# abajcsy/legged_games_gym

Hardware: AMD Instinct MI355X
Metric: env-steps/sec (whole node), ANYmal-C flat 4096 envs/GPU (higher is better)
Workload: dtype f32; 1 GPU; anymal_c_flat, 4096 envs/GPU, plane, actuator-net torques, self-collision ON (asset.self_collisions = 0), random-init policy [48, 128, 64, 32, 12] rollout (act = mu + sigma*eps), fixed command (0.5,0,0), obs noise + friction/mass randomisation + pushes on; envs_per_gpu=4096, decimation=4, parallelism=env-sharded x1, state_finite=True, policy=MFMA actor inside k_step (v_mfma_f32_16x16x4_f32, 4 waves)

## Files before the change

### legged_games_gym_amd/csrc/lg_kernels.hip

```cpp
#include <hip/hip_runtime.h>
#include <math.h>
#include <stdio.h>
#include <string.h>
#include <new>

#define LG_POLICY_BLOCKS_ONLY
#include "lg_host.h"

using namespace lg;

#define LG_BLOCK 64
#define LG_JS 40
#define LG_PASSES 2
#define LG_STEP_WAVES 4

struct AnymalTraits {
    static constexpr int K = 4, L = 3, NREP = 4, NPT = 5;
    static constexpr int pt_joint(int i) { return i < 2 ? 1 : 2; }
    static constexpr int pt_rep(int i) { return i < 2 ? 1 : (i < 4 ? 2 : 3); }
    static constexpr int FOOT_REP = 3;
    static constexpr int NCAP = 3, NGRP = 2;
    static constexpr int cap_p0(int c) { return 2 * c; }
    static constexpr int cap_p1(int c) { return c < 2 ? 2 * c + 1 : 4; }
    static constexpr int cap_grp(int c) { return c == 0 ? 0 : 1; }
    static constexpr int grp_c0(int g) { return g == 0 ? 0 : 2; }
    static constexpr int grp_c1(int g) { return g == 0 ? 1 : 4; }
    static constexpr int grp_cap_lo(int g) { return g == 0 ? 0 : 1; }
    static constexpr int grp_cap_hi(int g) { return g == 0 ? 1 : 3; }
};
struct CassieTraits {
    static constexpr int K = 2, L = 6, NREP = 6, NPT = 2;
    static constexpr int pt_joint(int) { return 5; }
    static constexpr int pt_rep(int) { return 5; }
    static constexpr int FOOT_REP = 5;
    static constexpr int NCAP = 1, NGRP = 1;
    static constexpr int cap_p0(int) { return 0; }
    static constexpr int cap_p1(int) { return 1; }
    static constexpr int cap_grp(int) { return 0; }
    static constexpr int grp_c0(int) { return 0; }
    static constexpr int grp_c1(int) { return 1; }
    static constexpr int grp_cap_lo(int) { return 0; }
    static constexpr int grp_cap_hi(int) { return 1; }
};
template <class T> struct Tab { static constexpr int GRP = T::L * LG_JS + 4 * T::NPT;
                          static constexpr int BPT = GRP + T::NGRP + 1;
                          static constexpr int STRIDE = BPT + 4; };
enum { J_POS = 0, J_ROT = 3, J_AXIS = 12, J_MASS = 15, J_COM = 16, J_INERTIA = 19, J_LO = 25, J_HI = 26, J_VLIM = 27,
       J_ARM = 28, J_DAMP = 29, J_KP = 30, J_KD = 31, J_Q0 = 32, J_TLIM = 33, J_SLO = 34, J_SHI = 35, J_DVL = 36,
       J_SUBM = 37  };

struct BaseTab { float mass, com[3], inertia[6]; float pts[LG_MAX_BASE_POINTS][4]; int32_t num_pts; float mass_robot; };

struct RollArgs {
    int      steps;
    float   *obs;
    const float *obs0;
    float   *actions, *mean;
    float   *rew;
    uint8_t *done, *time_outs;
    float   *extras;
    int      sub;
    int     *cursor;
};

struct PostHead {
    int32_t  resample_interval, heading_command, push_interval, max_episode_length;
    float    max_push_vel; uint32_t termination_mask, penalised_mask, _pad0;
    int64_t *episode_length_buf; float *commands, *contact_forces; uint32_t _pad[2];
};
struct PostRew {
    float    dt_policy, soft_dof_vel_limit, soft_torque_limit, max_contact_force, base_height_target, tracking_sigma;
    int32_t  only_positive_rewards; uint32_t slot_mask ; int32_t num_height_points, terrain_curriculum;
    float   *last_actions, *feet_air_time; uint8_t *last_contacts;
    float    reward_scale[LG_NUM_REWARD_TERMS];
    float   *env_origins; uint32_t _pad[2];
};
struct PostObs {
    float    obs_scale_lin_vel, obs_scale_ang_vel, obs_scale_dof_pos, obs_scale_dof_vel;
    float    noise_lin_vel, noise_ang_vel, noise_gravity, noise_dof_pos, noise_dof_vel, clip_observations;
    int32_t  add_noise, num_obs, num_envs; uint32_t _pad;
    float   *roll_obs;
};
struct PostStore {
    float   *dof_state, *actions, *torques, *last_actions, *last_dof_vel, *feet_air_time; uint8_t *last_contacts; float *root_states;
};
struct PostStoreEnv {
    float   *last_root_vel, *commands, *base_lin_vel, *base_ang_vel, *projected_gravity, *rew_buf; uint8_t *reset_buf, *time_out_buf;
    int64_t *episode_length_buf; float *roll_rew; uint8_t *roll_done, *roll_time_outs;
};
struct PostArgs { PostHead head; PostRew rew; PostObs obs; PostStore store; PostStoreEnv store_env; };
static_assert(sizeof(PostHead) == 64 && sizeof(PostRew) == 160 && sizeof(PostObs) == 64 && sizeof(PostStore) == 64 && sizeof(PostStoreEnv) == 96, "blocks of whole 8-dword groups, no padding");
static_assert(LG_NUM_REWARD_TERMS <= 32, "PostRew::slot_mask");

struct KArgs {
    lg_params  P;
    lg_buffers B;
    BaseTab    base;
    const float *limb_table;
    const float *hpts;
    const float *weights;
    const float *actions_in;
    const int32_t *env_ids;
    int32_t    count;
    uint32_t   penalised_mask, termination_mask;
    unsigned int *done_counter;
    float *accum_alt;
    int   flush_parts;
    int   defer;
    int64_t    step;
    PolicyArgs pol;
    unsigned long long *prof;
    unsigned int *status;
    int   spin_limit;
    int   debug_skip;
    RollArgs roll;
    PostArgs post;
};

template <bool ROLL> LG_DEV const KArgs &step_args(const KArgs &A) {
    if constexpr (ROLL) {
        typedef __attribute__((address_space(4))) const KArgs *KernArgs;
        KernArgs p = (KernArgs)__builtin_amdgcn_kernarg_segment_ptr();
        asm volatile("" : "+s"(p));
        return *(const KArgs *)p;
    } else return A;
}

typedef uint32_t lg_u32x16 __attribute__((ext_vector_type(16)));
typedef uint32_t lg_u32x8 __attribute__((ext_vector_type(8)));
template <class S> struct KargFetch {
    static_assert(sizeof(S) % 32 == 0 && sizeof(S) <= 192, "blocks are fetched 16 and 8 dwords at a time");
    static constexpr int N16 = sizeof(S) / 64, N8 = sizeof(S) % 64 / 32;
    lg_u32x16 a[N16 ? N16 : 1];
    lg_u32x8  b;
};
template <class S> LG_DEV KargFetch<S> karg_request(const S &src) {
    typedef lg_u32x16 __attribute__((aligned(4))) w16;
    typedef lg_u32x8 __attribute__((aligned(4))) w8;
    typedef __attribute__((address_space(4))) const char *kptr;
    const kptr p = (kptr)reinterpret_cast<const char *>(&src);
    KargFetch<S> f;
#pragma unroll
    for (int i = 0; i < KargFetch<S>::N16; i++) f.a[i] = *(__attribute__((address_space(4))) const w16 *)(p + 64 * i);
    if constexpr (KargFetch<S>::N8 != 0) f.b = *(__attribute__((address_space(4))) const w8 *)(p + 64 * KargFetch<S>::N16);
    return f;
}
template <class S> LG_DEV S karg_take(KargFetch<S> &f) {
    S out;
#pragma unroll
    for (int i = 0; i < KargFetch<S>::N16; i++) { asm volatile("" : "+s"(f.a[i])); __builtin_memcpy(reinterpret_cast<char *>(&out) + 64 * i, &f.a[i], 64); }
    if constexpr (KargFetch<S>::N8 != 0) { asm volatile("" : "+s"(f.b)); __builtin_memcpy(reinterpret_cast<char *>(&out) + 64 * KargFetch<S>::N16, &f.b, 32); }
    return out;
}

LG_DEV const double *cmd_x_range(const KArgs &A) { return A.P.cmd_curriculum ? A.B.cmd_range : nullptr; }
LG_DEV void cmd_x_range_f32(const KArgs &A, float *out) {
    const double *xr = cmd_x_range(A);
    out[0] = xr ? (float)xr[0] : A.P.cmd_lin_vel_x[0];
    out[1] = xr ? (float)xr[1] : A.P.cmd_lin_vel_x[1];
}
LG_DEV bool curriculum_tick_step(const KArgs &A, int64_t step) {
    return A.P.cmd_curriculum && A.step < 0 && A.P.max_episode_length > 0 && step % A.P.max_episode_length == 0;
}

LG_DEV void lg_report(unsigned int *status, unsigned int bit) {
    if (status) __hip_atomic_fetch_or(status, bit, __ATOMIC_RELAXED, __HIP_MEMORY_SCOPE_SYSTEM);
}

#define LG_NPROF 20
#define LG_NPROF_BLOCKS 1024
#define LG_NPROF_ROLL 33
#define LG_NPROF_TOTAL (LG_NPROF + LG_NPROF_BLOCKS * 40 + LG_NPROF_ROLL * LG_NPROF_BLOCKS)
#ifdef LG_PROFILE
__device__ __forceinline__ void lg_prof(int idx, unsigned long long *out, unsigned long long note = 0) {
    __shared__ unsigned long long acc[LG_NPROF], prev, t0, w0;
    __builtin_amdgcn_sched_barrier(0);
    unsigned long long t = __builtin_readcyclecounter();
    if (threadIdx.x == 0) {
        if (idx < 0) { for (int i = 0; i < LG_NPROF; i++) acc[i] = 0; t0 = t; w0 = wall_clock64(); }
        else if (idx >= 18) { if (idx == 18) acc[18] = note; else acc[19] += note; t = prev; }
        else acc[idx] += t - prev;
        if (out) {
            acc[14] = t - t0; acc[15] = wall_clock64() - w0;
            if (blockIdx.x < LG_NPROF_BLOCKS) {
                unsigned long long *a = out + LG_NPROF + (size_t)blockIdx.x * 40, *b = a + 20;
                for (int i = 0; i < 16; i++) { a[i] += acc[i]; b[i] = acc[i]; }
                a[16] = a[16] > acc[14] ? a[16] : acc[14];
                b[16] = w0; b[17] = w0 + acc[15]; b[18] = acc[18]; b[19] = acc[19];
            }
        }
        prev = idx >= 18 ? prev : __builtin_readcyclecounter();
    }
    __builtin_amdgcn_sched_barrier(0);
}
#ifdef LG_PROFILE_LIGHT
#define LG_PROF(i)
#else
#define LG_PROF(i) lg_prof(i, nullptr)
#endif
#define LG_PROF_NOTE(i, v) lg_prof(i, nullptr, v)
#define LG_PROF_BEGIN() lg_prof(-1, nullptr)
#define LG_PROF_END(i, out) lg_prof(i, out)
#ifdef LG_PROFILE_LIGHT
#define LG_PROF_COUNT(f, cond) do { if ((f) == 1 || (f) == 2) { if (__ballot(cond)) lg_prof(19, nullptr, 1ull << (8 * (f))); } } while (0)
#else
#define LG_PROF_COUNT(f, cond) do { const unsigned long long b_ = __ballot(cond); if (b_) lg_prof(19, nullptr, (1ull << (8 * (f))) + ((f) == 0 ? (unsigned long long)__popcll(b_) << 48 : 0ull)); } while (0)
#endif
#else
#define LG_PROF(i)
#define LG_PROF_BEGIN()
#define LG_PROF_END(i, out)
#define LG_PROF_NOTE(i, v)
#define LG_PROF_COUNT(f, cond)
#endif
enum { PF_PROLOGUE = 0, PF_TORQUE, PF_KINEMATICS, PF_INWARD, PF_BASE, PF_OUTWARD, PF_INTEGRATE, PF_POST, PF_EXTRAS,
       PF_POST_HEIGHTS, PF_POST_TERMS, PF_POST_REWARD, PF_POST_RESET, PF_POST_OBS };

struct HfFetch { int16_t s00, s10, s01, s11; float tx, ty; };
template <bool HF> LG_DEV HfFetch hf_fetch(const KArgs &A, float x, float y) {
    HfFetch f; f.s00 = f.s10 = f.s01 = f.s11 = 0; f.tx = f.ty = 0.0f;
    if (!HF) return f;
    const lg_params &P = A.P;
    float inv = 1.0f / P.hf_horizontal_scale;
    float gx = (x + P.hf_border) * inv, gy = (y + P.hf_border) * inv;
    if (!(fabsf(gx) < 1e9f)) gx = 0.0f;
    if (!(fabsf(gy) < 1e9f)) gy = 0.0f;
    float fx = floorf(gx), fy = floorf(gy);
    int ix = (int)fx, iy = (int)fy;
    f.tx = gx - fx; f.ty = gy - fy;
    auto at = [&](int i, int j) {
        i = min(max(i, 0), P.hf_rows - 1); j = min(max(j, 0), P.hf_cols - 1);
        return A.B.height_samples[(size_t)i * P.hf_cols + j];
    };
    f.s00 = at(ix, iy); f.s10 = at(ix + 1, iy); f.s01 = at(ix, iy + 1); f.s11 = at(ix + 1, iy + 1);
    return f;
}
template <bool HF> LG_DEV void hf_contact(const KArgs &A, const HfFetch &f, float pz, float radius, float &depth, V3 &n) {
    if (!HF) { n = v3(0, 0, 1); depth = radius - pz; return; }
    const lg_params &P = A.P;
    float inv = 1.0f / P.hf_horizontal_scale;
    float h00 = (float)f.s00 * P.hf_vertical_scale, h10 = (float)f.s10 * P.hf_vertical_scale;
    float h01 = (float)f.s01 * P.hf_vertical_scale, h11 = (float)f.s11 * P.hf_vertical_scale;
    const float thr = P.hf_step_threshold;
    float wall_depth = -1e30f; V3 wall_n = v3(0, 0, 1);
    if (thr > 0.0f) {
        const float hs = P.hf_horizontal_scale;
        if (fmaxf(fabsf(h10 - h00), fabsf(h11 - h01)) > thr) {
            const bool up = (h10 + h11) > (h00 + h01);
            const float top = up ? h10 + (h11 - h10) * f.ty : h00 + (h01 - h00) * f.ty;
            const float dist = (up ? 1.0f - f.tx : f.tx) * hs;
            if (pz - radius < top) {
                float d = radius - dist; V3 fn = v3(up ? -1.0f : 1.0f, 0, 0);
                if (pz > top) {
                    const float dz = pz - top, len = sqrtf(dist * dist + dz * dz), il = 1.0f / fmaxf(len, 1e-9f);
                    d = radius - len; fn = v3((up ? -dist : dist) * il, 0, dz * il);
                }
                if (d > wall_depth) { wall_depth = d; wall_n = fn; }
            }
            if (up) { h10 = h00; h11 = h01; } else { h00 = h10; h01 = h11; }
        }
        if (fmaxf(fabsf(h01 - h00), fabsf(h11 - h10)) > thr) {
            const bool up = (h01 + h11) > (h00 + h10);
            const float top = up ? h01 + (h11 - h01) * f.tx : h00 + (h10 - h00) * f.tx;
            const float dist = (up ? 1.0f - f.ty : f.ty) * hs;
            if (pz - radius < top) {
                float d = radius - dist; V3 fn = v3(0, up ? -1.0f : 1.0f, 0);
                if (pz > top) {
                    const float dz = pz - top, len = sqrtf(dist * dist + dz * dz), il = 1.0f / fmaxf(len, 1e-9f);
                    d = radius - len; fn = v3(0, (up ? -dist : dist) * il, dz * il);
                }
                if (d > wall_depth) { wall_depth = d; wall_n = fn; }
            }
            if (up) { h01 = h00; h11 = h10; } else { h00 = h01; h10 = h11; }
        }
    }
    float hx0 = h00 + (h10 - h00) * f.tx, hx1 = h01 + (h11 - h01) * f.tx;
    float h = hx0 + (hx1 - hx0) * f.ty;
    float dhdx = ((h10 - h00) + ((h11 - h01) - (h10 - h00)) * f.ty) * inv;
    float dhdy = (hx1 - hx0) * inv;
    float l = 1.0f / sqrtf(dhdx * dhdx + dhdy * dhdy + 1.0f);
    n = v3(-dhdx * l, -dhdy * l, l);
    depth = radius - (pz - h) * n.z;
    if (wall_depth > depth) { depth = wall_depth; n = wall_n; }
}
struct Contact { V3 r, n, vc, f, fs; float depth, bt, vtn; bool on; };

LG_DEV float prod_rn(float a, float b) {
#pragma clang fp contract(off)
    return a * b;
}
LG_DEV float sub_rn(float a, float b) {
#pragma clang fp contract(off)
    return a - b;
}
LG_DEV float plane_normal_force(const lg_params &P, float kn, float depth, float vz) {
    return __builtin_fmaf(-kn, vz, prod_rn(P.contact_stiffness, depth));
}
LG_DEV V3 plane_force(const Contact &c, V3 v, float fn) {
    return v3(sub_rn(c.fs.x, prod_rn(v.x, c.bt)), sub_rn(c.fs.y, prod_rn(v.y, c.bt)), fn);
}
LG_DEV float plane_slip_speed(V3 v) { return sqrtf(__builtin_fmaf(v.x, v.x, prod_rn(v.y, v.y))); }

template <bool HF>
LG_DEV void contact_setup(Contact &c, const lg_params &P, float mu, V3 r, V3 n, float depth, V3 vc, V3 fprev) {
    if constexpr (!HF) {
        c.r = r; c.depth = depth; c.vc = vc; c.on = depth > -P.contact_margin; c.f = v3(0, 0, 0); c.fs = v3(0, 0, 0);
        c.vtn = plane_slip_speed(vc);
        float fn_est = fmaxf(fprev.z, 0.0f);
        c.bt = fminf(P.friction_damping, mu * fn_est / fmaxf(c.vtn, P.stick_velocity));
        return;
    }
    c.r = r; c.n = n; c.depth = depth; c.vc = vc; c.on = depth > -P.contact_margin; c.f = v3(0, 0, 0); c.fs = v3(0, 0, 0);
    float vn0 = dot(n, vc);
    V3 vt0 = vc - n * vn0;
    c.vtn = sqrtf(dot(vt0, vt0));
    float fn_est = fmaxf(dot(n, fprev), 0.0f);
    c.bt = fminf(P.friction_damping, mu * fn_est / fmaxf(c.vtn, P.stick_velocity));
}
template <bool HF>
LG_DEV void contact_assemble(const Contact &c, const lg_params &P, float kn, AI &IA, S6 &pA) {
    if constexpr (!HF) {
        if (c.on) {
            const float dt = P.sim_dt;
            const V3 f = plane_force(c, c.vc, plane_normal_force(P, kn, c.depth, c.vc.z));
            ai_add_point(IA, dt * c.bt, c.r);
            const float kk = kn - c.bt, k = prod_rn(dt, kk), kx = prod_rn(k, c.r.x), ky = prod_rn(k, c.r.y);
            IA.A[0] = __builtin_fmaf(ky, c.r.y, IA.A[0]); IA.A[1] = __builtin_fmaf(-c.r.x, ky, IA.A[1]); IA.A[3] = __builtin_fmaf(kx, c.r.x, IA.A[3]);
            IA.H[2] = __builtin_fmaf(c.r.y, k, IA.H[2]); IA.H[5] = __builtin_fmaf(-c.r.x, k, IA.H[5]);
            IA.M[5] = __builtin_fmaf(dt, kk, IA.M[5]);
            const V3 rxf = v3(__builtin_fmaf(c.r.y, f.z, -prod_rn(c.r.z, f.y)), __builtin_fmaf(c.r.z, f.x, -prod_rn(c.r.x, f.z)),
                              __builtin_fmaf(c.r.x, f.y, -prod_rn(c.r.y, f.x)));
            pA.w = pA.w - rxf;
            pA.v = pA.v - f;
            asm volatile("" : "+v"(IA.H[0]), "+v"(IA.H[4]), "+v"(IA.H[8]), "+v"(IA.M[1]), "+v"(IA.M[2]), "+v"(IA.M[4]));
        }
        return;
    }
    if (c.on) {
        const float dt = P.sim_dt;
        float vn = dot(c.n, c.vc);
        V3 vt = c.vc - c.n * vn;
        V3 f = c.n * (P.contact_stiffness * c.depth - kn * vn) - vt * c.bt + c.fs;
        ai_add_point(IA, dt * c.bt, c.r);
        ai_add_rank1(IA, dt * (kn - c.bt), cross(c.r, c.n), c.n);
        pA.w = pA.w - cross(c.r, f);
        pA.v = pA.v - f;
    }
}
template <bool HF>
LG_DEV void contact_evaluate(Contact &c, const lg_params &P, float kn, float mu, S6 acc, bool more = true) {
    if constexpr (!HF) {
        if (c.on) {
            V3 v1 = c.vc + (acc.v + cross(acc.w, c.r)) * P.sim_dt;
            float fn = plane_normal_force(P, kn, c.depth, v1.z);
            if (fn <= 0.0f) { c.on = false; c.f = v3(0, 0, 0); }
            else {
                c.f = plane_force(c, v1, fn);
                if (!more) return;
                float vtm = plane_slip_speed(v1), cone = mu * fn;
                if (c.bt * vtm > cone) { const float s = -cone / vtm; c.fs = v3(v1.x * s, v1.y * s, 0.0f); c.bt = 0.0f; }
                else if (c.bt > 0.0f) c.bt = fminf(P.friction_damping, cone / fmaxf(vtm, P.stick_velocity));
            }
        }
        return;
    }
    if (c.on) {
        V3 v1 = c.vc + (acc.v + cross(acc.w, c.r)) * P.sim_dt;
        float vn = dot(c.n, v1);
        V3 vt = v1 - c.n * vn;
        float fn = P.contact_stiffness * c.depth - kn * vn;
        if (fn <= 0.0f) { c.on = false; c.f = v3(0, 0, 0); }
        else {
            c.f = c.n * fn - vt * c.bt + c.fs;
            if (!more) return;
            float vtm = sqrtf(dot(vt, vt)), cone = mu * fn;
            if (c.bt * vtm > cone) { c.fs = vt * (-cone / vtm); c.bt = 0.0f; }
            else if (c.bt > 0.0f) c.bt = fminf(P.friction_damping, cone / fmaxf(vtm, P.stick_velocity));
        }
    }
}

LG_DEV float motor_torque(float tau, float qd, float vlim) {
    if (vlim <= 0.0f || tau * qd <= 0.0f) return tau;
    float s = (vlim - fabsf(qd)) / (0.1f * vlim);
    return tau * fminf(fmaxf(s, 0.0f), 1.0f);
}
LG_DEV V3 clamp_norm(V3 a, float lim) {
    float n2 = dot(a, a);
    if (!(n2 <= lim * lim)) { float k = (n2 > 0.0f && n2 < INFINITY) ? lim * __builtin_amdgcn_rsqf(n2) : 0.0f; return a * k; }
    return a;
}

LG_DEV void body_terms(V3 grav, float m, V3 com_l, const float *Il, const M3 &R, V3 w, V3 v, RI &I0, S6 &p0) {
    V3 c = mul(R, com_l);
    M3 Ilf; Ilf.m[0] = Il[0]; Ilf.m[1] = Il[1]; Ilf.m[2] = Il[2]; Ilf.m[3] = Il[1]; Ilf.m[4] = Il[3]; Ilf.m[5] = Il[4];
    Ilf.m[6] = Il[2]; Ilf.m[7] = Il[4]; Ilf.m[8] = Il[5];
    M3 Rt;
#pragma unroll
    for (int i = 0; i < 3; i++)
#pragma unroll
        for (int j2 = 0; j2 < 3; j2++) Rt.m[3 * i + j2] = R.m[3 * j2 + i];
    M3 Ic = mul(mul(R, Ilf), Rt);
    I0.A[0] = Ic.m[0]; I0.A[1] = Ic.m[1]; I0.A[2] = Ic.m[2]; I0.A[3] = Ic.m[4]; I0.A[4] = Ic.m[5]; I0.A[5] = Ic.m[8];
    {
        float cc = dot(c, c);
        I0.A[0] += m * (cc - c.x * c.x); I0.A[1] -= m * c.x * c.y; I0.A[2] -= m * c.x * c.z;
        I0.A[3] += m * (cc - c.y * c.y); I0.A[4] -= m * c.y * c.z; I0.A[5] += m * (cc - c.z * c.z);
    }
    I0.h = v3(prod_rn(m, c.x), prod_rn(m, c.y), prod_rn(m, c.z));
    I0.m = m;
    V3 l = (v + cross(w, c)) * m;
    V3 n = mul(Ic, w) + cross(c, l);
    V3 fg = grav * m;
    p0.w = (cross(w, n) + cross(v, l)) - cross(c, fg);
    p0.v = cross(w, l) - fg;
}
LG_DEV void body_terms(V3 grav, float m, V3 com_l, const float *Il, const M3 &R, V3 w, V3 v, AI &I0, S6 &p0) {
    V3 c = mul(R, com_l);
    M3 Ilf; Ilf.m[0] = Il[0]; Ilf.m[1] = Il[1]; Ilf.m[2] = Il[2]; Ilf.m[3] = Il[1]; Ilf.m[4] = Il[3]; Ilf.m[5] = Il[4];
    Ilf.m[6] = Il[2]; Ilf.m[7] = Il[4]; Ilf.m[8] = Il[5];
    M3 Rt;
#pragma unroll
    for (int i = 0; i < 3; i++)
#pragma unroll
        for (int j2 = 0; j2 < 3; j2++) Rt.m[3 * i + j2] = R.m[3 * j2 + i];
    M3 Ic = mul(mul(R, Ilf), Rt);
#pragma unroll
    for (int i = 0; i < 9; i++) I0.H[i] = 0.0f;
#pragma unroll
    for (int i = 0; i < 6; i++) I0.M[i] = 0.0f;
    I0.A[0] = Ic.m[0]; I0.A[1] = Ic.m[1]; I0.A[2] = Ic.m[2]; I0.A[3] = Ic.m[4]; I0.A[4] = Ic.m[5]; I0.A[5] = Ic.m[8];
    ai_add_point(I0, m, c);
    V3 l = (v + cross(w, c)) * m;
    V3 n = mul(Ic, w) + cross(c, l);
    V3 fg = grav * m;
    p0.w = (cross(w, n) + cross(v, l)) - cross(c, fg);
    p0.v = cross(w, l) - fg;
}
struct FkOut { M3 R; V3 db, ax, w, v; };
LG_DEV FkOut fk_joint(const float *tj, const M3 &Rpar, V3 wpar, V3 vpar, float q, float qd) {
    FkOut o;
    o.db = mul(Rpar, v3(tj[J_POS], tj[J_POS + 1], tj[J_POS + 2]));
    M3 Rfix;
#pragma unroll
    for (int i = 0; i < 9; i++) Rfix.m[i] = tj[J_ROT + i];
    const M3 Rz = mul(Rpar, Rfix);
    o.ax = v3(Rz.m[0], Rz.m[3], Rz.m[6]);
    float sn, cs;
    __sincosf(q, &sn, &cs);
#pragma unroll
    for (int r = 0; r < 3; r++) {
        o.R.m[3 * r] = Rz.m[3 * r];
        o.R.m[3 * r + 1] = cs * Rz.m[3 * r + 1] + sn * Rz.m[3 * r + 2];
        o.R.m[3 * r + 2] = cs * Rz.m[3 * r + 2] - sn * Rz.m[3 * r + 1];
    }
    o.w = wpar + o.ax * qd;
    o.v = vpar + cross(wpar, o.db);
    return o;
}
template <bool HF> struct RigidOf { typedef RI type; };
template <> struct RigidOf<true> { typedef AI type; };
template <bool HF> struct BtQuads { static constexpr int N = HF ? 7 : 4; };
LG_DEV void bt_store(float4 (*dst)[LG_BLOCK], int lane, const RI &I, const S6 &p) {
    dst[0][lane] = make_float4(I.A[0], I.A[1], I.A[2], I.A[3]); dst[1][lane] = make_float4(I.A[4], I.A[5], I.h.x, I.h.y);
    dst[2][lane] = make_float4(I.h.z, I.m, p.w.x, p.w.y); dst[3][lane] = make_float4(p.w.z, p.v.x, p.v.y, p.v.z);
}
LG_DEV void bt_store(float4 (*dst)[LG_BLOCK], int lane, const AI &I, const S6 &p) {
    dst[0][lane] = make_float4(I.A[0], I.A[1], I.A[2], I.A[3]); dst[1][lane] = make_float4(I.A[4], I.A[5], I.H[0], I.H[1]);
    dst[2][lane] = make_float4(I.H[2], I.H[3], I.H[4], I.H[5]); dst[3][lane] = make_float4(I.H[6], I.H[7], I.H[8], I.M[0]);
    dst[4][lane] = make_float4(I.M[1], I.M[2], I.M[3], I.M[4]); dst[5][lane] = make_float4(I.M[5], p.w.x, p.w.y, p.w.z);
    dst[6][lane] = make_float4(p.v.x, p.v.y, p.v.z, 0.0f);
}
LG_DEV void bt_load(const float4 (*src)[LG_BLOCK], int lane, AI &I, S6 &p) {
    float4 a = src[0][lane], b = src[1][lane], c = src[2][lane], d = src[3][lane], e = src[4][lane], f = src[5][lane], g = src[6][lane];
    I.A[0] = a.x; I.A[1] = a.y; I.A[2] = a.z; I.A[3] = a.w; I.A[4] = b.x; I.A[5] = b.y; I.H[0] = b.z; I.H[1] = b.w;
    I.H[2] = c.x; I.H[3] = c.y; I.H[4] = c.z; I.H[5] = c.w; I.H[6] = d.x; I.H[7] = d.y; I.H[8] = d.z; I.M[0] = d.w;
    I.M[1] = e.x; I.M[2] = e.y; I.M[3] = e.z; I.M[4] = e.w; I.M[5] = f.x; p.w = v3(f.y, f.z, f.w); p.v = v3(g.x, g.y, g.z);
}
LG_DEV void bt_load(const float4 (*src)[LG_BLOCK], int lane, RI &I, S6 &p) {
    float4 a = src[0][lane], b = src[1][lane], c = src[2][lane], d = src[3][lane];
    I.A[0] = a.x; I.A[1] = a.y; I.A[2] = a.z; I.A[3] = a.w; I.A[4] = b.x; I.A[5] = b.y; I.h = v3(b.z, b.w, c.x); I.m = c.y;
    p.w = v3(c.z, c.w, d.x); p.v = v3(d.y, d.z, d.w);
}

#define LG_SC_REC 4
template <class T> struct SelfLds {
    float4 pos[T::NPT][LG_BLOCK];
    float4 vel[T::NPT][LG_BLOCK];
    float4 grp[T::NGRP][LG_BLOCK];
    float4 basepose[5][LG_BLOCK];
    float4 rec[T::K][T::NGRP][LG_SC_REC][LG_BLOCK];
    alignas(16) int ready[LG_STEP_WAVES];
    float4 base_pts[LG_MAX_BASE_POINTS];
};
LG_DEV V3 xyz(float4 a) { return v3(a.x, a.y, a.z); }
template <bool SA, bool SB> LG_DEV void seg_seg_closest(V3 a0, V3 a1, V3 b0, V3 b1, float &s, float &t) {
    const float eps = 1e-12f;
    V3 d1 = a1 - a0, d2 = b1 - b0, r = a0 - b0;
    float a = SA ? 0.0f : dot(d1, d1), e = SB ? 0.0f : dot(d2, d2), f = SB ? 0.0f : dot(d2, r);
    if ((SA || a <= eps) && (SB || e <= eps)) { s = 0.0f; t = 0.0f; }
    else if (SA || a <= eps) { s = 0.0f; t = fminf(fmaxf(f / e, 0.0f), 1.0f); }
    else {
        float c = dot(d1, r);
        if (SB || e <= eps) { t = 0.0f; s = fminf(fmaxf(-c / a, 0.0f), 1.0f); }
        else {
            float b = dot(d1, d2), denom = a * e - b * b;
            s = (denom > eps) ? fminf(fmaxf((b * f - c * e) / denom, 0.0f), 1.0f) : 0.0f;
            t = (b * s + f) / e;
            if (t < 0.0f) { t = 0.0f; s = fminf(fmaxf(-c / a, 0.0f), 1.0f); }
            else if (t > 1.0f) { t = 1.0f; s = fminf(fmaxf((b - c) / a, 0.0f), 1.0f); }
        }
    }
}
struct SelfHit { V3 n, pa, pb; float depth, f0; };
template <bool SA, bool SB, class Vel>
LG_DEV bool capsule_contact(const lg_params &P, float kn, V3 a0, V3 a1, float ra, V3 b0, V3 b1, float rb, Vel vel, SelfHit &h) {
    float s, t;
    seg_seg_closest<SA, SB>(a0, a1, b0, b1, s, t);
    V3 ca = a0 + (a1 - a0) * s, cb = b0 + (b1 - b0) * t, diff = ca - cb;
// ... 605 lines not shown
    static constexpr int NZB = T::L > 4 ? 2 : 1;
    enum { ROOT0 = NB, ROOT1, CMD, TERRAIN, CMD_STEP, PUSH, NOISE, SLOTS = NOISE + 3 * NZB };
    float4 u[SLOTS][LG_BLOCK];
    LG_DEV void put(const lg_params &P, int e, int64_t step, int lane, int slot, int purpose, int block) {
        float r[4];
        rand4(P.seed, e, step, purpose, block, r);
        u[slot][lane] = make_float4(r[0], r[1], r[2], r[3]);
    }
    LG_DEV void draw(const lg_params &P, int e, int k, int64_t step, int lane, int h, int nh) {
        const int b0 = (k * T::L) >> 2;
#pragma unroll
        for (int s = 0; s < SLOTS; s++) {
            if (s % nh != h) continue;
            if (s < NB) put(P, e, step, lane, s, RNG_DOF, b0 + s);
            else if (s == ROOT0) put(P, e, step, lane, s, RNG_ROOT, 0);
            else if (s == ROOT1) put(P, e, step, lane, s, RNG_ROOT, 1);
            else if (s == CMD) put(P, e, step, lane, s, RNG_CMD_RESET, 0);
            else if (s == TERRAIN) { if (P.terrain_curriculum) put(P, e, step, lane, s, RNG_TERRAIN, 0); }
            else if (s == CMD_STEP) put(P, e, step, lane, s, RNG_CMD_STEP, 0);
            else if (s == PUSH) { if (P.push_interval > 0 && step % P.push_interval == 0) put(P, e, step, lane, s, RNG_PUSH, 0); }
            else if (P.add_noise) put(P, e, step, lane, s, RNG_NOISE, ((s - NOISE) / NZB * T::K + k) * 2 + (s - NOISE) % NZB);
        }
    }
    LG_DEV void get(int slot, int lane, float (&out)[4]) const { const float4 w = u[slot][lane]; out[0] = w.x; out[1] = w.y; out[2] = w.z; out[3] = w.w; }
};

template <class T>
LG_DEV void reset_values(const KArgs &A, const float *tab, int e, int k, int64_t step, float (&root)[13], float (&q)[T::L],
                         float (&qd)[T::L], float (&cmd)[4], float (&origin)[3], int &level, bool &level_changed, const float *xr ,
                         const ResetRand<T> *rr = nullptr, int lane = 0) {
    constexpr int L = T::L;
    const lg_params &P = A.P;
    float u[4], v[4];
    auto uniforms = [&](int purpose, int block, int slot, float (&out)[4]) {
        if (rr) rr->get(slot, lane, out);
        else rand4(P.seed, e, step, purpose, block, out);
    };
    level_changed = false;
    if (P.terrain_curriculum && A.B.terrain_levels) {
        float dx = root[0] - origin[0], dy = root[1] - origin[1], dist = sqrtf(dx * dx + dy * dy);
        int up = dist > P.terrain_env_length / 2;
        int down = (dist < sqrtf(cmd[0] * cmd[0] + cmd[1] * cmd[1]) * P.max_episode_length_s * 0.5f) && !up;
        int lvl = A.B.terrain_levels[e] + up - down;
        if (lvl >= P.terrain_num_rows) {
            uniforms(RNG_TERRAIN, 0, ResetRand<T>::TERRAIN, u);
            lvl = (int)(u[0] * P.terrain_num_rows);
            if (lvl >= P.terrain_num_rows) lvl = P.terrain_num_rows - 1;
        } else if (lvl < 0) lvl = 0;
        level = lvl; level_changed = true;
        const float *to = A.B.terrain_origins + ((size_t)lvl * P.terrain_num_cols + A.B.terrain_types[e]) * 3;
        origin[0] = to[0]; origin[1] = to[1]; origin[2] = to[2];
    }
    const int b0 = (k * L) >> 2;
#pragma unroll
    for (int j = 0; j < L; j++) {
        int d = k * L + j;
        float uj;
        if (rr) uj = reinterpret_cast<const float *>(&rr->u[(d >> 2) - b0][lane])[d & 3];
        else {
            rand4(P.seed, e, step, RNG_DOF, d >> 2, u);
            uj = (d & 3) == 0 ? u[0] : ((d & 3) == 1 ? u[1] : ((d & 3) == 2 ? u[2] : u[3]));
        }
        q[j] = tab[j * LG_JS + J_Q0] * urange(0.5f, 1.5f, uj);
        qd[j] = 0.0f;
    }
#pragma unroll
    for (int i = 0; i < 13; i++) root[i] = P.base_init_state[i];
    root[0] += origin[0]; root[1] += origin[1]; root[2] += origin[2];
    uniforms(RNG_ROOT, 0, ResetRand<T>::ROOT0, u); uniforms(RNG_ROOT, 1, ResetRand<T>::ROOT1, v);
    if (P.custom_origins) { root[0] += urange(-1.0f, 1.0f, u[0]); root[1] += urange(-1.0f, 1.0f, u[1]); }
    root[7] = urange(-0.5f, 0.5f, u[2]); root[8] = urange(-0.5f, 0.5f, u[3]);
    root[9] = urange(-0.5f, 0.5f, v[0]); root[10] = urange(-0.5f, 0.5f, v[1]);
    root[11] = urange(-0.5f, 0.5f, v[2]); root[12] = urange(-0.5f, 0.5f, v[3]);
    uniforms(RNG_CMD_RESET, 0, ResetRand<T>::CMD, u);
    resample_commands_u(P, xr, u, cmd);
}

template <class T, bool UB = false >
LG_DEV void write_observations(const KArgs &A, int e, int k, bool live, int64_t step, const float *root, const float (&q)[T::L],
                               const float (&qd)[T::L], const float (&act)[T::L], const float *tab, V3 blv, V3 bav, V3 pg,
                               const float (&cmd)[4], bool heights_from_buffer ,
                               const ResetRand<T> *rr = nullptr, int lane = 0, float *obs_out = nullptr ,
                               float *lds_row = nullptr ,
                               const PostObs *ub = nullptr) {
    constexpr int K = T::K, L = T::L;
    const lg_params &P = A.P;
#define LG_OBS_U(f) (UB ? ub->f : P.f)
    float head[12] = {blv.x * LG_OBS_U(obs_scale_lin_vel), blv.y * LG_OBS_U(obs_scale_lin_vel), blv.z * LG_OBS_U(obs_scale_lin_vel),
                      bav.x * LG_OBS_U(obs_scale_ang_vel), bav.y * LG_OBS_U(obs_scale_ang_vel), bav.z * LG_OBS_U(obs_scale_ang_vel),
                      pg.x, pg.y, pg.z,
                      cmd[0] * LG_OBS_U(obs_scale_lin_vel), cmd[1] * LG_OBS_U(obs_scale_lin_vel), cmd[2] * LG_OBS_U(obs_scale_ang_vel)};
    float hnz[12] = {LG_OBS_U(noise_lin_vel), LG_OBS_U(noise_lin_vel), LG_OBS_U(noise_lin_vel), LG_OBS_U(noise_ang_vel), LG_OBS_U(noise_ang_vel), LG_OBS_U(noise_ang_vel),
                     LG_OBS_U(noise_gravity), LG_OBS_U(noise_gravity), LG_OBS_U(noise_gravity), 0.0f, 0.0f, 0.0f};
    float val[4][L], nz[4][L];
#pragma unroll
    for (int j = 0; j < L; j++) {
        float hv = head[j], hn = hnz[j];
#pragma unroll
        for (int kk = 1; kk < K; kk++) { hv = (k == kk) ? head[kk * L + j] : hv; hn = (k == kk) ? hnz[kk * L + j] : hn; }
        val[0][j] = hv; nz[0][j] = hn;
        val[1][j] = (q[j] - tab[j * LG_JS + J_Q0]) * LG_OBS_U(obs_scale_dof_pos); nz[1][j] = LG_OBS_U(noise_dof_pos);
        val[2][j] = qd[j] * LG_OBS_U(obs_scale_dof_vel); nz[2][j] = LG_OBS_U(noise_dof_vel);
        val[3][j] = act[j]; nz[3][j] = 0.0f;
    }
    float *obs = (UB ? obs_out : (obs_out ? obs_out : A.B.obs_buf)) + (size_t)e * LG_OBS_U(num_obs);
#pragma unroll
    for (int g = 0; g < 4; g++) {
        float u[4], u2[4];
        const bool noisy = LG_OBS_U(add_noise) && g < 3;
        if (noisy) {
            if (rr) { rr->get(ResetRand<T>::NOISE + g * ResetRand<T>::NZB, lane, u); if (L > 4) rr->get(ResetRand<T>::NOISE + g * ResetRand<T>::NZB + 1, lane, u2); }
            else {
                rand4(P.seed, e, step, RNG_NOISE, (g * K + k) * 2, u);
                if (L > 4) rand4(P.seed, e, step, RNG_NOISE, (g * K + k) * 2 + 1, u2);
            }
        }
#pragma unroll
        for (int j = 0; j < L; j++) {
            float o = val[g][j];
            if (noisy) {
                float uj = (j < 4) ? u[j & 3] : u2[j & 3];
                o += (2.0f * uj - 1.0f) * nz[g][j];
            }
            o = fminf(fmaxf(o, -LG_OBS_U(clip_observations)), LG_OBS_U(clip_observations));
            if (live) obs[g * 12 + k * L + j] = o;
            if (lds_row) lds_row[g * 12 + k * L + j] = o;
        }
    }
#undef LG_OBS_U
    if (P.measure_heights && heights_from_buffer) {
        const float *mh = A.B.measured_heights + (size_t)e * P.num_height_points;
        const int nchunk = (P.num_height_points + 3) >> 2;
        for (int c = k; c < nchunk; c += K) {
            float u[4] = {0, 0, 0, 0}, hv[4];
#pragma unroll
            for (int t = 0; t < 4; t++) hv[t] = mh[min(4 * c + t, P.num_height_points - 1)];
            if (P.add_noise) rand4(P.seed, e, step, RNG_NOISE_H, c, u);
#pragma unroll
            for (int t = 0; t < 4; t++) {
                int i = 4 * c + t;
                if (i < P.num_height_points) {
                    float h = root[2] - 0.5f - hv[t];
                    float o = fminf(fmaxf(h, -1.0f), 1.0f) * P.obs_scale_height;
                    if (P.add_noise) o += (2.0f * u[t] - 1.0f) * P.noise_height;
                    o = fminf(fmaxf(o, -P.clip_observations), P.clip_observations);
                    if (live) obs[48 + i] = o;
                }
            }
        }
    }
}

template <class T> LG_DEV void stage_base_points(const KArgs &A, SelfLds<T> *sc) {
    if (threadIdx.x == 0) {
#pragma unroll
        for (int i = 0; i < LG_MAX_BASE_POINTS; i++) sc->base_pts[i] = make_float4(A.base.pts[i][0], A.base.pts[i][1], A.base.pts[i][2], A.base.pts[i][3]);
    }
}
template <class T> LG_DEV void stage_limb_table(const KArgs &A, float *lds_tab) {
    for (int i = threadIdx.x; i < T::K * Tab<T>::STRIDE; i += blockDim.x) lds_tab[i] = A.limb_table[i];
    __syncthreads();
}

LG_DEV float *accum_slot(const KArgs &A, int64_t step) { return (A.defer && (step & 1)) ? A.accum_alt : A.B.extras_accum; }
LG_DEV int *level_parts_slot(const KArgs &A, int64_t step, int nwg) { return reinterpret_cast<int *>(A.done_counter + 1) + ((step & 1) ? nwg : 0); }
LG_DEV void finish_extras(const KArgs &A, int t, int64_t step_used, bool publish_step, float *accum, const int *parts = nullptr, int n_parts = 0, bool do_levels = true) {
    const lg_params &P = A.P;
    const int R = P.num_reward_slots;
    __shared__ float level_part[16];
    if (publish_step && t == 0 && A.B.step_counter) A.B.step_counter[0] = step_used;
    float cnt = __hip_atomic_load(accum + R, __ATOMIC_RELAXED, __HIP_MEMORY_SCOPE_AGENT);
    float v = (t < R) ? __hip_atomic_load(accum + t, __ATOMIC_RELAXED, __HIP_MEMORY_SCOPE_AGENT) : 0.0f;
    const bool levels = do_levels && P.terrain_curriculum && A.B.terrain_levels;
    if (levels) {
        float acc = 0.0f;
        const int nt = blockDim.x;
        constexpr int INFLIGHT = 8;
        const int n_items = parts ? n_parts : P.num_envs;
        const int *items = parts ? parts : A.B.terrain_levels;
        for (int e0 = t; e0 < n_items; e0 += nt * INFLIGHT) {
            int lv[INFLIGHT];
#pragma unroll
            for (int u = 0; u < INFLIGHT; u++) {
                const int e = e0 + u * nt;
                lv[u] = e < n_items ? __hip_atomic_load(items + e, __ATOMIC_RELAXED, __HIP_MEMORY_SCOPE_AGENT) : 0;
            }
#pragma unroll
            for (int u = 0; u < INFLIGHT; u++) acc += (float)lv[u];
        }
#pragma unroll
        for (int o = 32; o > 0; o >>= 1) acc += __shfl_xor(acc, o);
        if ((t & 63) == 0) level_part[t >> 6] = acc;
    }
    __syncthreads();
    if (t >= 64) return;
    if (t < R) {
        if (cnt > 0.0f) A.B.episode_means[t] = v / cnt / P.max_episode_length_s;
        __hip_atomic_store(accum + t, 0.0f, __ATOMIC_RELAXED, __HIP_MEMORY_SCOPE_AGENT);
    }
    if (t == R) __hip_atomic_store(accum + R, 0.0f, __ATOMIC_RELAXED, __HIP_MEMORY_SCOPE_AGENT);
    if (levels && t == 0) {
        float acc = 0.0f;
        for (int w = 0; w < (int)(blockDim.x >> 6); w++) acc += level_part[w];
        A.B.episode_means[R] = acc / (float)P.num_envs;
    }
}
LG_DEV void roll_finish(const KArgs &A, int t, int64_t step0, int rt0, int rt1) {
    const lg_params &P = A.P;
    const int R = P.num_reward_slots, stride = LG_NUM_REWARD_TERMS + 2;
    int last = -1;
    for (int s = rt1 - 1; s >= rt0 && last < 0; s--)
        if (__hip_atomic_load(A.roll.extras + (size_t)s * stride + R, __ATOMIC_RELAXED, __HIP_MEMORY_SCOPE_AGENT) > 0.0f) last = s;
    if (last >= 0 && t < R) {
        const float v = __hip_atomic_load(A.roll.extras + (size_t)last * stride + t, __ATOMIC_RELAXED, __HIP_MEMORY_SCOPE_AGENT);
        const float c = __hip_atomic_load(A.roll.extras + (size_t)last * stride + R, __ATOMIC_RELAXED, __HIP_MEMORY_SCOPE_AGENT);
        A.B.episode_means[t] = v / c / P.max_episode_length_s;
    }
    if (t == 0 && A.B.step_counter) A.B.step_counter[0] = step0 + rt1 - 1;
    if (t == 0 && A.roll.cursor) A.roll.cursor[0] = rt1;
    __builtin_amdgcn_s_waitcnt(0);
    __builtin_amdgcn_wave_barrier();
    for (int i = rt0 * stride + t; i < rt1 * stride; i += 64) __hip_atomic_store(A.roll.extras + i, 0.0f, __ATOMIC_RELAXED, __HIP_MEMORY_SCOPE_AGENT);
}

LG_DEV void redraw_reset_command(const KArgs &A, float x0, float x1, int e, int64_t step, float *obs_row) {
    const lg_params &P = A.P; const lg_buffers &B = A.B;
    float u[4], cmd[4];
#pragma unroll
    for (int i = 0; i < 4; i++) cmd[i] = B.commands[(size_t)e * 4 + i];
    rand4(P.seed, e, step, RNG_CMD_RESET, 0, u);
    resample_commands_x(P, x0, x1, u, cmd);
#pragma unroll
    for (int i = 0; i < 4; i++) B.commands[(size_t)e * 4 + i] = cmd[i];
    const float c = P.clip_observations;
    obs_row[9] = fminf(fmaxf(cmd[0] * P.obs_scale_lin_vel, -c), c); obs_row[10] = fminf(fmaxf(cmd[1] * P.obs_scale_lin_vel, -c), c);
    obs_row[11] = fminf(fmaxf(cmd[2] * P.obs_scale_ang_vel, -c), c);
}
LG_DEV void curriculum_apply(const KArgs &A, int t, int nt, int64_t step, float cnt, const uint8_t *resets, float *obs) {
    const lg_params &P = A.P;
    if (!(cnt > 0.0f) || P.cmd_curriculum_slot < 0) return;
    double *xr = A.B.cmd_range;
    const double mean_sum = (double)A.B.episode_means[P.cmd_curriculum_slot] * P.cmd_episode_length_s;
    const double lo0 = xr[0], hi0 = xr[1];
    if (!(mean_sum / P.cmd_max_episode_length > 0.8 * P.cmd_tracking_scale_dt)) return;
    const double lo = fmin(fmax(lo0 - 0.5, -P.cmd_max_curriculum), 0.0), hi = fmin(fmax(hi0 + 0.5, 0.0), P.cmd_max_curriculum);
    if (lo == lo0 && hi == hi0) return;
    __syncthreads();
    if (t == 0) { xr[0] = lo; xr[1] = hi; }
    const float x0 = (float)lo, x1 = (float)hi;
    for (int e = t; e < P.num_envs; e += nt)
        if (resets[e]) redraw_reset_command(A, x0, x1, e, step, obs + (size_t)e * P.num_obs);
}

template <bool OFF, int L = 3, bool HF = false> struct StepSharedT {
    float pose[LG_BLOCK][5];
    float hsum[LG_STEP_WAVES][LG_BLOCK];
    float root_z[LG_BLOCK];
    int   rst[LG_BLOCK];
    float r_t[LG_NUM_REWARD_TERMS][LG_BLOCK];
    float4 fk[OFF ? L : 1][4][LG_BLOCK];
    float4 bt[OFF ? L : 1][BtQuads<HF>::N][LG_BLOCK];
    int    fk_ready;
};

struct EpisodeSums {
    float sum[LG_NUM_REWARD_TERMS] = {};
    LG_DEV void load(const KArgs &A, int e) {
#pragma unroll
        for (int t = 0; t < LG_NUM_REWARD_TERMS; t++) {
            const int slot = A.P.reward_slot[t];
            sum[t] = slot >= 0 ? A.B.episode_sums[(size_t)slot * A.P.num_envs + e] : 0.0f;
        }
    }
    template <int K, class SH> LG_DEV void update(const KArgs &A, int e, int lane, SH &sh, bool keep, float *accum) {
        const lg_params &P = A.P;
        const bool reset = keep && sh.rst[lane] != 0;
        if (keep) {
#pragma unroll
            for (int t = 0; t < LG_NUM_REWARD_TERMS; t++) {
                const int slot = P.reward_slot[t];
                if (slot >= 0) {
                    sum[t] += sh.r_t[t][lane];
                    A.B.episode_sums[(size_t)slot * P.num_envs + e] = reset ? 0.0f : sum[t];
                }
            }
        }
        const unsigned long long finished = __ballot(reset);
        if (finished == 0) return;
#pragma unroll
        for (int t = 0; t < LG_NUM_REWARD_TERMS; t++) sh.r_t[t][lane] = reset ? sum[t] : 0.0f;
        __builtin_amdgcn_fence(__ATOMIC_RELEASE, "wavefront");
        __builtin_amdgcn_wave_barrier();
        if (lane < LG_NUM_REWARD_TERMS) {
            int slot = -1;
#pragma unroll
            for (int t = 0; t < LG_NUM_REWARD_TERMS; t++) slot = lane == t ? P.reward_slot[t] : slot;
            float tot = 0.0f;
            for (int i = 0; i < LG_BLOCK; i += K) tot += sh.r_t[lane][i];
            if (slot >= 0) atomicAdd(accum + slot, tot);
        } else if (lane == LG_NUM_REWARD_TERMS) atomicAdd(accum + P.num_reward_slots, (float)__popcll(finished));
    }
};

template <class T, bool NET, bool HF, int NW, bool SC = false> struct HelperWave {
    static constexpr bool OFF = NW >= 2;
    static LG_DEV void run(const KArgs &A, int wave, int lane, int e, int k, int d0, bool live, int64_t step, const float *tab,
                           float2 (*lds_x)[LG_BLOCK], float (*lds_tau)[LG_BLOCK], StepSharedT<OFF, T::L, HF> &sh, SelfLds<T> *sc = nullptr,
                           const float *lds_tab = nullptr, ResetRand<T> *reset_rand = nullptr, int *s_last = nullptr, float4 (*hnoise)[LG_BLOCK] = nullptr,
                           int sub0 = 0 , float *roll_accum = nullptr ,
                           bool tick_step = false ) {
        const lg_buffers &B = A.B;
        const lg_params &P = A.P;
        const int j = wave - 1;
        bool missed = false;
        LstmSplit st;
        float (*part[4])[4] = {st.h0, st.c0, st.h1, st.c1};
        float *row[4] = {nullptr, nullptr, nullptr, nullptr};
        LstmLane LW;
        if (NET) {
            const size_t plane = (size_t)P.num_envs * (T::K * T::L);
            LW = lstm_load(A.weights, lane);
            row[0] = B.sea_hidden_state + (size_t)(d0 + j) * 8; row[1] = B.sea_cell_state + (size_t)(d0 + j) * 8;
            row[2] = B.sea_hidden_state + (plane + d0 + j) * 8; row[3] = B.sea_cell_state + (plane + d0 + j) * 8;
#pragma unroll
            for (int a = 0; a < 4; a++) {
                float4 lo = reinterpret_cast<const float4 *>(row[a])[0], hi = reinterpret_cast<const float4 *>(row[a])[1];
                float u[8] = {lo.x, lo.y, lo.z, lo.w, hi.x, hi.y, hi.z, hi.w};
                lstm_split(u, part[a][0], part[a][1]);
            }
        }
        if (NET || OFF) {
            for (int it = 0; it < P.decimation; it++) {
                __syncthreads();
                float tau_j = 0.0f;
                if (NET) {
                    const float2 x = lds_x[j][lane];
                    tau_j = actuator_step_mfma(LW, x.x, x.y, st);
                    lds_tau[j][lane] = tau_j;
                }
                if (OFF) {
                    volatile int *flag = &sh.fk_ready;
                    int spin = 0;
                    for (; *flag < sub0 + it + 1 && spin < A.spin_limit; spin++) __builtin_amdgcn_s_sleep(1);
                    missed |= spin >= A.spin_limit;
#pragma unroll 1
                    for (int b = j; b < T::L; b += NW - 1) {
                        const float4 f0 = sh.fk[b][0][lane], f1 = sh.fk[b][1][lane], f2 = sh.fk[b][2][lane], f3 = sh.fk[b][3][lane];
                        M3 R; R.m[0] = f0.x; R.m[1] = f0.y; R.m[2] = f0.z; R.m[3] = f0.w; R.m[4] = f1.x; R.m[5] = f1.y; R.m[6] = f1.z; R.m[7] = f1.w; R.m[8] = f2.x;
                        const float *tb = tab + b * LG_JS;
                        float Il[6];
#pragma unroll
                        for (int i = 0; i < 6; i++) Il[i] = tb[J_INERTIA + i];
                        typename RigidOf<HF>::type I0; S6 p0;
                        body_terms(v3(P.gravity[0], P.gravity[1], P.gravity[2]), tb[J_MASS], v3(tb[J_COM], tb[J_COM + 1], tb[J_COM + 2]), Il, R,
                                   v3(f2.y, f2.z, f2.w), v3(f3.x, f3.y, f3.z), I0, p0);
                        bt_store(sh.bt[b], lane, I0, p0);
                    }
                }
                __syncthreads();
                if constexpr (SC && NW == LG_STEP_WAVES) {
                    self_detect<T>(A, lds_tab, lane, wave, *sc);
                    if (wave == LG_STEP_WAVES - 1) self_detect<T>(A, lds_tab, lane, 0, *sc);
                    asm volatile("s_waitcnt lgkmcnt(0)" ::: "memory");
                    if (lane == 0 && A.debug_skip != 2) sc->ready[wave] = sub0 + it + 1;
                }
            }
        }
        reset_rand->draw(P, e, k, step, lane, wave - 1, NW - 1);
        if (P.measure_heights && P.add_noise) {
            const int nchunk = (P.num_height_points + 3) >> 2;
#pragma unroll
            for (int b = 0; b < HeightCrew<T, NW>::NCH; b++) {
                const int c = k + b * HeightCrew<T, NW>::NV;
                if (b % (NW > 1 ? NW - 1 : 1) == wave - 1 && c < nchunk) {
                    float r[4];
                    rand4(P.seed, e, step, RNG_NOISE_H, c, r);
                    hnoise[b][lane] = make_float4(r[0], r[1], r[2], r[3]);
                }
            }
        }
        if (NET) {
#pragma unroll
            for (int a = 0; a < 4; a++) {
                float u[8];
                lstm_unsplit(part[a][0], part[a][1], u);
                if (live) {
                    reinterpret_cast<float4 *>(row[a])[0] = make_float4(u[0], u[1], u[2], u[3]);
                    reinterpret_cast<float4 *>(row[a])[1] = make_float4(u[4], u[5], u[6], u[7]);
                }
            }
        }
        __syncthreads();
        HeightCrew<T, NW> hc;
        float hs = 0.0f;
        if (P.measure_heights) hs = hc.template sample<HF>(A, e, k + T::K * wave, live, sh.pose[lane][0], sh.pose[lane][1], sh.pose[lane][2], sh.pose[lane][3], sh.pose[lane][4]);
        sh.hsum[wave][lane] = hs;
        __syncthreads();
        const bool keeper = wave == 1 && live && k == 0;
        EpisodeSums es;
        if (keeper) es.load(A, e);
        float un[HeightCrew<T, NW>::NCH][4];
        if (P.measure_heights) hc.draw_noise(P, e, k + T::K * wave, step, un);
        __syncthreads();
        if (wave == 1) {
            es.template update<T::K>(A, e, lane, sh, keeper, roll_accum ? roll_accum : accum_slot(A, step));
            if (roll_accum) {  }
            else {
            if (P.terrain_curriculum && A.B.terrain_levels) {
                int lv = keeper ? __hip_atomic_load(A.B.terrain_levels + e, __ATOMIC_RELAXED, __HIP_MEMORY_SCOPE_AGENT) : 0;
#pragma unroll
                for (int o = 32; o > 0; o >>= 1) lv += __shfl_xor(lv, o);
                if (lane == 0) __hip_atomic_store(level_parts_slot(A, step, gridDim.x) + blockIdx.x, lv, __ATOMIC_RELAXED, __HIP_MEMORY_SCOPE_AGENT);
            }
            if (tick_step) {  }
            else if (A.defer) {
                if (lane == 0 && atomicAdd(A.done_counter, 1u) == gridDim.x - 1) {
                    if (B.step_counter) B.step_counter[0] = step;
                    __hip_atomic_store(A.done_counter, 0u, __ATOMIC_RELAXED, __HIP_MEMORY_SCOPE_AGENT);
                }
            } else {
            asm volatile("s_waitcnt vmcnt(0)" ::: "memory");
            if (lane == 0) {
                const unsigned int ticket = atomicAdd(A.done_counter, 1u);
                const int last = ticket == gridDim.x - 1;
                if (last) __hip_atomic_store(A.done_counter, 0u, __ATOMIC_RELAXED, __HIP_MEMORY_SCOPE_AGENT);
                *s_last = last;
            }
            }
            }
        }
        if (P.measure_heights) hc.write_obs(A, e, k + T::K * wave, live, step, sh.root_z[lane], un);
        if (missed && lane == 0) lg_report(A.status, LG_STATUS_FRAME_HANDOVER_TIMEOUT);
        if (NET) {
            const bool reset = sh.rst[lane] != 0 && live;
            if (__ballot(reset) != 0 && reset) {
#pragma unroll
                for (int a = 0; a < 4; a++) {
                    reinterpret_cast<float4 *>(row[a])[0] = make_float4(0.0f, 0.0f, 0.0f, 0.0f);
                    reinterpret_cast<float4 *>(row[a])[1] = make_float4(0.0f, 0.0f, 0.0f, 0.0f);
                }
            }
        }
    }
};

template <bool SC, class T> struct SelfStore { char unused; LG_DEV SelfLds<T> *get() { return nullptr; } };
template <class T> struct SelfStore<true, T> { SelfLds<T> lds; LG_DEV SelfLds<T> *get() { return &lds; } };

template <class T, bool NET, bool HF, bool POL = false, int NW = LG_STEP_WAVES, bool SC = false, bool ROLL = false>
__global__ void __launch_bounds__(NW * LG_BLOCK) k_step(const KArgs A_launch) {
    const KArgs &A = A_launch;
    static_assert(!NET || (NW == LG_STEP_WAVES && 1 + T::L == NW), "one actuator wave per joint of the limb");
    static_assert(!ROLL || (POL && !HF), "the multi-step rollout kernel is the fused-actor kernel on the plane");
    static_assert(!POL || (NET && NW == LG_POLICY_WAVES && T::K * T::L <= 16), "fused policy needs the four-wave actuator-net kernel");
    constexpr int K = T::K, L = T::L, ND = K * L, NREP = T::NREP;
    const lg_params &P = A.P;
    const lg_buffers &B = A.B;
    __shared__ float lds_tab[T::K * Tab<T>::STRIDE];
    __shared__ float2 lds_x[NET ? L : 1][LG_BLOCK];
    __shared__ float lds_tau[NET ? L : 1][LG_BLOCK];
    constexpr bool OFF = NW >= 2;
    __shared__ StepSharedT<OFF, L, HF> sh;
    __shared__ SelfStore<SC, T> sc_store;
    __shared__ ResetRand<T> reset_rand;
    __shared__ float4 hnoise[NW > 1 ? HeightCrew<T, NW>::NCH : 1][LG_BLOCK];
    __shared__ int s_last;
    __shared__ float4 pol_xa[POL ? 4 : 1][64], pol_xb[POL ? 8 : 1][64], pol_xy[1][64];
    __shared__ float lds_act[POL ? 16 : 1][16];
    __shared__ float lds_obs[ROLL ? 16 : 1][48];
    __shared__ float s_tick_cnt;
    __shared__ float s_xr[2];
    __shared__ int s_roll[2];
    int roll_begin = 0;
    if (ROLL && A.P.cmd_curriculum && A.roll.sub > 0) {
        roll_begin = A.roll.cursor[0];
        if (roll_begin >= A.roll.steps) return;
    }
    LG_PROF_BEGIN();
    if (threadIdx.x == 0) sh.fk_ready = 0;
    if constexpr (SC) {
        if (threadIdx.x < LG_STEP_WAVES) sc_store.get()->ready[threadIdx.x] = 0;
        stage_base_points<T>(A, sc_store.get());
    }
    stage_limb_table<T>(A, lds_tab);

    const int N = P.num_envs;
    const int wave = threadIdx.x / LG_BLOCK, lane = threadIdx.x % LG_BLOCK;
    const int tid = blockIdx.x * LG_BLOCK + lane;
    int e = tid / K;
    const int k = tid % K;
    const bool live = e < N;
    if (!live) e = N - 1;
    const float *tab = lds_tab + k * Tab<T>::STRIDE;
    const int d0 = e * ND + k * L;
    const int64_t step0 = A.step >= 0 ? A.step : B.step_counter[0] + 1 - roll_begin;
    if (threadIdx.x == 0) {
        cmd_x_range_f32(A, s_xr);
        if (ROLL) {
            int roll_end = A.roll.steps;
            if (P.cmd_curriculum) {
                const int64_t M = P.max_episode_length, first = step0 + roll_begin;
                roll_end = min(roll_end, roll_begin + (int)((M - first % M) % M) + 1);
            }
            s_roll[0] = roll_begin; s_roll[1] = roll_end;
        }
    }
    const int e_wg = e, k_wg = k;
    auto one_step = [&](const int rt) {
    const KArgs &A = step_args<ROLL>(A_launch);
    const lg_params &P = A.P;
    const lg_buffers &B = A.B;
    const int N = P.num_envs;
    int tix = threadIdx.x;
    if constexpr (ROLL) asm volatile("" : "+v"(tix));
    const int wave = tix / LG_BLOCK, lane = tix % LG_BLOCK;
    int e = e_wg;
    const int k = ROLL ? (blockIdx.x * LG_BLOCK + lane) % K : k_wg;
    if constexpr (ROLL) { e = (blockIdx.x * LG_BLOCK + lane) / K; if (e >= N) e = N - 1; }
    const float *tab = lds_tab + k * Tab<T>::STRIDE;
    int d0 = e * ND + k * L;
    const int64_t step = step0 + rt;
    const int sub0 = ROLL ? rt * P.decimation : 0;
    float *const roll_accum = ROLL ? A.roll.extras + (size_t)rt * (LG_NUM_REWARD_TERMS + 2) : nullptr;
    float *const roll_obs_out = nullptr;

    if (POL) {
        if (ROLL) {
            PolicyArgs pa = A.pol;
            pa.obs = A.roll.obs + (size_t)rt * N * P.num_obs;
            if (rt == 0 && A.roll.obs0) {
                pa.obs = A.roll.obs0;
                const size_t row0 = (size_t)blockIdx.x * 16 * P.num_obs;
                const int n = min(16, N - (int)blockIdx.x * 16) * P.num_obs;
                for (int i = tix; i < n; i += NW * LG_BLOCK) A.roll.obs[row0 + i] = A.roll.obs0[row0 + i];
            }
            pa.actions = A.roll.actions + (size_t)rt * N * ND;
            pa.mean = A.roll.mean ? A.roll.mean + (size_t)rt * N * ND : nullptr;
            policy_forward<3, 8, 4, 2>(pa, pol_xa, pol_xb, pol_xy, blockIdx.x, wave, lane, step, lds_act, rt > s_roll[0] ? lds_obs : nullptr);
        } else policy_forward<3, 8, 4, 2>(A.pol, pol_xa, pol_xb, pol_xy, blockIdx.x, wave, lane, step, lds_act);
        __syncthreads();
    }
    if (wave > 0) {
        HelperWave<T, NET, HF, NW, SC>::run(A, wave, lane, e, k, d0, live, step, tab, lds_x, lds_tau, sh, sc_store.get(), lds_tab, &reset_rand, &s_last, hnoise, sub0, roll_accum,
                                            !ROLL && curriculum_tick_step(A, step));
    } else {
    float root[13], q[L], qd[L], act[L], tau[L];
#pragma unroll
    for (int i = 0; i < 13; i++) root[i] = B.root_states[(size_t)e * 13 + i];
#pragma unroll
    for (int j = 0; j < L; j++) {
        float2 s = reinterpret_cast<const float2 *>(B.dof_state)[d0 + j];
        q[j] = s.x; qd[j] = s.y;
        float a = POL ? lds_act[k * L + j][lane / K] : A.actions_in[d0 + j];
        act[j] = fminf(fmaxf(a, -P.clip_actions), P.clip_actions);
        tau[j] = 0.0f;
    }
    const float mu = 0.5f * ((B.friction_coeffs ? B.friction_coeffs[e] : 1.0f) + P.ground_friction);
    const float base_mass = A.base.mass + (B.base_mass_delta ? B.base_mass_delta[e] : 0.0f);
    float last_qd[L];
    if (L <= 3) {
#pragma unroll
        for (int j = 0; j < L; j++) last_qd[j] = B.last_dof_vel[d0 + j];
    }

    float Frep[NREP][3], Fbase[3];
    {
        const float *cf = B.contact_forces + ((size_t)e * (1 + K * NREP) + 1 + k * NREP) * 3;
#pragma unroll
        for (int r = 0; r < NREP; r++) { Frep[r][0] = cf[3 * r]; Frep[r][1] = cf[3 * r + 1]; Frep[r][2] = cf[3 * r + 2]; }
        const float *c0 = B.contact_forces + (size_t)e * (1 + K * NREP) * 3;
        Fbase[0] = c0[0]; Fbase[1] = c0[1]; Fbase[2] = c0[2];
    }
    if (P.decimation == 0) {
#pragma unroll
        for (int j = 0; j < L; j++) tau[j] = B.torques[d0 + j];
    }
    LG_PROF(PF_PROLOGUE);
#pragma unroll 1
    for (int it = 0; it < P.decimation; it++) {
        if (!NET) pd_torques<L>(P, tab, act, q, qd, B.last_dof_vel + d0, tau);
        if (NET || OFF) {
            if (NET) {
#pragma unroll
                for (int j = 0; j < L; j++) lds_x[j][lane] = make_float2(act[j] * P.action_scale + tab[j * LG_JS + J_Q0] - q[j], qd[j]);
            }
            __syncthreads();
            auto join = [&]() {
                __syncthreads();
                if (NET) {
#pragma unroll
                    for (int j = 0; j < L; j++) tau[j] = lds_tau[j][lane];
                }
            };
            constexpr bool LEAN = NW == LG_STEP_WAVES && L <= 3 && !HF;
            physics_substep<T, HF, decltype(join), OFF, SC, LEAN, ROLL>(A, tab, k, root, q, qd, tau, base_mass, mu, Frep, Fbase, join, sh.bt, sh.fk, &sh.fk_ready, sub0 + it + 1,
                                                                  sc_store.get(), it == P.decimation - 1, SC && NW == LG_STEP_WAVES);
        } else {
            physics_substep<T, HF, NoWait, false, SC>(A, tab, k, root, q, qd, tau, base_mass, mu, Frep, Fbase, NoWait(), nullptr, nullptr, nullptr, 0,
                                                      sc_store.get(), it == P.decimation - 1);
        }
    }

    if (L > 3) {
        asm volatile("" : "+v"(e));
        d0 = e * ND + k * L;
    }
#define U_(blk, arg) (ROLL ? (blk) : (arg))
    PostHead ph; PostRew pr; PostObs po; PostStore ps; PostStoreEnv pe;
    KargFetch<PostRew> pr_f; KargFetch<PostObs> po_f; KargFetch<PostStore> ps_f; KargFetch<PostStoreEnv> pe_f;
    if constexpr (ROLL) { KargFetch<PostHead> ph_f = karg_request(A.post.head); ph = karg_take(ph_f); }
    int64_t ep_len = U_(ph.episode_length_buf, B.episode_length_buf)[e] + 1;
    V3 blv = quat_rotate_inverse(root + 3, v3(root[7], root[8], root[9]));
    V3 bav = quat_rotate_inverse(root + 3, v3(root[10], root[11], root[12]));
    V3 pg = quat_rotate_inverse(root + 3, v3(0, 0, -1));
    float cmd[4];
#pragma unroll
    for (int i = 0; i < 4; i++) cmd[i] = U_(ph.commands, B.commands)[(size_t)e * 4 + i];
    constexpr bool EARLY_POST = L <= 3 && HF;
    float last_act[L], fat, origin[3];
    uint8_t lc;
    if (EARLY_POST) {
#pragma unroll
        for (int j = 0; j < L; j++) last_act[j] = B.last_actions[d0 + j];
        fat = B.feet_air_time[(size_t)e * K + k];
        lc = B.last_contacts[(size_t)e * K + k];
#pragma unroll
        for (int i = 0; i < 3; i++) origin[i] = B.env_origins[(size_t)e * 3 + i];
    }
    sh.pose[lane][0] = root[0]; sh.pose[lane][1] = root[1]; sh.pose[lane][2] = root[2]; sh.pose[lane][3] = root[5]; sh.pose[lane][4] = root[6];
    __syncthreads();
    if (ep_len % U_(ph.resample_interval, P.resample_interval) == 0) {
        if (NW > 1) { float u[4]; reset_rand.get(ResetRand<T>::CMD_STEP, lane, u); resample_commands_u(P, s_xr, u, cmd); }
        else resample_commands(P, s_xr, e, step, RNG_CMD_STEP, cmd);
    }
    if (U_(ph.heading_command, P.heading_command)) {
        V3 fwd = quat_apply(root + 3, v3(1, 0, 0));
        float heading = atan2f(fwd.y, fwd.x);
        cmd[2] = fminf(fmaxf(0.5f * wrap_to_pi(cmd[3] - heading), -1.0f), 1.0f);
    }
    HeightCrew<T, NW> hc;
    float hsum = 0.0f;
    if (U_(0, P.measure_heights)) hsum = hc.template sample<HF>(A, e, k, live, root[0], root[1], root[2], root[5], root[6]);
    sh.hsum[0][lane] = hsum;
    if constexpr (ROLL) pr_f = karg_request(A.post.rew);
    __syncthreads();
    if constexpr (ROLL) pr = karg_take(pr_f);
    if (NW == 4) hsum = (sh.hsum[0][lane] + sh.hsum[1][lane]) + (sh.hsum[2][lane] + sh.hsum[3][lane]);
    else if (NW == 2) hsum = sh.hsum[0][lane] + sh.hsum[1][lane];
    if (U_(ph.push_interval, P.push_interval) > 0 && step % U_(ph.push_interval, P.push_interval) == 0) {
        float u[4];
        if (NW > 1) reset_rand.get(ResetRand<T>::PUSH, lane, u);
        else rand4(P.seed, e, step, RNG_PUSH, 0, u);
        root[7] = urange(-U_(ph.max_push_vel, P.max_push_vel), U_(ph.max_push_vel, P.max_push_vel), u[0]);
        root[8] = urange(-U_(ph.max_push_vel, P.max_push_vel), U_(ph.max_push_vel, P.max_push_vel), u[1]);
    }

    const int rep0 = 1 + k * NREP;
    if (live) {
        float *cf = U_(ph.contact_forces, B.contact_forces) + ((size_t)e * (1 + K * NREP) + rep0) * 3;
#pragma unroll
        for (int r = 0; r < NREP; r++) { cf[3 * r] = Frep[r][0]; cf[3 * r + 1] = Frep[r][1]; cf[3 * r + 2] = Frep[r][2]; }
        if (k == 0) { float *c0 = U_(ph.contact_forces, B.contact_forces) + (size_t)e * (1 + K * NREP) * 3; c0[0] = Fbase[0]; c0[1] = Fbase[1]; c0[2] = Fbase[2]; }
    }
    LG_PROF(PF_POST_HEIGHTS);
    int term_local = 0;
    float coll_local = 0.0f;
#pragma unroll
    for (int r = 0; r < NREP; r++) {
        float n = sqrtf(Frep[r][0] * Frep[r][0] + Frep[r][1] * Frep[r][1] + Frep[r][2] * Frep[r][2]);
        if ((U_(ph.termination_mask, A.termination_mask) >> (rep0 + r)) & 1u) term_local |= (n > 1.0f);
        if ((U_(ph.penalised_mask, A.penalised_mask) >> (rep0 + r)) & 1u) coll_local += (n > 0.1f) ? 1.0f : 0.0f;
    }
    float nbase = sqrtf(Fbase[0] * Fbase[0] + Fbase[1] * Fbase[1] + Fbase[2] * Fbase[2]);
    int contact_term = group_or<K>(term_local);
    if (U_(ph.termination_mask, A.termination_mask) & 1u) contact_term |= (nbase > 1.0f);
    float coll = group_sum<K>(coll_local);
    if (U_(ph.penalised_mask, A.penalised_mask) & 1u) coll += (nbase > 0.1f) ? 1.0f : 0.0f;
    const bool time_out = ep_len > U_(ph.max_episode_length, P.max_episode_length);
    int bad = 0;
#pragma unroll
    for (int i = 0; i < 13; i++) bad |= !isfinite(root[i]);
#pragma unroll
    for (int j = 0; j < L; j++) bad |= !isfinite(q[j]) || !isfinite(qd[j]);
    bad = group_or<K>(bad);
    const bool reset = contact_term || time_out || bad;

    if (!EARLY_POST) {
#pragma unroll
        for (int j = 0; j < L; j++) { last_act[j] = U_(pr.last_actions, B.last_actions)[d0 + j]; if (L > 3) last_qd[j] = B.last_dof_vel[d0 + j]; }
    }
    float s_ar = 0, s_acc = 0, s_lim = 0, s_dv = 0, s_dvl = 0, s_tl = 0, s_tq = 0, s_ss = 0;
#pragma unroll
    for (int j = 0; j < L; j++) {
        const float *tj = tab + j * LG_JS;
        float da = last_act[j] - act[j]; s_ar += da * da;
        float dd = (last_qd[j] - qd[j]) / U_(pr.dt_policy, P.dt_policy); s_acc += dd * dd;
        float ol = -fminf(q[j] - tj[J_SLO], 0.0f); ol += fmaxf(q[j] - tj[J_SHI], 0.0f); s_lim += ol;
        s_dv += qd[j] * qd[j];
        s_dvl += fminf(fmaxf(fabsf(qd[j]) - tj[J_DVL] * U_(pr.soft_dof_vel_limit, P.soft_dof_vel_limit), 0.0f), 1.0f);
        s_tl += fmaxf(fabsf(tau[j]) - tj[J_TLIM] * U_(pr.soft_torque_limit, P.soft_torque_limit), 0.0f);
        s_tq += tau[j] * tau[j];
        s_ss += fabsf(q[j] - tj[J_Q0]);
    }
    s_ar = group_sum<K>(s_ar); s_acc = group_sum<K>(s_acc); s_lim = group_sum<K>(s_lim); s_dv = group_sum<K>(s_dv);
    s_dvl = group_sum<K>(s_dvl); s_tl = group_sum<K>(s_tl); s_tq = group_sum<K>(s_tq); s_ss = group_sum<K>(s_ss);
    const float *ff = Frep[T::FOOT_REP];
    const float cmd_xy = sqrtf(cmd[0] * cmd[0] + cmd[1] * cmd[1]);
    float fnorm = sqrtf(ff[0] * ff[0] + ff[1] * ff[1] + ff[2] * ff[2]);
    float fcf = group_sum<K>(fmaxf(fnorm - U_(pr.max_contact_force, P.max_contact_force), 0.0f));
    int stumble = group_or<K>(sqrtf(ff[0] * ff[0] + ff[1] * ff[1]) > 5.0f * fabsf(ff[2]) ? 1 : 0);
    float nfly = group_sum<K>(ff[2] > 0.1f ? 1.0f : 0.0f);
    float air = 0.0f;
    if (!EARLY_POST) { fat = U_(pr.feet_air_time, B.feet_air_time)[(size_t)e * K + k]; lc = U_(pr.last_contacts, B.last_contacts)[(size_t)e * K + k]; }
    if (U_(pr.reward_scale[LG_REW_FEET_AIR_TIME], P.reward_scale[LG_REW_FEET_AIR_TIME]) != 0.0f) {
        bool contact = ff[2] > 1.0f, filt = contact || lc;
        lc = (uint8_t)contact;
        bool first = (fat > 0.0f) && filt;
        fat += U_(pr.dt_policy, P.dt_policy);
        air = (fat - 0.5f) * (first ? 1.0f : 0.0f);
        fat *= filt ? 0.0f : 1.0f;
        air = group_sum<K>(air) * ((cmd_xy > 0.1f) ? 1.0f : 0.0f);
    }
    const float base_h = U_(0, P.measure_heights) ? group_sum<K>(hsum) / (float)U_(pr.num_height_points, P.num_height_points) : root[2];
    float term[LG_NUM_REWARD_TERMS];
    term[LG_REW_ACTION_RATE] = s_ar;
    term[LG_REW_ANG_VEL_XY] = bav.x * bav.x + bav.y * bav.y;
    term[LG_REW_BASE_HEIGHT] = (base_h - U_(pr.base_height_target, P.base_height_target)) * (base_h - U_(pr.base_height_target, P.base_height_target));
    term[LG_REW_COLLISION] = coll;
    term[LG_REW_DOF_ACC] = s_acc;
    term[LG_REW_DOF_POS_LIMITS] = s_lim;
    term[LG_REW_DOF_VEL] = s_dv;
    term[LG_REW_DOF_VEL_LIMITS] = s_dvl;
    term[LG_REW_FEET_AIR_TIME] = air;
    term[LG_REW_FEET_CONTACT_FORCES] = fcf;
    term[LG_REW_LIN_VEL_Z] = blv.z * blv.z;
    term[LG_REW_NO_FLY] = (nfly == 1.0f) ? 1.0f : 0.0f;
    term[LG_REW_ORIENTATION] = pg.x * pg.x + pg.y * pg.y;
    term[LG_REW_STAND_STILL] = s_ss * ((cmd_xy < 0.1f) ? 1.0f : 0.0f);
    term[LG_REW_STUMBLE] = stumble ? 1.0f : 0.0f;
    term[LG_REW_TERMINATION] = (reset && !time_out) ? 1.0f : 0.0f;
    term[LG_REW_TORQUE_LIMITS] = s_tl;
    term[LG_REW_TORQUES] = s_tq;
    {
        float ex = cmd[0] - blv.x, ey = cmd[1] - blv.y, ew = cmd[2] - bav.z;
        term[LG_REW_TRACKING_LIN_VEL] = __expf(-(ex * ex + ey * ey) / U_(pr.tracking_sigma, P.tracking_sigma));
        term[LG_REW_TRACKING_ANG_VEL] = __expf(-(ew * ew) / U_(pr.tracking_sigma, P.tracking_sigma));
    }
    LG_PROF(PF_POST_TERMS);
    float rew = 0.0f;
    const bool writer = live && k == 0;
    float r_t[LG_NUM_REWARD_TERMS];
#pragma unroll
    for (int t = 0; t < LG_NUM_REWARD_TERMS; t++) r_t[t] = U_((pr.slot_mask >> t) & 1u, P.reward_slot[t] >= 0) ? term[t] * U_(pr.reward_scale[t], P.reward_scale[t]) : 0.0f;
#pragma unroll
    for (int t = 0; t < LG_NUM_REWARD_TERMS; t++) if (t != LG_REW_TERMINATION) rew += r_t[t];
    if (U_(pr.only_positive_rewards, P.only_positive_rewards)) rew = fmaxf(rew, 0.0f);
    rew += r_t[LG_REW_TERMINATION];
#pragma unroll
    for (int t = 0; t < LG_NUM_REWARD_TERMS; t++) sh.r_t[t][lane] = r_t[t];

    LG_PROF(PF_POST_REWARD);
    if (!EARLY_POST) { const float *eo = U_(pr.env_origins, B.env_origins); origin[0] = eo[(size_t)e * 3]; origin[1] = eo[(size_t)e * 3 + 1]; origin[2] = eo[(size_t)e * 3 + 2]; }
    if (reset) {
        int level = 0; bool level_changed = false;
        reset_values<T>(A, tab, e, k, step, root, q, qd, cmd, origin, level, level_changed, s_xr, NW > 1 ? &reset_rand : nullptr, lane);
        if (writer && level_changed) {
            __hip_atomic_store(B.terrain_levels + e, level, __ATOMIC_RELAXED, __HIP_MEMORY_SCOPE_AGENT);
            B.env_origins[(size_t)e * 3] = origin[0]; B.env_origins[(size_t)e * 3 + 1] = origin[1]; B.env_origins[(size_t)e * 3 + 2] = origin[2];
        }
        fat = 0.0f; ep_len = 0;
    }

    sh.rst[lane] = reset ? 1 : 0; sh.root_z[lane] = root[2];
    if (NW > 1 && U_(pr.terrain_curriculum, P.terrain_curriculum)) asm volatile("s_waitcnt vmcnt(0)" ::: "memory");
    if constexpr (ROLL) { po_f = karg_request(A.post.obs); ps_f = karg_request(A.post.store); }
    __syncthreads();
    if constexpr (ROLL) { po = karg_take(po_f); ps = karg_take(ps_f); }
    if (NW == 1) { EpisodeSums es; const bool keep = live && k == 0; if (keep) es.load(A, e); es.template update<K>(A, e, lane, sh, keep, accum_slot(A, step)); }

    LG_PROF(PF_POST_RESET);
#ifdef LG_PROFILE
    { int nr = 0; for (int i = 0; i < LG_BLOCK; i += K) nr += sh.rst[i]; LG_PROF_NOTE(18, (unsigned long long)nr); }
#endif
    if constexpr (ROLL) write_observations<T, true>(A, e, k, live, step, root, q, qd, act, tab, blv, bav, pg, cmd, false, &reset_rand, lane,
                                                    po.roll_obs + (size_t)(rt + 1) * po.num_envs * po.num_obs, lds_obs[lane / K], &po);
    else write_observations<T>(A, e, k, live, step, root, q, qd, act, tab, blv, bav, pg, cmd, false, NW > 1 ? &reset_rand : nullptr, lane, roll_obs_out, ROLL ? lds_obs[lane / K] : nullptr);
    if (U_(0, P.measure_heights)) {
        if (NW > 1) {
            float un[HeightCrew<T, NW>::NCH][4];
#pragma unroll
            for (int b = 0; b < HeightCrew<T, NW>::NCH; b++) { const float4 w = hnoise[b][lane]; un[b][0] = w.x; un[b][1] = w.y; un[b][2] = w.z; un[b][3] = w.w; }
            hc.write_obs(A, e, k, live, step, root[2], un);
        } else hc.write_obs(A, e, k, live, step, root[2]);
    }

    LG_PROF(PF_POST_OBS);
    if constexpr (ROLL) pe_f = karg_request(A.post.store_env);
    if (live) {
#pragma unroll
        for (int j = 0; j < L; j++) {
            reinterpret_cast<float2 *>(U_(ps.dof_state, B.dof_state))[d0 + j] = make_float2(q[j], qd[j]);
            U_(ps.actions, B.actions)[d0 + j] = act[j];
            U_(ps.torques, B.torques)[d0 + j] = tau[j];
            U_(ps.last_actions, B.last_actions)[d0 + j] = act[j];
            U_(ps.last_dof_vel, B.last_dof_vel)[d0 + j] = qd[j];
        }
        U_(ps.feet_air_time, B.feet_air_time)[(size_t)e * K + k] = fat;
        U_(ps.last_contacts, B.last_contacts)[(size_t)e * K + k] = lc;
        if constexpr (ROLL) pe = karg_take(pe_f);
        if (k == 0) {
#pragma unroll
            for (int i = 0; i < 13; i++) U_(ps.root_states, B.root_states)[(size_t)e * 13 + i] = root[i];
#pragma unroll
            for (int i = 0; i < 6; i++) U_(pe.last_root_vel, B.last_root_vel)[(size_t)e * 6 + i] = root[7 + i];
#pragma unroll
            for (int i = 0; i < 4; i++) U_(pe.commands, B.commands)[(size_t)e * 4 + i] = cmd[i];
            float *const o_blv = U_(pe.base_lin_vel, B.base_lin_vel), *const o_bav = U_(pe.base_ang_vel, B.base_ang_vel), *const o_pg = U_(pe.projected_gravity, B.projected_gravity);
            o_blv[(size_t)e * 3] = blv.x; o_blv[(size_t)e * 3 + 1] = blv.y; o_blv[(size_t)e * 3 + 2] = blv.z;
            o_bav[(size_t)e * 3] = bav.x; o_bav[(size_t)e * 3 + 1] = bav.y; o_bav[(size_t)e * 3 + 2] = bav.z;
            o_pg[(size_t)e * 3] = pg.x; o_pg[(size_t)e * 3 + 1] = pg.y; o_pg[(size_t)e * 3 + 2] = pg.z;
            U_(pe.rew_buf, B.rew_buf)[e] = rew;
            U_(pe.reset_buf, B.reset_buf)[e] = (uint8_t)reset;
            U_(pe.time_out_buf, B.time_out_buf)[e] = (uint8_t)time_out;
            U_(pe.episode_length_buf, B.episode_length_buf)[e] = ep_len;
            if constexpr (ROLL) {
                pe.roll_rew[(size_t)rt * po.num_envs + e] = rew;
                pe.roll_done[(size_t)rt * po.num_envs + e] = (uint8_t)reset;
                pe.roll_time_outs[(size_t)rt * po.num_envs + e] = (uint8_t)time_out;
            }
        }
    }
#undef U_
    }
    };
    if constexpr (ROLL) {
#ifdef LG_PROFILE
        if (threadIdx.x == 0 && A.prof && blockIdx.x < LG_NPROF_BLOCKS) A.prof[LG_NPROF + LG_NPROF_BLOCKS * 40 + blockIdx.x] = wall_clock64();
#endif
        __syncthreads();
#pragma unroll 1
        for (int rt = s_roll[0]; rt < s_roll[1]; rt++) {
            one_step(rt);
            asm volatile("s_waitcnt lgkmcnt(0)\n\ts_barrier" ::: "memory");
#ifdef LG_PROFILE
            if (threadIdx.x == 0 && A.prof && blockIdx.x < LG_NPROF_BLOCKS && rt + 1 < LG_NPROF_ROLL)
                A.prof[LG_NPROF + LG_NPROF_BLOCKS * 40 + (size_t)(rt + 1) * LG_NPROF_BLOCKS + blockIdx.x] = wall_clock64();
#endif
        }
        const KArgs &A = step_args<ROLL>(A_launch);
        const lg_params &P = A.P;
        const int N = P.num_envs;
        const int roll_end = s_roll[1];
        const bool tick = P.cmd_curriculum && (step0 + roll_end - 1) % P.max_episode_length == 0;
        asm volatile("s_waitcnt vmcnt(0)" ::: "memory");
        if (tick) __threadfence();
        __syncthreads();
        if (threadIdx.x == 0) {
            const unsigned int ticket = atomicAdd(A.done_counter, 1u);
            s_last = (ticket == gridDim.x - 1);
            if (s_last) __hip_atomic_store(A.done_counter, 0u, __ATOMIC_RELAXED, __HIP_MEMORY_SCOPE_AGENT);
            if (s_last && tick) s_tick_cnt = __hip_atomic_load(A.roll.extras + (size_t)(roll_end - 1) * (LG_NUM_REWARD_TERMS + 2) + P.num_reward_slots,
                                                               __ATOMIC_RELAXED, __HIP_MEMORY_SCOPE_AGENT);
        }
        __syncthreads();
        if (s_last) {
            if (threadIdx.x < LG_BLOCK) roll_finish(A, threadIdx.x, step0, s_roll[0], roll_end);
            if (tick) {
                __threadfence();
                __syncthreads();
                curriculum_apply(A, threadIdx.x, blockDim.x, step0 + roll_end - 1, s_tick_cnt, A.roll.done + (size_t)(roll_end - 1) * N,
                                 A.roll.obs + (size_t)roll_end * N * P.num_obs);
            }
        }
        LG_PROF_END(PF_EXTRAS, A.prof);
        return;
    } else one_step(0);
    const int64_t step = step0;
    LG_PROF(PF_POST);
    if (curriculum_tick_step(A, step)) {
        __threadfence();
        __syncthreads();
        if (threadIdx.x == 0) {
            const unsigned int ticket = atomicAdd(A.done_counter, 1u);
            s_last = (ticket == gridDim.x - 1);
            if (s_last) {
                __hip_atomic_store(A.done_counter, 0u, __ATOMIC_RELAXED, __HIP_MEMORY_SCOPE_AGENT);
                s_tick_cnt = __hip_atomic_load(accum_slot(A, step) + P.num_reward_slots, __ATOMIC_RELAXED, __HIP_MEMORY_SCOPE_AGENT);
            }
        }
        __syncthreads();
        if (s_last) {
            __threadfence();
            if (A.defer) {
                finish_extras(A, threadIdx.x, step, false, accum_slot(A, step - 1), NW > 1 ? level_parts_slot(A, step - 1, gridDim.x) : nullptr, gridDim.x);
                __syncthreads();
            }
            finish_extras(A, threadIdx.x, step, true, accum_slot(A, step), NW > 1 ? level_parts_slot(A, step, gridDim.x) : nullptr, gridDim.x);
            __threadfence();
            __syncthreads();
            curriculum_apply(A, threadIdx.x, blockDim.x, step, s_tick_cnt, B.reset_buf, B.obs_buf);
        }
        LG_PROF_END(PF_EXTRAS, A.prof);
        return;
    }
    if (NW == 1 && !A.defer) {
        asm volatile("s_waitcnt vmcnt(0)" ::: "memory");
        if (threadIdx.x == 0) {
            unsigned int ticket = atomicAdd(A.done_counter, 1u);
            s_last = (ticket == gridDim.x - 1);
            if (s_last) __hip_atomic_store(A.done_counter, 0u, __ATOMIC_RELAXED, __HIP_MEMORY_SCOPE_AGENT);
        }
    }
    if (A.defer) {
        if (NW == 1 && threadIdx.x == 0 && atomicAdd(A.done_counter, 1u) == gridDim.x - 1) {
            if (B.step_counter) B.step_counter[0] = step;
            __hip_atomic_store(A.done_counter, 0u, __ATOMIC_RELAXED, __HIP_MEMORY_SCOPE_AGENT);
        }
        if (blockIdx.x == 0) finish_extras(A, threadIdx.x, step, false, accum_slot(A, step - 1), NW > 1 ? level_parts_slot(A, step - 1, gridDim.x) : nullptr, gridDim.x);
        LG_PROF_END(PF_EXTRAS, A.prof);
        return;
    }
    __syncthreads();
    if (s_last) finish_extras(A, threadIdx.x, step, true, A.B.extras_accum, NW > 1 ? level_parts_slot(A, step, gridDim.x) : nullptr, gridDim.x);
    LG_PROF_END(PF_EXTRAS, A.prof);
}

template <class T, bool NET>
__global__ void __launch_bounds__(LG_BLOCK) k_reset(const KArgs A) {
    constexpr int K = T::K, L = T::L, ND = K * L;
    const lg_params &P = A.P;
    const lg_buffers &B = A.B;
    __shared__ float lds_tab[T::K * Tab<T>::STRIDE];
    stage_limb_table<T>(A, lds_tab);
    const int tid = blockIdx.x * LG_BLOCK + threadIdx.x;
    const int idx = tid / K, k = tid % K;
    if (idx >= A.count) return;
    const int e = A.env_ids[idx];
    const int N = P.num_envs;
    const float *tab = lds_tab + k * Tab<T>::STRIDE;
    const int d0 = e * ND + k * L;
    float root[13], q[L], qd[L], cmd[4], origin[3];
#pragma unroll
    for (int i = 0; i < 13; i++) root[i] = B.root_states[(size_t)e * 13 + i];
#pragma unroll
    for (int i = 0; i < 4; i++) cmd[i] = B.commands[(size_t)e * 4 + i];
#pragma unroll
    for (int i = 0; i < 3; i++) origin[i] = B.env_origins[(size_t)e * 3 + i];
    int level = 0; bool level_changed = false;
    float xr[2];
    cmd_x_range_f32(A, xr);
    reset_values<T>(A, tab, e, k, A.step, root, q, qd, cmd, origin, level, level_changed, xr);
#pragma unroll
    for (int j = 0; j < L; j++) {
        reinterpret_cast<float2 *>(B.dof_state)[d0 + j] = make_float2(q[j], qd[j]);
        B.last_actions[d0 + j] = 0.0f;
        B.last_dof_vel[d0 + j] = 0.0f;
    }
    B.feet_air_time[(size_t)e * K + k] = 0.0f;
    if (NET) {
        const size_t plane = (size_t)N * ND;
#pragma unroll
        for (int j = 0; j < L; j++)
#pragma unroll
            for (int u = 0; u < 8; u++) {
                B.sea_hidden_state[(size_t)(d0 + j) * 8 + u] = 0.0f; B.sea_cell_state[(size_t)(d0 + j) * 8 + u] = 0.0f;
                B.sea_hidden_state[(plane + d0 + j) * 8 + u] = 0.0f; B.sea_cell_state[(plane + d0 + j) * 8 + u] = 0.0f;
            }
    }
    if (k == 0) {
#pragma unroll
        for (int i = 0; i < 13; i++) B.root_states[(size_t)e * 13 + i] = root[i];
#pragma unroll
        for (int i = 0; i < 4; i++) B.commands[(size_t)e * 4 + i] = cmd[i];
        if (level_changed) {
            B.terrain_levels[e] = level;
#pragma unroll
            for (int i = 0; i < 3; i++) B.env_origins[(size_t)e * 3 + i] = origin[i];
        }
        B.episode_length_buf[e] = 0;
        B.reset_buf[e] = 1;
        for (int t = 0; t < P.num_reward_slots; t++) {
            atomicAdd(B.extras_accum + t, B.episode_sums[(size_t)t * N + e]);
            B.episode_sums[(size_t)t * N + e] = 0.0f;
        }
        atomicAdd(B.extras_accum + P.num_reward_slots, 1.0f);
    }
}

__global__ void __launch_bounds__(64) k_extras(const KArgs A) {
    const int64_t last = A.step >= 0 ? A.step : (A.B.step_counter ? A.B.step_counter[0] : 0);
    finish_extras(A, threadIdx.x, A.step, false, A.B.extras_accum, A.flush_parts > 0 ? level_parts_slot(A, last, A.flush_parts) : nullptr, A.flush_parts);
    if (A.accum_alt) finish_extras(A, threadIdx.x, A.step, false, A.accum_alt, nullptr, 0, false);
}

__global__ void __launch_bounds__(64) k_actuator(const float *table, const float *pos_err, const float *vel, float *torques,
                                                  float *hidden, float *cell, int rows) {
    const int lane = threadIdx.x;
    int r = blockIdx.x * 64 + lane;
    const bool live = r < rows;
    if (!live) r = rows - 1;
    const LstmLane W = lstm_load(table, lane);
    float *ptr[4] = {hidden + (size_t)r * 8, cell + (size_t)r * 8, hidden + ((size_t)rows + r) * 8, cell + ((size_t)rows + r) * 8};
    LstmSplit st;
    float (*arr[4])[4] = {st.h0, st.c0, st.h1, st.c1};
#pragma unroll
    for (int a = 0; a < 4; a++) {
        float u[8];
#pragma unroll
        for (int i = 0; i < 8; i++) u[i] = ptr[a][i];
        lstm_split(u, arr[a][0], arr[a][1]);
    }
    float t = actuator_step_mfma(W, pos_err[r], vel[r], st);
#pragma unroll
    for (int a = 0; a < 4; a++) {
        float u[8];
        lstm_unsplit(arr[a][0], arr[a][1], u);
        if (live) {
#pragma unroll
            for (int i = 0; i < 8; i++) ptr[a][i] = u[i];
        }
    }
    if (live) torques[r] = t;
}

template <class T, bool HF, bool SC = false>
__global__ void __launch_bounds__(LG_BLOCK) k_physics(const KArgs A, const float *torques, int write_contacts) {
    constexpr int K = T::K, L = T::L, ND = K * L, NREP = T::NREP;
    const lg_buffers &B = A.B;
    __shared__ float lds_tab[T::K * Tab<T>::STRIDE];
    __shared__ SelfStore<SC, T> sc_store;
    if constexpr (SC) stage_base_points<T>(A, sc_store.get());
    stage_limb_table<T>(A, lds_tab);
    const int N = A.P.num_envs;
    const int tid = blockIdx.x * LG_BLOCK + threadIdx.x;
    int e = tid / K;
    const int k = tid % K;
    const bool live = e < N;
    if (!live) e = N - 1;
    const float *tab = lds_tab + k * Tab<T>::STRIDE;
    const int d0 = e * ND + k * L;
    float root[13], q[L], qd[L], tau[L], Frep[NREP][3], Fbase[3];
#pragma unroll
    for (int i = 0; i < 13; i++) root[i] = B.root_states[(size_t)e * 13 + i];
#pragma unroll
    for (int j = 0; j < L; j++) { q[j] = B.dof_state[2 * (d0 + j)]; qd[j] = B.dof_state[2 * (d0 + j) + 1]; tau[j] = torques[d0 + j]; }
    const float mu = 0.5f * ((B.friction_coeffs ? B.friction_coeffs[e] : 1.0f) + A.P.ground_friction);
    const float base_mass = A.base.mass + (B.base_mass_delta ? B.base_mass_delta[e] : 0.0f);
    {
        const float *cf = B.contact_forces + ((size_t)e * (1 + K * NREP) + 1 + k * NREP) * 3;
#pragma unroll
        for (int r = 0; r < NREP; r++) { Frep[r][0] = cf[3 * r]; Frep[r][1] = cf[3 * r + 1]; Frep[r][2] = cf[3 * r + 2]; }
        const float *c0 = B.contact_forces + (size_t)e * (1 + K * NREP) * 3;
        Fbase[0] = c0[0]; Fbase[1] = c0[1]; Fbase[2] = c0[2];
    }
    write_contacts = 1;
    physics_substep<T, HF, NoWait, false, SC>(A, tab, k, root, q, qd, tau, base_mass, mu, Frep, Fbase, NoWait(), nullptr, nullptr, nullptr, 0, sc_store.get(), true);
    if (!live) return;
#pragma unroll
    for (int j = 0; j < L; j++) { B.dof_state[2 * (d0 + j)] = q[j]; B.dof_state[2 * (d0 + j) + 1] = qd[j]; }
    if (write_contacts) {
        float *cf = B.contact_forces + ((size_t)e * (1 + K * NREP) + 1 + k * NREP) * 3;
#pragma unroll
        for (int r = 0; r < NREP; r++) { cf[3 * r] = Frep[r][0]; cf[3 * r + 1] = Frep[r][1]; cf[3 * r + 2] = Frep[r][2]; }
    }
    if (k == 0) {
#pragma unroll
        for (int i = 0; i < 13; i++) B.root_states[(size_t)e * 13 + i] = root[i];
        if (write_contacts) { float *c0 = B.contact_forces + (size_t)e * (1 + K * NREP) * 3; c0[0] = Fbase[0]; c0[1] = Fbase[1]; c0[2] = Fbase[2]; }
    }
}

template <class T>
__global__ void __launch_bounds__(LG_BLOCK) k_obs(const KArgs A) {
    constexpr int K = T::K, L = T::L, ND = K * L;
    const lg_buffers &B = A.B;
    __shared__ float lds_tab[T::K * Tab<T>::STRIDE];
    stage_limb_table<T>(A, lds_tab);
    const int N = A.P.num_envs;
    const int tid = blockIdx.x * LG_BLOCK + threadIdx.x;
    int e = tid / K;
    const int k = tid % K;
    const bool live = e < N;
    if (!live) e = N - 1;
    const float *tab = lds_tab + k * Tab<T>::STRIDE;
    const int d0 = e * ND + k * L;
    float root[13], q[L], qd[L], act[L], cmd[4];
#pragma unroll
    for (int i = 0; i < 13; i++) root[i] = B.root_states[(size_t)e * 13 + i];
#pragma unroll
    for (int j = 0; j < L; j++) { q[j] = B.dof_state[2 * (d0 + j)]; qd[j] = B.dof_state[2 * (d0 + j) + 1]; act[j] = B.actions[d0 + j]; }
#pragma unroll
    for (int i = 0; i < 4; i++) cmd[i] = B.commands[(size_t)e * 4 + i];
    V3 blv = v3(B.base_lin_vel[(size_t)e * 3], B.base_lin_vel[(size_t)e * 3 + 1], B.base_lin_vel[(size_t)e * 3 + 2]);
    V3 bav = v3(B.base_ang_vel[(size_t)e * 3], B.base_ang_vel[(size_t)e * 3 + 1], B.base_ang_vel[(size_t)e * 3 + 2]);
    V3 pg = v3(B.projected_gravity[(size_t)e * 3], B.projected_gravity[(size_t)e * 3 + 1], B.projected_gravity[(size_t)e * 3 + 2]);
    write_observations<T>(A, e, k, live, A.step, root, q, qd, act, tab, blv, bav, pg, cmd, true);
}

__global__ void __launch_bounds__(256) k_resample_reset(const KArgs A) {
    const lg_params &P = A.P; const lg_buffers &B = A.B;
    const int e = blockIdx.x * 256 + threadIdx.x;
    if (e >= P.num_envs || !B.reset_buf[e]) return;
    const double *xr = cmd_x_range(A);
    redraw_reset_command(A, xr ? (float)xr[0] : P.cmd_lin_vel_x[0], xr ? (float)xr[1] : P.cmd_lin_vel_x[1], e, A.step, B.obs_buf + (size_t)e * P.num_obs);
}

static thread_local char g_err[512] = "";
int lg::fail(int code, const char *fmt, const char *arg) { snprintf(g_err, sizeof g_err, fmt, arg); return code; }

enum RobotKind { ROBOT_ANYMAL = 0, ROBOT_CASSIE = 1 };

struct lg_sim {
    lg_params      P;
    lg_robot_model M;
    lg_buffers     B;
    BaseTab        base;
    RobotKind      kind;
    int            device;
    bool           has_net, bound;
    float         *d_limb_table;
    float         *d_weights;
    unsigned int  *d_done;
    float         *d_accum_alt;
    int            defer;
    unsigned long long *d_prof;
    int            num_cus;
    float         *d_roll_extras;
    unsigned int  *h_status;
    int            spin_limit, debug_skip;
};

template <class T> static int check_topology(const lg_robot_model *m) {
    if (m->num_limbs != T::K || m->chain_len != T::L) return 0;
    if (m->num_bodies != 1 + T::K * T::NREP || m->num_base_points < 1 || m->num_base_points > T::K) return 0;
    for (int i = 0; i < m->num_base_points; i++) if (m->base_points[i].report_body != 0) return 0;
    for (int k = 0; k < T::K; k++) {
        if (m->num_limb_points[k] != T::NPT) return 0;
        for (int i = 0; i < T::NPT; i++) {
            if (m->limb_points[k][i].joint != T::pt_joint(i)) return 0;
            if (m->limb_points[k][i].report_body != 1 + k * T::NREP + T::pt_rep(i)) return 0;
        }
        if (m->foot_body[k] != 1 + k * T::NREP + T::FOOT_REP) return 0;
    }
    return 1;
}

static void m3_mul(const double *A, const double *B, double *C) { for (int i = 0; i < 3; i++) for (int j = 0; j < 3; j++) C[3 * i + j] = A[3 * i] * B[j] + A[3 * i + 1] * B[3 + j] + A[3 * i + 2] * B[6 + j]; }
static void m3_tr(const double *A, double *B) { for (int i = 0; i < 3; i++) for (int j = 0; j < 3; j++) B[3 * i + j] = A[3 * j + i]; }
static void m3_vec(const double *A, const float *v, float *out) { for (int i = 0; i < 3; i++) out[i] = (float)(A[3 * i] * v[0] + A[3 * i + 1] * v[1] + A[3 * i + 2] * v[2]); }
static void m3_align_x(const float *a, double *Q) {
    double ax = a[0], ay = a[1], az = a[2], n = sqrt(ax * ax + ay * ay + az * az);
    ax /= n; ay /= n; az /= n;
    double bx, by, bz;
    if (fabs(ax) <= fabs(ay) && fabs(ax) <= fabs(az)) { bx = 0; by = -az; bz = ay; }
    else if (fabs(ay) <= fabs(az)) { bx = az; by = 0; bz = -ax; }
    else { bx = -ay; by = ax; bz = 0; }
    n = sqrt(bx * bx + by * by + bz * bz); bx /= n; by /= n; bz /= n;
    const double cx = ay * bz - az * by, cy = az * bx - ax * bz, cz = ax * by - ay * bx;
    Q[0] = ax; Q[1] = bx; Q[2] = cx; Q[3] = ay; Q[4] = by; Q[5] = cy; Q[6] = az; Q[7] = bz; Q[8] = cz;
    if (fabs(ax - 1.0) < 1e-12) { for (int i = 0; i < 9; i++) Q[i] = (i % 4 == 0) ? 1.0 : 0.0; }
}

template <class T> static void fill_limb_table(const lg_params &P, const lg_robot_model &M, float *t) {
    memset(t, 0, sizeof(float) * T::K * Tab<T>::STRIDE);
    for (int k = 0; k < T::K; k++) {
        float *tk = t + k * Tab<T>::STRIDE;
        double Q[T::L][9], Qpar[9] = {1, 0, 0, 0, 1, 0, 0, 0, 1};
        for (int j = 0; j < T::L; j++) {
            int d = k * T::L + j;
            float *tj = tk + j * LG_JS;
            m3_align_x(M.joint_axis[d], Q[j]);
            double QparT[9], QjT[9], Rf[9], tmp[9], Rnew[9];
            m3_tr(Qpar, QparT); m3_tr(Q[j], QjT);
            for (int i = 0; i < 9; i++) Rf[i] = M.joint_rot[d][i];
            m3_mul(QparT, Rf, tmp); m3_mul(tmp, Q[j], Rnew);
            m3_vec(QparT, M.joint_pos[d], tj + J_POS);
            for (int i = 0; i < 9; i++) tj[J_ROT + i] = (float)Rnew[i];
            tj[J_AXIS] = 1.0f; tj[J_AXIS + 1] = 0.0f; tj[J_AXIS + 2] = 0.0f;
            tj[J_MASS] = M.body_mass[d];
            m3_vec(QjT, M.body_com[d], tj + J_COM);
            {
                const float *I6 = M.body_inertia[d];
                double If[9] = {I6[0], I6[1], I6[2], I6[1], I6[3], I6[4], I6[2], I6[4], I6[5]}, T1[9], T2[9];
                m3_mul(QjT, If, T1); m3_mul(T1, Q[j], T2);
                tj[J_INERTIA] = (float)T2[0]; tj[J_INERTIA + 1] = (float)T2[1]; tj[J_INERTIA + 2] = (float)T2[2];
                tj[J_INERTIA + 3] = (float)T2[4]; tj[J_INERTIA + 4] = (float)T2[5]; tj[J_INERTIA + 5] = (float)T2[8];
            }
            tj[J_LO] = M.dof_lower[d]; tj[J_HI] = M.dof_upper[d]; tj[J_VLIM] = M.dof_vel_limit[d];
            tj[J_ARM] = M.dof_armature[d]; tj[J_DAMP] = M.dof_damping[d];
            tj[J_KP] = P.p_gains[d]; tj[J_KD] = P.d_gains[d]; tj[J_Q0] = P.default_dof_pos[d]; tj[J_TLIM] = P.torque_limits[d];
            tj[J_SLO] = P.soft_pos_lower[d]; tj[J_SHI] = P.soft_pos_upper[d]; tj[J_DVL] = P.dof_vel_limits[d];
            float sub = 0.0f;
            for (int jj = j; jj < T::L; jj++) sub += M.body_mass[k * T::L + jj];
            tj[J_SUBM] = sub;
            for (int i = 0; i < 9; i++) Qpar[i] = Q[j][i];
        }
        for (int i = 0; i < T::NPT; i++) {
            float *tp = tk + T::L * LG_JS + 4 * i;
            double QjT[9];
            m3_tr(Q[T::pt_joint(i)], QjT);
            m3_vec(QjT, M.limb_points[k][i].pos, tp); tp[3] = M.limb_points[k][i].radius;
        }
        for (int g = 0; g < T::NGRP; g++) {
            const float *a = M.limb_points[k][T::grp_c0(g)].pos, *b = M.limb_points[k][T::grp_c1(g)].pos;
            const float c[3] = {0.5f * (a[0] + b[0]), 0.5f * (a[1] + b[1]), 0.5f * (a[2] + b[2])};
            float R = 0.0f;
            for (int cap = 0; cap < T::NCAP; cap++) if (T::cap_grp(cap) == g)
                for (int e = 0; e < 2; e++) {
                    const lg_point &pt = M.limb_points[k][e ? T::cap_p1(cap) : T::cap_p0(cap)];
                    const float dx = pt.pos[0] - c[0], dy = pt.pos[1] - c[1], dz = pt.pos[2] - c[2];
                    R = fmaxf(R, sqrtf(dx * dx + dy * dy + dz * dz) + pt.radius);
                }
            tk[Tab<T>::GRP + g] = R * 1.0001f;
        }
        for (int c = 0; c < 4; c++) tk[Tab<T>::BPT + c] = 0.0f;
        if (k < M.num_base_points) { memcpy(tk + Tab<T>::BPT, M.base_points[k].pos, 12); tk[Tab<T>::BPT + 3] = M.base_points[k].radius; }
    }
}

template <class T> static int check_capsules(const lg_robot_model *m) {
    auto mergeable = [](const lg_point &a, const lg_point &b) { return a.joint == b.joint && a.radius == b.radius && a.report_body == b.report_body; };
    for (int k = 0; k < T::K; k++) {
        int next = 0;
        for (int c = 0; c < T::NCAP; c++) {
            const int p0 = T::cap_p0(c), p1 = T::cap_p1(c);
            if (p0 != next) return 0;
            if (p1 != p0 && !(p1 == p0 + 1 && mergeable(m->limb_points[k][p0], m->limb_points[k][p1]))) return 0;
            if (p1 == p0 && p0 + 1 < T::NPT && mergeable(m->limb_points[k][p0], m->limb_points[k][p0 + 1])) return 0;
            if (T::pt_joint(p0) != T::pt_joint(p1)) return 0;
            next = p1 + 1;
        }
        if (next != T::NPT) return 0;
    }
    for (int i = 0; i < m->num_base_points; i += 2)
        if (i + 1 < m->num_base_points && m->base_points[i].radius != m->base_points[i + 1].radius) return 0;
    return 1;
}

static void build_lstm_table(const float *w, float *t ) {
    const float *in_scale = w, *out_scale = w + 2, *Wih0 = w + 3, *Whh0 = Wih0 + 64, *bih0 = Whh0 + 256, *bhh0 = bih0 + 32;
    const float *Wih1 = bhh0 + 32, *Whh1 = Wih1 + 256, *bih1 = Whh1 + 256, *bhh1 = bih1 + 32, *lw = bhh1 + 32, *lb = lw + 8;
    for (int l = 0; l < 64; l++) {
        const int g = l & 31, hb = l >> 5;
        const double sc = (g >= 16 && g < 24) ? -2.0 * 1.4426950408889634 : -1.4426950408889634;
        auto S = [&](double v) { return (float)(sc * v); };
        t[LW_B0 * 64 + l] = hb ? 0.0f : S((double)bih0[g] + (double)bhh0[g]);
        t[LW_X * 64 + l] = S((double)Wih0[2 * g + hb] * in_scale[hb]);
        t[LW_B1 * 64 + l] = hb ? 0.0f : S((double)bih1[g] + (double)bhh1[g]);
        for (int s = 0; s < 4; s++) {
            t[(LW_H0 + s) * 64 + l] = S(Whh0[8 * g + s + 4 * hb]);
            t[(LW_I1 + s) * 64 + l] = S(Wih1[8 * g + s + 4 * hb]);
            t[(LW_H1 + s) * 64 + l] = S(Whh1[8 * g + s + 4 * hb]);
            t[(LW_LIN + s) * 64 + l] = lw[s + 4 * hb];
        }
        t[LW_LB * 64 + l] = lb[0];
        t[LW_OUT * 64 + l] = out_scale[0];
    }
}

static int upload_tables(lg_sim *s) {
    float host[LG_MAX_LIMBS * (LG_MAX_CHAIN * LG_JS + 4 * LG_MAX_LIMB_POINTS + 1)];
    size_t n;
    if (s->kind == ROBOT_ANYMAL) { fill_limb_table<AnymalTraits>(s->P, s->M, host); n = AnymalTraits::K * Tab<AnymalTraits>::STRIDE; }
    else { fill_limb_table<CassieTraits>(s->P, s->M, host); n = CassieTraits::K * Tab<CassieTraits>::STRIDE; }
    HIP_TRY(hipMemcpy(s->d_limb_table, host, n * sizeof(float), hipMemcpyHostToDevice));
    HIP_TRY(hipMemcpy(s->d_limb_table + LG_MAX_LIMBS * (LG_MAX_CHAIN * LG_JS + 4 * LG_MAX_LIMB_POINTS + 1), s->P.height_points, sizeof(float) * 2 * LG_MAX_HEIGHT_POINTS, hipMemcpyHostToDevice));
    s->base.mass = s->M.base_mass;
    memcpy(s->base.com, s->M.base_com, 12); memcpy(s->base.inertia, s->M.base_inertia, 24);
    memset(s->base.pts, 0, sizeof s->base.pts);
    s->base.num_pts = s->M.num_base_points;
    s->base.mass_robot = s->M.base_mass;
    for (int d = 0; d < s->M.num_limbs * s->M.chain_len; d++) s->base.mass_robot += s->M.body_mass[d];
    for (int i = 0; i < s->M.num_base_points; i++) { memcpy(s->base.pts[i], s->M.base_points[i].pos, 12); s->base.pts[i][3] = s->M.base_points[i].radius; }
    return 0;
}

static void fill_args(const lg_sim *s, KArgs &a, int64_t step) {
    a.P = s->P; a.B = s->B; a.base = s->base; a.limb_table = s->d_limb_table; a.hpts = s->d_limb_table + LG_MAX_LIMBS * (LG_MAX_CHAIN * LG_JS + 4 * LG_MAX_LIMB_POINTS + 1); a.weights = s->d_weights;
    a.actions_in = nullptr; a.env_ids = nullptr; a.count = 0; a.step = step; memset(&a.pol, 0, sizeof a.pol);
    a.penalised_mask = s->M.penalised_mask; a.termination_mask = s->M.termination_mask; a.done_counter = s->d_done; a.prof = s->d_prof;
    a.accum_alt = s->d_accum_alt; a.defer = s->defer; a.flush_parts = 0;
    a.status = s->h_status; a.spin_limit = s->spin_limit; a.debug_skip = s->debug_skip;
    memset(&a.roll, 0, sizeof a.roll);
}
static void fill_post_args(KArgs &a) {
    const lg_params &P = a.P; const lg_buffers &B = a.B;
    memset(&a.post, 0, sizeof a.post);
    PostHead &h = a.post.head;
    h.resample_interval = P.resample_interval; h.heading_command = P.heading_command; h.push_interval = P.push_interval;
    h.max_episode_length = P.max_episode_length; h.max_push_vel = P.max_push_vel; h.termination_mask = a.termination_mask;
    h.penalised_mask = a.penalised_mask;
    h.episode_length_buf = B.episode_length_buf; h.commands = B.commands; h.contact_forces = B.contact_forces;
    PostRew &r = a.post.rew;
    r.dt_policy = P.dt_policy; r.soft_dof_vel_limit = P.soft_dof_vel_limit; r.soft_torque_limit = P.soft_torque_limit;
    r.max_contact_force = P.max_contact_force; r.base_height_target = P.base_height_target; r.tracking_sigma = P.tracking_sigma;
    r.only_positive_rewards = P.only_positive_rewards; r.num_height_points = P.num_height_points; r.terrain_curriculum = P.terrain_curriculum;
    for (int t = 0; t < LG_NUM_REWARD_TERMS; t++) { r.reward_scale[t] = P.reward_scale[t]; if (P.reward_slot[t] >= 0) r.slot_mask |= 1u << t; }
    r.last_actions = B.last_actions; r.feet_air_time = B.feet_air_time; r.last_contacts = B.last_contacts; r.env_origins = B.env_origins;
    PostObs &o = a.post.obs;
    o.obs_scale_lin_vel = P.obs_scale_lin_vel; o.obs_scale_ang_vel = P.obs_scale_ang_vel; o.obs_scale_dof_pos = P.obs_scale_dof_pos;
    o.obs_scale_dof_vel = P.obs_scale_dof_vel; o.noise_lin_vel = P.noise_lin_vel; o.noise_ang_vel = P.noise_ang_vel; o.noise_gravity = P.noise_gravity;
    o.noise_dof_pos = P.noise_dof_pos; o.noise_dof_vel = P.noise_dof_vel; o.clip_observations = P.clip_observations;
    o.add_noise = P.add_noise; o.num_obs = P.num_obs; o.num_envs = P.num_envs; o.roll_obs = a.roll.obs;
    PostStore &w = a.post.store;
    w.dof_state = B.dof_state; w.actions = B.actions; w.torques = B.torques; w.last_actions = B.last_actions; w.last_dof_vel = B.last_dof_vel;
    w.feet_air_time = B.feet_air_time; w.last_contacts = B.last_contacts; w.root_states = B.root_states;
    PostStoreEnv &v = a.post.store_env;
    v.last_root_vel = B.last_root_vel;
    v.commands = B.commands; v.base_lin_vel = B.base_lin_vel; v.base_ang_vel = B.base_ang_vel; v.projected_gravity = B.projected_gravity;
    v.rew_buf = B.rew_buf; v.reset_buf = B.reset_buf; v.time_out_buf = B.time_out_buf; v.episode_length_buf = B.episode_length_buf;
    v.roll_rew = a.roll.rew; v.roll_done = a.roll.done; v.roll_time_outs = a.roll.time_outs;
}
static int status_error(const lg_sim *s) {
    const unsigned int st = s->h_status ? __atomic_load_n(s->h_status, __ATOMIC_RELAXED) : 0u;
    if (!st) return 0;
    static thread_local char text[160];
    snprintf(text, sizeof text, "0x%x%s%s", st, (st & LG_STATUS_FRAME_HANDOVER_TIMEOUT) ? " frame hand-over poll timed out" : "",
             (st & LG_STATUS_SELF_COLLISION_TIMEOUT) ? " self-collision hand-over poll timed out" : "");
    return fail(-20, "device status %s: an earlier launch on this handle ran with a missed LDS hand-over -- its physics is invalid (lg_clear_device_status() after re-initialising the state)", text);
}
static int entry_check(const lg_sim *s) { return (!s || !s->bound) ? fail(-8, "lg_bind has not been called") : status_error(s); }
template <class T> static int grid_for(int n_env_like) { return (n_env_like * T::K + LG_BLOCK - 1) / LG_BLOCK; }
static int step_grid(const lg_sim *s) { return s->kind == ROBOT_ANYMAL ? grid_for<AnymalTraits>(s->P.num_envs) : grid_for<CassieTraits>(s->P.num_envs); }
static int step_waves(const lg_sim *s) {
    if (s->kind == ROBOT_ANYMAL && s->P.control_type == LG_CTRL_ACTUATOR_NET) return LG_STEP_WAVES;
    return step_grid(s) <= s->num_cus ? 4 : (step_grid(s) <= 2 * s->num_cus ? 2 : 1);
}
static bool fused_actor_ok(const lg_sim *s, const lg_policy *p) {
    const bool flat_actor = p->tiles[0] == 3 && p->tiles[1] == 8 && p->tiles[2] == 4 && p->tiles[3] == 2 && p->dims[4] == s->M.num_limbs * s->M.chain_len;
    return s->kind == ROBOT_ANYMAL && s->P.control_type == LG_CTRL_ACTUATOR_NET && s->P.terrain_type != LG_TERRAIN_HEIGHTFIELD && flat_actor &&
           p->dims[0] == s->P.num_obs;
}

int lg::launch_policy_act_flat(const PolicyArgs &A, void *stream) {
    hipLaunchKernelGGL((k_policy_act<3, 8, 4, 2>), dim3((A.num_envs + 15) / 16), dim3(64 * LG_POLICY_WAVES), 0, (hipStream_t)stream, A);
    return (int)hipGetLastError();
}

extern "C" {

const char *lg_last_error(void) { return g_err; }
int lg_abi_version(void) { return LG_ABI_VERSION; }
#ifdef LG_PROFILE
int lg_debug_profile(lg_sim *s, unsigned long long *out16 , int reset) {
    if (!s || !s->d_prof) return -1;
    if (hipDeviceSynchronize() != hipSuccess) return -2;
    std::vector<unsigned long long> h(LG_NPROF_TOTAL);
    if (hipMemcpy(h.data(), s->d_prof, sizeof(unsigned long long) * LG_NPROF_TOTAL, hipMemcpyDeviceToHost) != hipSuccess) return -2;
    for (int i = 0; i < LG_NPROF; i++) out16[i] = 0;
    for (int b = 0; b < LG_NPROF_BLOCKS; b++) {
        const unsigned long long *a = h.data() + LG_NPROF + (size_t)b * 40;
        for (int i = 0; i < 16; i++) out16[i] += a[i];
        if (a[16] > out16[16]) out16[16] = a[16];
    }
    if (reset && hipMemset(s->d_prof, 0, sizeof(unsigned long long) * LG_NPROF_TOTAL) != hipSuccess) return -2;
    return 0;
}
int lg_debug_profile_blocks(lg_sim *s, unsigned long long *out, int blocks) {
    if (!s || !s->d_prof || blocks < 0 || blocks > LG_NPROF_BLOCKS) return -1;
    if (hipDeviceSynchronize() != hipSuccess) return -2;
    for (int b = 0; b < blocks; b++)
        if (hipMemcpy(out + (size_t)b * 20, s->d_prof + LG_NPROF + (size_t)b * 40 + 20, sizeof(unsigned long long) * 20, hipMemcpyDeviceToHost) != hipSuccess) return -2;
    return 0;
}
int lg_debug_profile_roll(lg_sim *s, unsigned long long *out) {
    if (!s || !s->d_prof) return -1;
    if (hipDeviceSynchronize() != hipSuccess) return -2;
    if (hipMemcpy(out, s->d_prof + LG_NPROF + (size_t)LG_NPROF_BLOCKS * 40, sizeof(unsigned long long) * LG_NPROF_ROLL * LG_NPROF_BLOCKS, hipMemcpyDeviceToHost) != hipSuccess) return -2;
    return 0;
}
#endif
int lg_sizeof(int which) {
    switch (which) { case 0: return (int)sizeof(lg_params); case 1: return (int)sizeof(lg_robot_model);
                     case 2: return (int)sizeof(lg_buffers); case 3: return (int)sizeof(lg_point);
                     case 4: return (int)sizeof(lg_mlp_net); case 5: return (int)sizeof(lg_adam_tensor);
                     case 6: return (int)sizeof(lg_rollout_step); case 7: return (int)sizeof(lg_ppo_batch); default: return -1; }
}

int lg_create(const lg_params *params, const lg_robot_model *model, const float *actuator_weights, int device_id, lg_sim **out) {
    if (!params || !model || !out) return fail(-1, "null argument");
    if (params->abi_version != LG_ABI_VERSION) return fail(-3, "ABI version mismatch");
    static_assert(LG_NUM_REWARD_TERMS + 1 <= 64, "k_extras uses one wave");
    static_assert(sizeof(KArgs) <= 4096, "kernel arguments must fit the 4 KiB kernarg segment");
    RobotKind kind;
    if (check_topology<AnymalTraits>(model)) kind = ROBOT_ANYMAL;
    else if (check_topology<CassieTraits>(model)) kind = ROBOT_CASSIE;
    else return fail(-4, "robot topology is not one of the compiled-in layouts (ANYmal-C 4x3, Cassie 2x6)");
    if (params->control_type == LG_CTRL_ACTUATOR_NET && !actuator_weights) return fail(-2, "actuator-net control without weights");
    if (params->control_type == LG_CTRL_ACTUATOR_NET && kind != ROBOT_ANYMAL) return fail(-2, "actuator net is compiled for the ANYmal layout only");
    if (params->self_collision && kind != ROBOT_ANYMAL) return fail(-4, "self-collision (asset.self_collisions = 0) is compiled for the quadruped layouts only");
    if (params->self_collision && !check_capsules<AnymalTraits>(model)) return fail(-4, "collision points do not form the compiled-in capsule layout (self-collision)");
    if (params->cmd_curriculum && (params->max_episode_length < 1 || params->cmd_curriculum_slot >= params->num_reward_slots))
        return fail(-2, "commands.curriculum needs max_episode_length >= 1 and the tracking reward's slot (or -1)");
    HIP_TRY(hipSetDevice(device_id));
    lg_sim *s = new (std::nothrow) lg_sim();
    if (!s) return fail(-5, "out of host memory");
    s->P = *params; s->M = *model; s->kind = kind; s->device = device_id; s->bound = false;
    s->has_net = actuator_weights != nullptr; s->d_weights = nullptr; s->d_limb_table = nullptr; s->d_done = nullptr; s->d_prof = nullptr; s->d_accum_alt = nullptr; s->defer = 0;
    s->h_status = nullptr; s->spin_limit = 1 << 22; s->debug_skip = 0; s->d_roll_extras = nullptr;
    if (hipHostMalloc(reinterpret_cast<void **>(&s->h_status), sizeof(unsigned int), hipHostMallocMapped) != hipSuccess) { lg_destroy(s); return fail(-10, "hipHostMalloc failed"); }
    *s->h_status = 0u;
    if (hipMalloc(&s->d_accum_alt, (LG_NUM_REWARD_TERMS + 2) * sizeof(float)) != hipSuccess || hipMemset(s->d_accum_alt, 0, (LG_NUM_REWARD_TERMS + 2) * sizeof(float)) != hipSuccess) { lg_destroy(s); return fail(-10, "hipMalloc failed"); }
    {
        const size_t n_done = 1 + 2 * (((size_t)params->num_envs * 4 + LG_BLOCK - 1) / LG_BLOCK);
        if (hipMalloc(&s->d_done, n_done * sizeof(unsigned int)) != hipSuccess || hipMemset(s->d_done, 0, n_done * sizeof(unsigned int)) != hipSuccess) { lg_destroy(s); return fail(-10, "hipMalloc failed"); }
    }
    memset(&s->B, 0, sizeof s->B);
    { hipDeviceProp_t prop; s->num_cus = (hipGetDeviceProperties(&prop, device_id) == hipSuccess && prop.multiProcessorCount > 0) ? prop.multiProcessorCount : 256; }
#ifdef LG_PROFILE
    if (hipMalloc(&s->d_prof, sizeof(unsigned long long) * LG_NPROF_TOTAL) != hipSuccess || hipMemset(s->d_prof, 0, sizeof(unsigned long long) * LG_NPROF_TOTAL) != hipSuccess) { lg_destroy(s); return fail(-10, "hipMalloc failed"); }
#endif
    if (hipMalloc(&s->d_limb_table, sizeof(float) * (LG_MAX_LIMBS * (LG_MAX_CHAIN * LG_JS + 4 * LG_MAX_LIMB_POINTS + 1) + 2 * LG_MAX_HEIGHT_POINTS)) != hipSuccess) { lg_destroy(s); return fail(-10, "hipMalloc failed"); }
    if (s->has_net) {
        float table[LW_ROWS * 64];
        build_lstm_table(actuator_weights, table);
        if (hipMalloc(&s->d_weights, sizeof table) != hipSuccess) { lg_destroy(s); return fail(-10, "hipMalloc failed"); }
        if (hipMemcpy(s->d_weights, table, sizeof table, hipMemcpyHostToDevice) != hipSuccess) { lg_destroy(s); return fail(-10, "hipMemcpy failed"); }
    }
    int rc = upload_tables(s);
    if (rc) { lg_destroy(s); return rc; }
    *out = s;
    return 0;
}

void lg_destroy(lg_sim *s) {
    if (!s) return;
    if (s->d_limb_table) (void)hipFree(s->d_limb_table);
    if (s->d_weights) (void)hipFree(s->d_weights);
    if (s->d_done) (void)hipFree(s->d_done);
    if (s->d_accum_alt) (void)hipFree(s->d_accum_alt);
    if (s->d_prof) (void)hipFree(s->d_prof);
    if (s->h_status) (void)hipHostFree(s->h_status);
    if (s->d_roll_extras) (void)hipFree(s->d_roll_extras);
    delete s;
}

int lg_bind(lg_sim *s, const lg_buffers *b) {
    if (!s || !b) return fail(-1, "null argument");
    const void *need[] = {b->root_states, b->dof_state, b->contact_forces, b->obs_buf, b->rew_buf, b->reset_buf, b->time_out_buf,
                          b->episode_length_buf, b->torques, b->actions, b->last_actions, b->last_dof_vel, b->last_root_vel, b->commands,
                          b->feet_air_time, b->last_contacts, b->base_lin_vel, b->base_ang_vel, b->projected_gravity, b->episode_sums,
                          b->episode_means, b->extras_accum, b->env_origins};
    for (size_t i = 0; i < sizeof need / sizeof *need; i++) if (!need[i]) return fail(-6, "a required buffer pointer is null");
    if (s->P.control_type == LG_CTRL_ACTUATOR_NET && (!b->sea_hidden_state || !b->sea_cell_state)) return fail(-6, "actuator state buffers missing");
    if (s->P.measure_heights && !b->measured_heights) return fail(-6, "measured_heights buffer missing");
    if (s->P.terrain_type == LG_TERRAIN_HEIGHTFIELD && !b->height_samples) return fail(-6, "height_samples missing");
    if (s->P.terrain_type == LG_TERRAIN_HEIGHTFIELD && (s->P.hf_rows < 2 || s->P.hf_cols < 2 || (int64_t)s->P.hf_rows * s->P.hf_cols > 0x7fffffff))
        return fail(-6, "height field must have 2 <= rows, cols and rows*cols < 2^31");
    if (s->P.terrain_curriculum && (!b->terrain_levels || !b->terrain_types || !b->terrain_origins)) return fail(-6, "terrain curriculum buffers missing");
    if (s->P.cmd_curriculum && !b->cmd_range) return fail(-6, "commands.curriculum needs the cmd_range buffer");
    s->B = *b; s->bound = true;
    return 0;
}

int lg_set_obs_buffer(lg_sim *s, float *obs_buf) {
    if (!s || !obs_buf) return fail(-1, "null argument");
    s->B.obs_buf = obs_buf;
    return 0;
}

int lg_set_params(lg_sim *s, const lg_params *p) {
    if (!s || !p) return fail(-1, "null argument");
    if (p->num_envs != s->P.num_envs || p->control_type != s->P.control_type) return fail(-7, "num_envs / control_type cannot change after create");
    if (p->cmd_curriculum && (p->max_episode_length < 1 || p->cmd_curriculum_slot >= p->num_reward_slots || (s->bound && !s->B.cmd_range)))
        return fail(-2, "commands.curriculum needs max_episode_length >= 1, the tracking reward's slot (or -1) and the cmd_range buffer");
    s->P = *p;
    return upload_tables(s);
}

#define LAUNCH_NW(TRAITS, HFV, SCV)                                                                                              \
    { if (nw == 4) hipLaunchKernelGGL((k_step<TRAITS, false, HFV, false, 4, SCV>), g, dim3(4 * LG_BLOCK), 0, st, a);             \
      else if (nw == 2) hipLaunchKernelGGL((k_step<TRAITS, false, HFV, false, 2, SCV>), g, dim3(2 * LG_BLOCK), 0, st, a);        \
      else hipLaunchKernelGGL((k_step<TRAITS, false, HFV, false, 1, SCV>), g, dim3(LG_BLOCK), 0, st, a); }

int lg_step(lg_sim *s, const float *actions, int64_t common_step_counter, void *stream) {
    if (int rc = entry_check(s)) return rc;
    if (!actions) return fail(-1, "null actions");
    if (common_step_counter < 0 && !s->B.step_counter) return fail(-9, "common_step_counter = -1 needs a step_counter buffer");
    KArgs a; fill_args(s, a, common_step_counter); a.actions_in = actions;
    hipStream_t st = (hipStream_t)stream;
    const bool hf = s->P.terrain_type == LG_TERRAIN_HEIGHTFIELD;
    const bool net = s->P.control_type == LG_CTRL_ACTUATOR_NET;
    const dim3 g(step_grid(s)), b(LG_STEP_WAVES * LG_BLOCK);
    const int nw = step_waves(s);
    if (s->kind == ROBOT_ANYMAL) {
        const bool sc = s->P.self_collision != 0;
        if (net && !hf) { if (sc) hipLaunchKernelGGL((k_step<AnymalTraits, true, false, false, 4, true>), g, b, 0, st, a);
                          else hipLaunchKernelGGL((k_step<AnymalTraits, true, false>), g, b, 0, st, a); }
        else if (net && hf) { if (sc) hipLaunchKernelGGL((k_step<AnymalTraits, true, true, false, 4, true>), g, b, 0, st, a);
                              else hipLaunchKernelGGL((k_step<AnymalTraits, true, true>), g, b, 0, st, a); }
        else if (!hf) { if (sc) LAUNCH_NW(AnymalTraits, false, true) else LAUNCH_NW(AnymalTraits, false, false) }
        else { if (sc) LAUNCH_NW(AnymalTraits, true, true) else LAUNCH_NW(AnymalTraits, true, false) }
    } else {
        if (!hf) LAUNCH_NW(CassieTraits, false, false)
        else LAUNCH_NW(CassieTraits, true, false)
    }
    HIP_TRY(hipGetLastError());
    return 0;
}

int lg_step_policy(lg_sim *s, lg_policy *p, const float *obs, float *actions, float *mean, uint64_t seed, int32_t deterministic,
                   int64_t common_step_counter, void *stream) {
    if (int rc = entry_check(s)) return rc;
    if (!p || !obs || !actions) return fail(-1, "null argument");
    if (common_step_counter < 0 && !s->B.step_counter) return fail(-9, "common_step_counter = -1 needs a step_counter buffer");
    if (!fused_actor_ok(s, p))
        return fail(-4, "the fused policy step is compiled for the 48-128-64-32 actor on the quadruped actuator-net plane kernel; use lg_policy_act + lg_step");
    KArgs a; fill_args(s, a, common_step_counter); a.actions_in = nullptr;
    fill_policy_args(p, a.pol, obs, actions, mean, s->P.num_envs, seed, common_step_counter, s->B.step_counter, deterministic);
    const dim3 g(step_grid(s)), b(LG_STEP_WAVES * LG_BLOCK);
    if (s->P.self_collision) hipLaunchKernelGGL((k_step<AnymalTraits, true, false, true, 4, true>), g, b, 0, (hipStream_t)stream, a);
    else hipLaunchKernelGGL((k_step<AnymalTraits, true, false, true>), g, b, 0, (hipStream_t)stream, a);
    HIP_TRY(hipGetLastError());
    return 0;
}

int lg_rollout_policy(lg_sim *s, lg_policy *p, const lg_rollout_buffers *r, uint64_t seed, int32_t deterministic, int64_t common_step_counter, void *stream) {
    if (int rc = entry_check(s)) return rc;
    if (!p || !r || !r->obs || !r->actions || !r->rew || !r->dones || !r->time_outs) return fail(-1, "null argument");
    if (r->steps < 1 || r->steps > LG_MAX_ROLL_STEPS) return fail(-1, "steps must be in [1, LG_MAX_ROLL_STEPS]");
    if (common_step_counter < 0 && !s->B.step_counter) return fail(-9, "common_step_counter = -1 needs a step_counter buffer");
    if (!fused_actor_ok(s, p) || s->P.measure_heights)
        return fail(-4, "the multi-step rollout kernel is compiled for the 48-128-64-32 actor on the quadruped actuator-net plane kernel; use lg_step_policy / lg_policy_act + lg_step");
    hipStream_t st = (hipStream_t)stream;
    const int stride = LG_NUM_REWARD_TERMS + 2;
    if (!s->d_roll_extras) {
        hipStreamCaptureStatus cap = hipStreamCaptureStatusNone;
        (void)hipStreamIsCapturing(st, &cap);
        if (cap != hipStreamCaptureStatusNone) return fail(-9, "first lg_rollout_policy call on a handle allocates its workspace: make one call outside stream capture");
        HIP_TRY(hipSetDevice(s->device));
        if (hipMalloc(&s->d_roll_extras, sizeof(float) * (LG_MAX_ROLL_STEPS * stride + 1)) != hipSuccess) return fail(-10, "hipMalloc failed");
        HIP_TRY(hipMemset(s->d_roll_extras, 0, sizeof(float) * (LG_MAX_ROLL_STEPS * stride + 1)));
    }
    KArgs a; fill_args(s, a, common_step_counter); a.actions_in = nullptr; a.defer = 0;
    fill_policy_args(p, a.pol, r->obs, r->actions, r->mean, s->P.num_envs, seed, common_step_counter, s->B.step_counter, deterministic);
    a.roll.steps = r->steps; a.roll.obs = r->obs; a.roll.actions = r->actions; a.roll.mean = r->mean; a.roll.rew = r->rew;
    a.roll.done = r->dones; a.roll.time_outs = r->time_outs; a.roll.extras = s->d_roll_extras;
    a.roll.obs0 = r->obs0;
    a.roll.cursor = reinterpret_cast<int *>(s->d_roll_extras + LG_MAX_ROLL_STEPS * stride);
    fill_post_args(a);
    const int launches = s->P.cmd_curriculum ? 1 + (r->steps + s->P.max_episode_length - 1) / s->P.max_episode_length : 1;
    const dim3 g(step_grid(s)), b(LG_STEP_WAVES * LG_BLOCK);
    for (int i = 0; i < launches; i++) {
        a.roll.sub = i;
        if (s->P.self_collision) hipLaunchKernelGGL((k_step<AnymalTraits, true, false, true, 4, true, true>), g, b, 0, st, a);
        else hipLaunchKernelGGL((k_step<AnymalTraits, true, false, true, 4, false, true>), g, b, 0, st, a);
        HIP_TRY(hipGetLastError());
    }
    return 0;
}

int lg_reset_idx(lg_sim *s, const int32_t *env_ids, int32_t count, int64_t common_step_counter, void *stream) {
    if (int rc = entry_check(s)) return rc;
    if (count <= 0) return 0;
    if (!env_ids) return fail(-1, "null env_ids");
    KArgs a; fill_args(s, a, common_step_counter); a.env_ids = env_ids; a.count = count;
    hipStream_t st = (hipStream_t)stream;
    const bool net = s->P.control_type == LG_CTRL_ACTUATOR_NET;
    if (s->kind == ROBOT_ANYMAL) {
        dim3 g(grid_for<AnymalTraits>(count)), b(LG_BLOCK);
        if (net) hipLaunchKernelGGL((k_reset<AnymalTraits, true>), g, b, 0, st, a);
        else hipLaunchKernelGGL((k_reset<AnymalTraits, false>), g, b, 0, st, a);
    } else {
        dim3 g(grid_for<CassieTraits>(count)), b(LG_BLOCK);
        hipLaunchKernelGGL((k_reset<CassieTraits, false>), g, b, 0, st, a);
    }
    hipLaunchKernelGGL(k_extras, dim3(1), dim3(64), 0, st, a);
    HIP_TRY(hipGetLastError());
    return 0;
}

int lg_device_status(lg_sim *s, int32_t synchronize) {
    if (!s) return fail(-1, "null argument");
    if (synchronize) { HIP_TRY(hipSetDevice(s->device)); HIP_TRY(hipDeviceSynchronize()); }
    const unsigned int st = __atomic_load_n(s->h_status, __ATOMIC_RELAXED);
    if (st) (void)status_error(s);
    return (int)(st & 0x7fffffffu);
}
int lg_clear_device_status(lg_sim *s) {
    if (!s) return fail(-1, "null argument");
    HIP_TRY(hipSetDevice(s->device)); HIP_TRY(hipDeviceSynchronize());
    __atomic_store_n(s->h_status, 0u, __ATOMIC_RELAXED);
    return 0;
}
int lg_debug_handover(lg_sim *s, int32_t skip, int32_t spin_limit) {
    if (!s) return fail(-1, "null argument");
    if (skip < 0 || skip > 2) return fail(-1, "skip must be 0 (off), 1 (frame flag) or 2 (self-collision flags)");
    s->debug_skip = skip; s->spin_limit = spin_limit > 0 ? spin_limit : (1 << 22);
    return 0;
}

int lg_set_deferred_extras(lg_sim *s, int32_t on) {
    if (!s) return fail(-1, "null argument");
    s->defer = on ? 1 : 0;
    return 0;
}

int lg_extras_flush(lg_sim *s, int64_t common_step_counter, void *stream) {
    if (int rc = entry_check(s)) return rc;
    KArgs a; fill_args(s, a, common_step_counter);
    a.flush_parts = (step_waves(s) > 1 && s->P.terrain_curriculum && s->B.terrain_levels) ? step_grid(s) : 0;
// ... 54 lines not shown
```

### legged_games_gym_amd/csrc/lg_policy.h

```cpp
#pragma once
#include "lg_device.h"

namespace lg {

typedef float f32x4 __attribute__((ext_vector_type(4)));

LG_DEV float elu1(float x) { return x > 0.0f ? x : (__builtin_amdgcn_exp2f(1.442695041f * x) - 1.0f); }

#define LG_POLICY_WAVES 4
template <int IN_T, int OUT_T, bool ACT>
LG_DEV void mlp_layer(const float *__restrict__ w , const float *__restrict__ b ,
                      const float4 (*xin)[64], float4 (*xout)[64], int wave, int lane) {
    constexpr int CH = IN_T > 16 ? 16 : IN_T;
#pragma unroll 1
    for (int o = wave; o < OUT_T; o += LG_POLICY_WAVES) {
        f32x4 acc;
#pragma unroll
        for (int r = 0; r < 4; r++) acc[r] = b[(o * 4 + r) * 64 + lane];
        const float *wo = w + (size_t)o * IN_T * 4 * 64 + lane;
#pragma unroll
        for (int t0 = 0; t0 < IN_T; t0 += CH) {
            float wr[CH * 4];
#pragma unroll
            for (int i = 0; i < CH * 4; i++) wr[i] = (t0 * 4 + i < IN_T * 4) ? wo[(t0 * 4 + i) * 64] : 0.0f;
            __builtin_amdgcn_sched_barrier(0);
#pragma unroll
            for (int t = 0; t < CH; t++) {
                if (t0 + t < IN_T) {
                    const float4 xv = xin[t0 + t][lane];
                    acc = __builtin_amdgcn_mfma_f32_16x16x4f32(wr[t * 4 + 0], xv.x, acc, 0, 0, 0);
                    acc = __builtin_amdgcn_mfma_f32_16x16x4f32(wr[t * 4 + 1], xv.y, acc, 0, 0, 0);
                    acc = __builtin_amdgcn_mfma_f32_16x16x4f32(wr[t * 4 + 2], xv.z, acc, 0, 0, 0);
                    acc = __builtin_amdgcn_mfma_f32_16x16x4f32(wr[t * 4 + 3], xv.w, acc, 0, 0, 0);
                }
            }
        }
        xout[o][lane] = ACT ? make_float4(elu1(acc[0]), elu1(acc[1]), elu1(acc[2]), elu1(acc[3])) : make_float4(acc[0], acc[1], acc[2], acc[3]);
    }
}

template <int IN_T> struct TileW {
    float w[IN_T * 4], b[4];
    LG_DEV void load(const float *__restrict__ wp, const float *__restrict__ bp, int o, int lane) {
#pragma unroll
        for (int i = 0; i < IN_T * 4; i++) w[i] = wp[((size_t)o * IN_T * 4 + i) * 64 + lane];
#pragma unroll
        for (int r = 0; r < 4; r++) b[r] = bp[(o * 4 + r) * 64 + lane];
    }
    template <bool ACT> LG_DEV float4 run(const float4 (*xin)[64], int lane) const {
        f32x4 acc = {b[0], b[1], b[2], b[3]};
#pragma unroll
        for (int t = 0; t < IN_T; t++) {
            const float4 xv = xin[t][lane];
            acc = __builtin_amdgcn_mfma_f32_16x16x4f32(w[t * 4 + 0], xv.x, acc, 0, 0, 0);
            acc = __builtin_amdgcn_mfma_f32_16x16x4f32(w[t * 4 + 1], xv.y, acc, 0, 0, 0);
            acc = __builtin_amdgcn_mfma_f32_16x16x4f32(w[t * 4 + 2], xv.z, acc, 0, 0, 0);
            acc = __builtin_amdgcn_mfma_f32_16x16x4f32(w[t * 4 + 3], xv.w, acc, 0, 0, 0);
        }
        return ACT ? make_float4(elu1(acc[0]), elu1(acc[1]), elu1(acc[2]), elu1(acc[3])) : make_float4(acc[0], acc[1], acc[2], acc[3]);
    }
};

struct PolicyArgs {
    const float *obs;
    const float *w[4];
    const float *b[4];
    const float *std;
    float *actions;
    float *mean;
    const int64_t *step_counter;
    int64_t step;
    uint64_t seed;
    int32_t num_envs, num_obs, num_actions, deterministic;
};

template <int D0T, int D1T, int D2T, int D3T>
LG_DEV void policy_forward(const PolicyArgs &A, float4 (*xa)[64], float4 (*xb)[64], float4 (*xy)[64], int block, int wave, int lane,
                           int64_t step, float (*lds_act)[16], const float (*lds_obs)[48] = nullptr ) {
    const int g = lane >> 4;
    int env = block * 16 + (lane & 15);
    const bool live = env < A.num_envs;
    if (!live) env = A.num_envs - 1;
    constexpr bool PRELOAD = D0T <= 4 && D1T == 2 * LG_POLICY_WAVES && D2T == LG_POLICY_WAVES && D3T == 2;
    TileW<PRELOAD ? D0T : 1> w0a, w0b;
    TileW<PRELOAD ? D1T : 1> w1;
    TileW<PRELOAD ? D2T : 1> w2;
    TileW<PRELOAD ? D3T : 1> w3;
    if constexpr (PRELOAD) {
        w0a.load(A.w[0], A.b[0], wave, lane); w0b.load(A.w[0], A.b[0], wave + LG_POLICY_WAVES, lane);
        w1.load(A.w[1], A.b[1], wave, lane);
        if (wave < D3T) w2.load(A.w[2], A.b[2], wave, lane);
        if (wave == 0) w3.load(A.w[3], A.b[3], 0, lane);
    }
    const float *o = A.obs + (size_t)env * A.num_obs;
    for (int t = wave; t < D0T; t += LG_POLICY_WAVES) {
        float v[4];
#pragma unroll
        for (int r = 0; r < 4; r++) { int k = 16 * t + 4 * g + r; v[r] = k < A.num_obs ? (lds_obs ? lds_obs[lane & 15][k] : o[k]) : 0.0f; }
        xa[t][lane] = make_float4(v[0], v[1], v[2], v[3]);
    }
    __syncthreads();
    if constexpr (PRELOAD) {
        xb[wave][lane] = w0a.template run<true>(xa, lane);
        xb[wave + LG_POLICY_WAVES][lane] = w0b.template run<true>(xa, lane);
    } else mlp_layer<D0T, D1T, true>(A.w[0], A.b[0], xa, xb, wave, lane);
    __syncthreads();
    if constexpr (PRELOAD) xa[wave][lane] = w1.template run<true>(xb, lane);
    else mlp_layer<D1T, D2T, true>(A.w[1], A.b[1], xb, xa, wave, lane);
    __syncthreads();
    if constexpr (PRELOAD) { if (wave < D3T) xb[wave][lane] = w2.template run<true>(xa, lane); }
    else mlp_layer<D2T, D3T, true>(A.w[2], A.b[2], xa, xb, wave, lane);
    if (wave == LG_POLICY_WAVES - 1) {
        float u[4];
        rand4(A.seed ^ 0x9E3779B97F4A7C15ull, env, step, 100 + g, 0, u);
        float rad0 = sqrtf(-2.0f * __logf(fmaxf(u[0], 1e-12f))), rad1 = sqrtf(-2.0f * __logf(fmaxf(u[2], 1e-12f)));
        float s0, c0, s1, c1;
        __sincosf(6.2831853f * u[1], &s0, &c0);
        __sincosf(6.2831853f * u[3], &s1, &c1);
        const float eps[4] = {rad0 * c0, rad0 * s0, rad1 * c1, rad1 * s1};
        float ns[4];
#pragma unroll
        for (int r = 0; r < 4; r++) { const int a = 4 * g + r; ns[r] = (a < A.num_actions && !A.deterministic) ? A.std[a] * eps[r] : 0.0f; }
        xy[0][lane] = make_float4(ns[0], ns[1], ns[2], ns[3]);
    }
    __syncthreads();
    if (wave != 0) return;
    const float4 nv = xy[0][lane];
    const float ns[4] = {nv.x, nv.y, nv.z, nv.w};
    if constexpr (PRELOAD) xy[0][lane] = w3.template run<false>(xb, lane);
    else mlp_layer<D3T, 1, false>(A.w[3], A.b[3], xb, xy, 0, lane);
    const float4 yv = xy[0][lane];
    const float y[4] = {yv.x, yv.y, yv.z, yv.w};
#pragma unroll
    for (int r = 0; r < 4; r++) {
        int a = 4 * g + r;
        if (a < A.num_actions) {
            float m = y[r], act = m + ns[r];
            if (lds_act) lds_act[a][lane & 15] = act;
            if (live) {
                if (A.mean) A.mean[(size_t)env * A.num_actions + a] = m;
                A.actions[(size_t)env * A.num_actions + a] = act;
            }
        }
    }
}

template <int D0T, int D1T, int D2T, int D3T>
__global__ void __launch_bounds__(64 * LG_POLICY_WAVES) k_policy_act(const PolicyArgs A) {
    constexpr int TA = D0T > D2T ? D0T : D2T, TB = D1T > D3T ? D1T : D3T;
    __shared__ float4 xa[TA][64], xb[TB][64], xy[1][64];
    const int64_t step = A.step >= 0 ? A.step : (A.step_counter ? A.step_counter[0] + 1 : 0);
    policy_forward<D0T, D1T, D2T, D3T>(A, xa, xb, xy, blockIdx.x, threadIdx.x >> 6, threadIdx.x & 63, step, nullptr);
}

typedef __bf16 bf16x8g __attribute__((ext_vector_type(8)));
typedef float f32x16p __attribute__((ext_vector_type(16)));
#define LG_PW_ENVS 32
#define LG_PW_WAVES 8
#define LG_PW_INFLIGHT 32

struct PolicyWideArgs {
    PolicyArgs base;
    const bf16x8g *wb[4];
    const float *bb[4];
};

LG_DEV void split8(const float (&v)[8], bf16x8g &hi, bf16x8g &lo) {
#pragma unroll
    for (int i = 0; i < 8; i++) { hi[i] = (__bf16)v[i]; lo[i] = (__bf16)(v[i] - (float)hi[i]); }
}

template <int KS, int TPW> struct WideStream {
    static constexpr int PF = (LG_PW_INFLIGHT / (2 * TPW) + 1) < KS + 1 ? (LG_PW_INFLIGHT / (2 * TPW) + 1) : KS + 1;
    bf16x8g wh[PF][TPW], wl[PF][TPW];
    LG_DEV void fetch(const bf16x8g *__restrict__ w, int o0, int rot, int lane, int s) {
        int sr = s + rot; sr = sr >= KS ? sr - KS : sr;
#pragma unroll
        for (int t = 0; t < TPW; t++) {
            const bf16x8g *q = w + ((size_t)((o0 + t) * KS + sr) * 2) * 64 + lane;
            wh[s % PF][t] = q[0]; wl[s % PF][t] = q[64];
        }
    }
    LG_DEV void prime(const bf16x8g *__restrict__ w, int o0, int rot, int lane) {
#pragma unroll
        for (int s = 0; s < PF - 1; s++) if (s < KS) fetch(w, o0, rot, lane, s);
    }
    LG_DEV void run(const bf16x8g *__restrict__ w, const bf16x8g (*xin)[2][64], int o0, int rot, int lane, f32x16p (&acc)[TPW]) {
#pragma unroll
        for (int t = 0; t < TPW; t++)
#pragma unroll
            for (int i = 0; i < 16; i++) acc[t][i] = 0.0f;
#pragma unroll
        for (int s = 0; s < KS; s++) {
            if (s + PF - 1 < KS) fetch(w, o0, rot, lane, s + PF - 1);
            int sr = s + rot; sr = sr >= KS ? sr - KS : sr;
            const bf16x8g bh = xin[sr][0][lane], bl = xin[sr][1][lane];
#pragma unroll
            for (int t = 0; t < TPW; t++) {
                acc[t] = __builtin_amdgcn_mfma_f32_32x32x16_bf16(wl[s % PF][t], bh, acc[t], 0, 0, 0);
                acc[t] = __builtin_amdgcn_mfma_f32_32x32x16_bf16(wh[s % PF][t], bl, acc[t], 0, 0, 0);
                acc[t] = __builtin_amdgcn_mfma_f32_32x32x16_bf16(wh[s % PF][t], bh, acc[t], 0, 0, 0);
            }
        }
    }
};

template <int TPW>
LG_DEV void wide_epilogue(const f32x16p (&acc)[TPW], const float *__restrict__ b, bf16x8g (*xout)[2][64], int o0, int lane) {
    const int h = lane >> 5;
#pragma unroll
    for (int t = 0; t < TPW; t++) {
        const float *bo = b + 32 * (o0 + t) + 4 * h;
#pragma unroll
        for (int jj = 0; jj < 2; jj++) {
            float v[8];
#pragma unroll
            for (int i = 0; i < 8; i++) v[i] = elu1(acc[t][8 * jj + i] + bo[8 * (2 * jj + (i >> 2)) + (i & 3)]);
            bf16x8g hi, lo;
            split8(v, hi, lo);
            xout[2 * (o0 + t) + jj][0][lane] = hi; xout[2 * (o0 + t) + jj][1][lane] = lo;
        }
    }
}

#ifdef LG_CHAIN_PROF
__device__ unsigned long long g_chain_prof[2048 * 16];
#define CHAIN_STAMP(i) do { if (threadIdx.x == 0 && blockIdx.y == 0) g_chain_prof[blockIdx.x * 16 + (i)] = __builtin_amdgcn_s_memtime(); } while (0)
#else
#define CHAIN_STAMP(i) do { } while (0)
#endif
struct WideNoTap {
    LG_DEV void operator()(const PolicyArgs &, int, int, int, bool, const float (&)[8]) const {}
};
struct WideObsCopy {
    float *dst;
    LG_DEV void operator()(const PolicyArgs &A, int env, int s, int h, bool live, const float (&v)[8]) const {
        if (dst && live) {
#pragma unroll
            for (int i = 0; i < 8; i++) { const int k = 16 * s + 8 * h + i; if (k < A.num_obs) dst[(size_t)env * A.num_obs + k] = v[i]; }
        }
    }
};
struct WideActStores {
    LG_DEV void operator()(const PolicyArgs &A, int env, int h, bool live, const f32x16p &y, const float (&by)[2][4], const float (&ns)[2][4]) const {
#pragma unroll
        for (int ii = 0; ii < 2; ii++) {
            const int g = 2 * ii + h;
#pragma unroll
            for (int r = 0; r < 4; r++) {
                const int a = 4 * g + r;
                if (a < A.num_actions && live) {
                    const float m = y[4 * ii + r] + by[ii][r];
                    if (A.mean) A.mean[(size_t)env * A.num_actions + a] = m;
                    A.actions[(size_t)env * A.num_actions + a] = m + ns[ii][r];
                }
            }
        }
    }
};

template <int K0S, int H1T, int H2T, int H3T, class Idx, class Tap, class Epilogue>
LG_DEV void wide_actor_body(const PolicyWideArgs &W, const Idx blk, bf16x8g (*xa)[2][64], bf16x8g (*xb)[2][64], const Tap &tap, const Epilogue &epilogue) {
    const PolicyArgs &A = W.base;
    constexpr int NW = LG_PW_WAVES;
    static_assert(H1T % NW == 0 && (H2T % NW == 0 || H2T <= NW) && H3T <= NW, "tiles per wave");
    constexpr int T1 = H1T / NW, T2 = H2T >= NW ? H2T / NW : 1, T3 = 1;
    const int wave = threadIdx.x >> 6, lane = threadIdx.x & 63, h = lane >> 5;
    const int wv = (wave + blk) % NW;
    const int r0 = (blk * 5) % K0S, r1 = (blk * 5) % (2 * H1T), r2 = (blk * 5) % (2 * H2T);
    const bool on2 = wv * T2 < H2T, on3 = wv * T3 < H3T;
    CHAIN_STAMP(0);
    const int64_t step = A.step >= 0 ? A.step : (A.step_counter ? A.step_counter[0] + 1 : 0);
    int env = blk * LG_PW_ENVS + (lane & 31);
    const bool live = env < A.num_envs;
    if (!live) env = A.num_envs - 1;
    const float *o = A.obs + (size_t)env * A.num_obs;
    WideStream<K0S, T1> s1;
    s1.prime(W.wb[0], wv * T1, r0, lane);
    for (int s = wave; s < K0S; s += NW) {
        float v[8];
#pragma unroll
        for (int i = 0; i < 8; i++) { const int k = 16 * s + 8 * h + i; v[i] = k < A.num_obs ? o[k] : 0.0f; }
        tap(A, env, s, h, live, v);
        bf16x8g hi, lo;
        split8(v, hi, lo);
        xa[s][0][lane] = hi; xa[s][1][lane] = lo;
    }
    float ns[2][4], by[2][4];
    if (wave == 0) {
#pragma unroll
        for (int ii = 0; ii < 2; ii++) {
            const int g = 2 * ii + h;
#pragma unroll
            for (int r = 0; r < 4; r++) { ns[ii][r] = 0.0f; by[ii][r] = 0.0f; }
            if (4 * g >= A.num_actions) continue;
            float u[4];
            rand4(A.seed ^ 0x9E3779B97F4A7C15ull, env, step, 100 + g, 0, u);
            const float rad0 = sqrtf(-2.0f * __logf(fmaxf(u[0], 1e-12f))), rad1 = sqrtf(-2.0f * __logf(fmaxf(u[2], 1e-12f)));
            float s0, c0, sn1, c1;
            __sincosf(6.2831853f * u[1], &s0, &c0);
            __sincosf(6.2831853f * u[3], &sn1, &c1);
            const float eps[4] = {rad0 * c0, rad0 * s0, rad1 * c1, rad1 * sn1};
#pragma unroll
            for (int r = 0; r < 4; r++) {
                const int a = 4 * g + r;
                if (a < A.num_actions) { by[ii][r] = W.bb[3][a]; ns[ii][r] = A.deterministic ? 0.0f : A.std[a] * eps[r]; }
            }
        }
    }
    __syncthreads();
    CHAIN_STAMP(1);
    f32x16p a1[T1];
    s1.run(W.wb[0], xa, wv * T1, r0, lane, a1);
    CHAIN_STAMP(2);
    WideStream<2 * H1T, T2> s2;
    if (on2) s2.prime(W.wb[1], wv * T2, r1, lane);
    __builtin_amdgcn_sched_barrier(0);
    wide_epilogue<T1>(a1, W.bb[0], xb, wv * T1, lane);
    CHAIN_STAMP(3);
    __syncthreads();
    CHAIN_STAMP(4);
    f32x16p a2[T2];
    WideStream<2 * H2T, T3> s3;
    if (on2) s2.run(W.wb[1], xb, wv * T2, r1, lane, a2);
    CHAIN_STAMP(5);
    if (on3) s3.prime(W.wb[2], wv * T3, r2, lane);
    __builtin_amdgcn_sched_barrier(0);
    if (on2) wide_epilogue<T2>(a2, W.bb[1], xa, wv * T2, lane);
    __syncthreads();
    CHAIN_STAMP(6);
    f32x16p a3[T3];
    WideStream<2 * H3T, 1> s4;
    if (on3) s3.run(W.wb[2], xa, wv * T3, r2, lane, a3);
    if (wave == 0) s4.prime(W.wb[3], 0, 0, lane);
    __builtin_amdgcn_sched_barrier(0);
    if (on3) wide_epilogue<T3>(a3, W.bb[2], xb, wv * T3, lane);
    __syncthreads();
    CHAIN_STAMP(7);
    if (wave != 0) return;
    f32x16p y[1];
    s4.run(W.wb[3], xb, 0, 0, lane, y);
    CHAIN_STAMP(8);
    epilogue(A, env, h, live, y[0], by, ns);
    CHAIN_STAMP(9);
}

template <int K0S, int H1T, int H2T, int H3T>
__global__ void __launch_bounds__(64 * LG_PW_WAVES) k_policy_act_wide(const PolicyWideArgs W) {
    constexpr int KA = K0S > 2 * H2T ? K0S : 2 * H2T, KB = H1T > H3T ? 2 * H1T : 2 * H3T;
    __shared__ bf16x8g xa[KA][2][64], xb[KB][2][64];
    wide_actor_body<K0S, H1T, H2T, H3T>(W, blockIdx.x, xa, xb, WideNoTap{}, WideActStores{});
}

struct ChainNet {
    const float *x; int ldx, num_in;
    const bf16x8g *wb[4]; const float *bb[4];
    float *act[3]; int lda[3];
    float *out; int out_dim;
};
struct ChainArgs { ChainNet net[2]; int mb; };

#define LG_CHAIN_INFLIGHT 32
template <int KS, int KTOT> struct WideStream2 {
    static constexpr int PF = (LG_CHAIN_INFLIGHT / 2 + 1) < KS + 1 ? (LG_CHAIN_INFLIGHT / 2 + 1) : KS + 1;
    bf16x8g wh[PF], wl[PF];
    LG_DEV void fetch(const bf16x8g *__restrict__ w, int tile, int k0, int rot, int lane, int s) {
        int sr = s + rot; sr = sr >= KS ? sr - KS : sr;
        const bf16x8g *q = w + ((size_t)(tile * KTOT + k0 + sr) * 2) * 64 + lane;
        wh[s % PF] = q[0]; wl[s % PF] = q[64];
    }
    LG_DEV void prime(const bf16x8g *__restrict__ w, int tile, int k0, int rot, int lane) {
#pragma unroll
        for (int s = 0; s < PF - 1; s++) if (s < KS) fetch(w, tile, k0, rot, lane, s);
    }
    LG_DEV void run(const bf16x8g *__restrict__ w, const bf16x8g (*xin)[2][2][64], int tile, int k0, int rot, int lane, f32x16p (&acc)[2], bool zero) {
        if (zero) {
#pragma unroll
            for (int i = 0; i < 16; i++) { acc[0][i] = 0.0f; acc[1][i] = 0.0f; }
        }
#pragma unroll
        for (int s = 0; s < KS; s++) {
            if (s + PF - 1 < KS) fetch(w, tile, k0, rot, lane, s + PF - 1);
            int sr = s + rot; sr = sr >= KS ? sr - KS : sr;
            const bf16x8g bh0 = xin[sr][0][0][lane], bl0 = xin[sr][0][1][lane], bh1 = xin[sr][1][0][lane], bl1 = xin[sr][1][1][lane];
            acc[0] = __builtin_amdgcn_mfma_f32_32x32x16_bf16(wl[s % PF], bh0, acc[0], 0, 0, 0);
            acc[1] = __builtin_amdgcn_mfma_f32_32x32x16_bf16(wl[s % PF], bh1, acc[1], 0, 0, 0);
            acc[0] = __builtin_amdgcn_mfma_f32_32x32x16_bf16(wh[s % PF], bl0, acc[0], 0, 0, 0);
            acc[1] = __builtin_amdgcn_mfma_f32_32x32x16_bf16(wh[s % PF], bl1, acc[1], 0, 0, 0);
            acc[0] = __builtin_amdgcn_mfma_f32_32x32x16_bf16(wh[s % PF], bh0, acc[0], 0, 0, 0);
            acc[1] = __builtin_amdgcn_mfma_f32_32x32x16_bf16(wh[s % PF], bh1, acc[1], 0, 0, 0);
        }
    }
};
struct ChainBias { float4 q[4]; };
LG_DEV ChainBias chain_bias(const float *__restrict__ b, int tile_g, int lane) {
    const float4 *bo = reinterpret_cast<const float4 *>(b + 32 * tile_g + 4 * (lane >> 5));
    ChainBias r;
#pragma unroll
    for (int c = 0; c < 4; c++) r.q[c] = bo[2 * c];
    return r;
}
LG_DEV void chain_epilogue2(const f32x16p (&acc)[2], const ChainBias &B, bf16x8g (*xout)[2][2][64], int tile_g, int tile_l, int lane,
                            float *__restrict__ act0, float *__restrict__ act1 ) {
    const int h = lane >> 5;
    const float bo[16] = {B.q[0].x, B.q[0].y, B.q[0].z, B.q[0].w, B.q[1].x, B.q[1].y, B.q[1].z, B.q[1].w,
                          B.q[2].x, B.q[2].y, B.q[2].z, B.q[2].w, B.q[3].x, B.q[3].y, B.q[3].z, B.q[3].w};
#pragma unroll
    for (int hf = 0; hf < 2; hf++) {
        float *act_row = hf ? act1 : act0;
#pragma unroll
        for (int jj = 0; jj < 2; jj++) {
            float v[8];
#pragma unroll
            for (int i = 0; i < 8; i++) v[i] = elu1(acc[hf][8 * jj + i] + bo[4 * (2 * jj + (i >> 2)) + (i & 3)]);
            if (act_row) {
                float *dst = act_row + 32 * tile_g + 16 * jj + 4 * h;
                *reinterpret_cast<float4 *>(dst) = make_float4(v[0], v[1], v[2], v[3]);
                *reinterpret_cast<float4 *>(dst + 8) = make_float4(v[4], v[5], v[6], v[7]);
            }
            bf16x8g hi, lo;
            split8(v, hi, lo);
            xout[2 * tile_l + jj][hf][0][lane] = hi; xout[2 * tile_l + jj][hf][1][lane] = lo;
        }
    }
}

template <int K0S>
__global__ void __launch_bounds__(64 * LG_PW_WAVES) k_mlp_chain_fwd64(const ChainArgs C) {
    static_assert(LG_PW_WAVES == 8 && K0S <= 16, "one layer-1 tile per wave; x0 fits the 16 k-step buffer");
    const ChainNet &N = C.net[blockIdx.y];
    __shared__ bf16x8g bufA[16][2][2][64], bufB[16][2][2][64];
    const int wave = threadIdx.x >> 6, lane = threadIdx.x & 63, h = lane >> 5;
    const int wv = (wave + blockIdx.x) & 7;
    const int r0 = (blockIdx.x * 5) % K0S, r1 = (blockIdx.x * 5) & 15, r2 = (blockIdx.x * 3) & 15;
    int row[2]; bool live[2];
#pragma unroll
    for (int hf = 0; hf < 2; hf++) {
        row[hf] = blockIdx.x * 64 + 32 * hf + (lane & 31);
        live[hf] = row[hf] < C.mb;
        if (!live[hf]) row[hf] = C.mb - 1;
    }
    auto arow = [&](int l, int hf) -> float * { return live[hf] ? N.act[l] + (size_t)row[hf] * N.lda[l] : nullptr; };
    CHAIN_STAMP(0);
    constexpr int NX = (2 * K0S + LG_PW_WAVES - 1) / LG_PW_WAVES;
    float4 xv[NX][2];
#pragma unroll
    for (int j = 0; j < NX; j++) {
        const int s = min(wave + LG_PW_WAVES * j, 2 * K0S - 1), ks = s >> 1, hf = s & 1, k0 = 16 * ks + 8 * h;
// ... 109 lines not shown
```

Measured before the change: 76.94 million env-steps/s.

## Run next-step actor MLP on helper waves overlapped with physics wave in rollout

In the persistent rollout kernel, the policy forward pass for step rt+1 moves from all waves at the start of each step onto the three helper waves. It runs as an MFMA actor split across those waves, with weights held in registers, while wave 0 does physics and post-processing for step rt. Wave 0 and the helpers synchronise through matched s_barrier calls, and the actions are handed over in LDS. This is meant to remove the serialized policy phase from the critical path. The cost is a complex barrier protocol with more VGPR pressure, and barrier-count mismatches between waves could deadlock the kernel.

```diff
diff --git a/legged_games_gym_amd/csrc/lg_kernels.hip b/legged_games_gym_amd/csrc/lg_kernels.hip
--- a/legged_games_gym_amd/csrc/lg_kernels.hip
+++ b/legged_games_gym_amd/csrc/lg_kernels.hip
@@ -66,14 +66,14 @@
 struct PostHead {
     int32_t  resample_interval, heading_command, push_interval, max_episode_length;
     float    max_push_vel; uint32_t termination_mask, penalised_mask, _pad0;
-    int64_t *episode_length_buf; float *commands, *contact_forces; uint32_t _pad[2];
+    int64_t *episode_length_buf; float *commands, *contact_forces, *env_origins;
 };
 struct PostRew {
     float    dt_policy, soft_dof_vel_limit, soft_torque_limit, max_contact_force, base_height_target, tracking_sigma;
     int32_t  only_positive_rewards; uint32_t slot_mask ; int32_t num_height_points, terrain_curriculum;
     float   *last_actions, *feet_air_time; uint8_t *last_contacts;
     float    reward_scale[LG_NUM_REWARD_TERMS];
-    float   *env_origins; uint32_t _pad[2];
+    uint32_t _pad[4];
 };
 struct PostObs {
     float    obs_scale_lin_vel, obs_scale_ang_vel, obs_scale_dof_pos, obs_scale_dof_vel;
@@ -126,6 +126,8 @@
     } else return A;
 }
 
+LG_DEV void roll_barrier() { asm volatile("s_waitcnt lgkmcnt(0)\n\ts_barrier" ::: "memory"); }
+
 typedef uint32_t lg_u32x16 __attribute__((ext_vector_type(16)));
 typedef uint32_t lg_u32x8 __attribute__((ext_vector_type(8)));
 template <class S> struct KargFetch {
@@ -214,7 +216,8 @@
 #define LG_PROF_COUNT(f, cond)
 #endif
 enum { PF_PROLOGUE = 0, PF_TORQUE, PF_KINEMATICS, PF_INWARD, PF_BASE, PF_OUTWARD, PF_INTEGRATE, PF_POST, PF_EXTRAS,
-       PF_POST_HEIGHTS, PF_POST_TERMS, PF_POST_REWARD, PF_POST_RESET, PF_POST_OBS };
+       PF_POST_HEIGHTS, PF_POST_TERMS, PF_POST_REWARD, PF_POST_RESET, PF_POST_OBS,
+       PF_WAIT_ACTIONS = PF_POST_RESET };
 
 struct HfFetch { int16_t s00, s10, s01, s11; float tx, ty; };
 template <bool HF> LG_DEV HfFetch hf_fetch(const KArgs &A, float x, float y) {
@@ -1426,13 +1429,33 @@
     }
 };
 
+struct RollIter {
+    int rt;
+    const int *s_roll;
+    float4 (*xa)[64], (*xb)[64], (*xy)[64];
+    float (*lds_act)[16];
+    const float (*lds_obs)[48];
+    LG_DEV bool phys() const { return rt >= s_roll[0]; }
+    LG_DEV bool next() const { return rt + 1 < s_roll[1]; }
+    LG_DEV PolicyArgs actor_args(const KArgs &A) const {
+        PolicyArgs pa = A.pol;
+        const size_t N = A.P.num_envs, ND = A.pol.num_actions;
+        pa.obs = (rt + 1 == 0 && A.roll.obs0) ? A.roll.obs0 : A.roll.obs + (size_t)(rt + 1) * N * A.P.num_obs;
+        pa.actions = A.roll.actions + (size_t)(rt + 1) * N * ND;
+        pa.mean = A.roll.mean ? A.roll.mean + (size_t)(rt + 1) * N * ND : nullptr;
+        return pa;
+    }
+};
+
 template <class T, bool NET, bool HF, int NW, bool SC = false> struct HelperWave {
     static constexpr bool OFF = NW >= 2;
+    template <bool RL = false >
     static LG_DEV void run(const KArgs &A, int wave, int lane, int e, int k, int d0, bool live, int64_t step, const float *tab,
                            float2 (*lds_x)[LG_BLOCK], float (*lds_tau)[LG_BLOCK], StepSharedT<OFF, T::L, HF> &sh, SelfLds<T> *sc = nullptr,
                            const float *lds_tab = nullptr, ResetRand<T> *reset_rand = nullptr, int *s_last = nullptr, float4 (*hnoise)[LG_BLOCK] = nullptr,
                            int sub0 = 0 , float *roll_accum = nullptr ,
-                           bool tick_step = false ) {
+                           bool tick_step = false ,
+                           const RollIter *ri = nullptr ) {
         const lg_buffers &B = A.B;
         const lg_params &P = A.P;
         const int j = wave - 1;
@@ -1441,7 +1464,7 @@
         float (*part[4])[4] = {st.h0, st.c0, st.h1, st.c1};
         float *row[4] = {nullptr, nullptr, nullptr, nullptr};
         LstmLane LW;
-        if (NET) {
+        if (NET && (!RL || ri->phys())) {
             const size_t plane = (size_t)P.num_envs * (T::K * T::L);
             LW = lstm_load(A.weights, lane);
             row[0] = B.sea_hidden_state + (size_t)(d0 + j) * 8; row[1] = B.sea_cell_state + (size_t)(d0 + j) * 8;
@@ -1453,7 +1476,7 @@
                 lstm_split(u, part[a][0], part[a][1]);
             }
         }
-        if (NET || OFF) {
+        if ((NET || OFF) && (!RL || ri->phys())) {
             for (int it = 0; it < P.decimation; it++) {
                 __syncthreads();
                 float tau_j = 0.0f;
@@ -1490,8 +1513,8 @@
                 }
             }
         }
-        reset_rand->draw(P, e, k, step, lane, wave - 1, NW - 1);
-        if (P.measure_heights && P.add_noise) {
+        if (!RL || ri->phys()) reset_rand->draw(P, e, k, step, lane, wave - 1, NW - 1);
+        if (!RL && P.measure_heights && P.add_noise) {
             const int nchunk = (P.num_height_points + 3) >> 2;
 #pragma unroll
             for (int b = 0; b < HeightCrew<T, NW>::NCH; b++) {
@@ -1503,7 +1526,7 @@
                 }
             }
         }
-        if (NET) {
+        if (NET && (!RL || ri->phys())) {
 #pragma unroll
             for (int a = 0; a < 4; a++) {
                 float u[8];
@@ -1513,6 +1536,41 @@
                     reinterpret_cast<float4 *>(row[a])[1] = make_float4(u[4], u[5], u[6], u[7]);
                 }
             }
+        }
+        if constexpr (RL) {
+            const int h = wave - 1;
+            const bool phys = ri->phys(), next = ri->next();
+            const PolicyArgs pa = ri->actor_args(A);
+            HelperActor actor;
+            if (next) actor.request(pa, h, lane);
+            if (phys) {
+                roll_barrier();
+                roll_barrier();
+            }
+            const bool keeper = wave == 1 && live && k == 0;
+            EpisodeSums es;
+            if (phys && keeper) es.load(A, e);
+            if (next) actor.layer0(pa, phys ? ri->lds_obs : nullptr, ri->xb, blockIdx.x, h, lane);
+            roll_barrier();
+            if (next) actor.layer1(ri->xb, ri->xa, h, lane);
+            roll_barrier();
+            if (next) actor.layer2(pa, ri->xa, ri->xb, ri->xy, blockIdx.x, h, lane, step + 1);
+            roll_barrier();
+            if (next && h == 1) actor.output(pa, ri->xb, ri->xy, blockIdx.x, lane, ri->lds_act);
+            if (phys) {
+                if (wave == 1) es.template update<T::K>(A, e, lane, sh, keeper, A.roll.extras + (size_t)ri->rt * (LG_NUM_REWARD_TERMS + 2));
+                if (missed && lane == 0) lg_report(A.status, LG_STATUS_FRAME_HANDOVER_TIMEOUT);
+                const bool reset = sh.rst[lane] != 0 && live;
+                if (NET && __ballot(reset) != 0 && reset) {
+#pragma unroll
+                    for (int a = 0; a < 4; a++) {
+                        reinterpret_cast<float4 *>(row[a])[0] = make_float4(0.0f, 0.0f, 0.0f, 0.0f);
+                        reinterpret_cast<float4 *>(row[a])[1] = make_float4(0.0f, 0.0f, 0.0f, 0.0f);
+                    }
+                }
+            }
+            roll_barrier();
+            return;
         }
         __syncthreads();
         HeightCrew<T, NW> hc;
@@ -1564,6 +1622,31 @@
                     reinterpret_cast<float4 *>(row[a])[1] = make_float4(0.0f, 0.0f, 0.0f, 0.0f);
                 }
             }
+        }
+    }
+    static LG_DEV void roll(const KArgs &A_launch, int64_t step0, float2 (*lds_x)[LG_BLOCK], float (*lds_tau)[LG_BLOCK], StepSharedT<OFF, T::L, HF> &sh,
+                            SelfLds<T> *sc, const float *lds_tab, ResetRand<T> *reset_rand, float4 (*hnoise)[LG_BLOCK], float4 (*xa)[64], float4 (*xb)[64],
+                            float4 (*xy)[64], float (*lds_act)[16], const float (*lds_obs)[48], const int *s_roll) {
+        constexpr int K = T::K, L = T::L, ND = K * L;
+#pragma unroll 1
+        for (int rt = s_roll[0] - 1; rt < s_roll[1]; rt++) {
+            const KArgs &A = step_args<true>(A_launch);
+            const lg_params &P = A.P;
+            const int N = P.num_envs;
+            int tix = threadIdx.x;
+            asm volatile("" : "+v"(tix));
+            const int lane = tix % LG_BLOCK, wave = __builtin_amdgcn_readfirstlane(tix / LG_BLOCK);
+            int e = (blockIdx.x * LG_BLOCK + lane) / K;
+            const int k = (blockIdx.x * LG_BLOCK + lane) % K;
+            const bool live = e < N;
+            if (!live) e = N - 1;
+            const float *tab = lds_tab + k * Tab<T>::STRIDE;
+            const int d0 = e * ND + k * L;
+            const int64_t step = step0 + rt;
+            RollIter ri;
+            ri.rt = rt; ri.s_roll = s_roll;
+            ri.xa = xa; ri.xb = xb; ri.xy = xy; ri.lds_act = lds_act; ri.lds_obs = lds_obs;
+            run<true>(A, wave, lane, e, k, d0, live, step, tab, lds_x, lds_tau, sh, sc, lds_tab, reset_rand, nullptr, hnoise, rt * P.decimation, nullptr, false, &ri);
         }
     }
 };
@@ -1637,7 +1720,7 @@
     const int N = P.num_envs;
     int tix = threadIdx.x;
     if constexpr (ROLL) asm volatile("" : "+v"(tix));
-    const int wave = tix / LG_BLOCK, lane = tix % LG_BLOCK;
+    const int wave = ROLL ? 0 : tix / LG_BLOCK, lane = tix % LG_BLOCK;
     int e = e_wg;
     const int k = ROLL ? (blockIdx.x * LG_BLOCK + lane) % K : k_wg;
     if constexpr (ROLL) { e = (blockIdx.x * LG_BLOCK + lane) / K; if (e >= N) e = N - 1; }
@@ -1645,26 +1728,14 @@
     int d0 = e * ND + k * L;
     const int64_t step = step0 + rt;
     const int sub0 = ROLL ? rt * P.decimation : 0;
-    float *const roll_accum = ROLL ? A.roll.extras + (size_t)rt * (LG_NUM_REWARD_TERMS + 2) : nullptr;
+    float *const roll_accum = nullptr;
     float *const roll_obs_out = nullptr;
 
-    if (POL) {
-        if (ROLL) {
-            PolicyArgs pa = A.pol;
-            pa.obs = A.roll.obs + (size_t)rt * N * P.num_obs;
-            if (rt == 0 && A.roll.obs0) {
-                pa.obs = A.roll.obs0;
-                const size_t row0 = (size_t)blockIdx.x * 16 * P.num_obs;
-                const int n = min(16, N - (int)blockIdx.x * 16) * P.num_obs;
-                for (int i = tix; i < n; i += NW * LG_BLOCK) A.roll.obs[row0 + i] = A.roll.obs0[row0 + i];
-            }
-            pa.actions = A.roll.actions + (size_t)rt * N * ND;
-            pa.mean = A.roll.mean ? A.roll.mean + (size_t)rt * N * ND : nullptr;
-            policy_forward<3, 8, 4, 2>(pa, pol_xa, pol_xb, pol_xy, blockIdx.x, wave, lane, step, lds_act, rt > s_roll[0] ? lds_obs : nullptr);
-        } else policy_forward<3, 8, 4, 2>(A.pol, pol_xa, pol_xb, pol_xy, blockIdx.x, wave, lane, step, lds_act);
+    if (POL && !ROLL) {
+        policy_forward<3, 8, 4, 2>(A.pol, pol_xa, pol_xb, pol_xy, blockIdx.x, wave, lane, step, lds_act);
         __syncthreads();
     }
-    if (wave > 0) {
+    if (!ROLL && wave > 0) {
         HelperWave<T, NET, HF, NW, SC>::run(A, wave, lane, e, k, d0, live, step, tab, lds_x, lds_tau, sh, sc_store.get(), lds_tab, &reset_rand, &s_last, hnoise, sub0, roll_accum,
                                             !ROLL && curriculum_tick_step(A, step));
     } else {
@@ -1675,8 +1746,10 @@
     for (int j = 0; j < L; j++) {
         float2 s = reinterpret_cast<const float2 *>(B.dof_state)[d0 + j];
         q[j] = s.x; qd[j] = s.y;
+        if constexpr (!ROLL) {
         float a = POL ? lds_act[k * L + j][lane / K] : A.actions_in[d0 + j];
         act[j] = fminf(fmaxf(a, -P.clip_actions), P.clip_actions);
+        }
         tau[j] = 0.0f;
     }
     const float mu = 0.5f * ((B.friction_coeffs ? B.friction_coeffs[e] : 1.0f) + P.ground_friction);
@@ -1700,6 +1773,14 @@
         for (int j = 0; j < L; j++) tau[j] = B.torques[d0 + j];
     }
     LG_PROF(PF_PROLOGUE);
+    volatile int *fk_ready = &sh.fk_ready;
+    if constexpr (ROLL) asm volatile("" : "+s"(fk_ready));
+    if constexpr (ROLL) {
+        roll_barrier();
+#pragma unroll
+        for (int j = 0; j < L; j++) act[j] = fminf(fmaxf(lds_act[k * L + j][lane / K], -P.clip_actions), P.clip_actions);
+        LG_PROF(PF_WAIT_ACTIONS);
+    }
 #pragma unroll 1
     for (int it = 0; it < P.decimation; it++) {
         if (!NET) pd_torques<L>(P, tab, act, q, qd, B.last_dof_vel + d0, tau);
@@ -1717,7 +1798,7 @@
                 }
             };
             constexpr bool LEAN = NW == LG_STEP_WAVES && L <= 3 && !HF;
-            physics_substep<T, HF, decltype(join), OFF, SC, LEAN, ROLL>(A, tab, k, root, q, qd, tau, base_mass, mu, Frep, Fbase, join, sh.bt, sh.fk, &sh.fk_ready, sub0 + it + 1,
+            physics_substep<T, HF, decltype(join), OFF, SC, LEAN, ROLL>(A, tab, k, root, q, qd, tau, base_mass, mu, Frep, Fbase, join, sh.bt, sh.fk, fk_ready, sub0 + it + 1,
                                                                   sc_store.get(), it == P.decimation - 1, SC && NW == LG_STEP_WAVES);
         } else {
             physics_substep<T, HF, NoWait, false, SC>(A, tab, k, root, q, qd, tau, base_mass, mu, Frep, Fbase, NoWait(), nullptr, nullptr, nullptr, 0,
@@ -1751,8 +1832,13 @@
 #pragma unroll
         for (int i = 0; i < 3; i++) origin[i] = B.env_origins[(size_t)e * 3 + i];
     }
+    if constexpr (ROLL) {
+        po_f = karg_request(A.post.obs);
+        roll_barrier();
+    } else {
     sh.pose[lane][0] = root[0]; sh.pose[lane][1] = root[1]; sh.pose[lane][2] = root[2]; sh.pose[lane][3] = root[5]; sh.pose[lane][4] = root[6];
     __syncthreads();
+    }
     if (ep_len % U_(ph.resample_interval, P.resample_interval) == 0) {
         if (NW > 1) { float u[4]; reset_rand.get(ResetRand<T>::CMD_STEP, lane, u); resample_commands_u(P, s_xr, u, cmd); }
         else resample_commands(P, s_xr, e, step, RNG_CMD_STEP, cmd);
@@ -1765,12 +1851,12 @@
     HeightCrew<T, NW> hc;
     float hsum = 0.0f;
     if (U_(0, P.measure_heights)) hsum = hc.template sample<HF>(A, e, k, live, root[0], root[1], root[2], root[5], root[6]);
+    if constexpr (!ROLL) {
     sh.hsum[0][lane] = hsum;
-    if constexpr (ROLL) pr_f = karg_request(A.post.rew);
     __syncthreads();
-    if constexpr (ROLL) pr = karg_take(pr_f);
     if (NW == 4) hsum = (sh.hsum[0][lane] + sh.hsum[1][lane]) + (sh.hsum[2][lane] + sh.hsum[3][lane]);
     else if (NW == 2) hsum = sh.hsum[0][lane] + sh.hsum[1][lane];
+    }
     if (U_(ph.push_interval, P.push_interval) > 0 && step % U_(ph.push_interval, P.push_interval) == 0) {
         float u[4];
         if (NW > 1) reset_rand.get(ResetRand<T>::PUSH, lane, u);
@@ -1780,7 +1866,7 @@
     }
 
     const int rep0 = 1 + k * NREP;
-    if (live) {
+    if (!ROLL && live) {
         float *cf = U_(ph.contact_forces, B.contact_forces) + ((size_t)e * (1 + K * NREP) + rep0) * 3;
 #pragma unroll
         for (int r = 0; r < NREP; r++) { cf[3 * r] = Frep[r][0]; cf[3 * r + 1] = Frep[r][1]; cf[3 * r + 2] = Frep[r][2]; }
@@ -1809,6 +1895,42 @@
     bad = group_or<K>(bad);
     const bool reset = contact_term || time_out || bad;
 
+    float q_pre[L], qd_pre[L], cmd_pre[4], z_pre;
+    if constexpr (ROLL) {
+        z_pre = root[2];
+#pragma unroll
+        for (int j = 0; j < L; j++) { q_pre[j] = q[j]; qd_pre[j] = qd[j]; }
+#pragma unroll
+        for (int i = 0; i < 4; i++) cmd_pre[i] = cmd[i];
+        origin[0] = ph.env_origins[(size_t)e * 3]; origin[1] = ph.env_origins[(size_t)e * 3 + 1]; origin[2] = ph.env_origins[(size_t)e * 3 + 2];
+        if (reset) {
+            int level = 0; bool level_changed = false;
+            reset_values<T>(A, tab, e, k, step, root, q, qd, cmd, origin, level, level_changed, s_xr, &reset_rand, lane);
+            if (live && k == 0 && level_changed) {
+                __hip_atomic_store(B.terrain_levels + e, level, __ATOMIC_RELAXED, __HIP_MEMORY_SCOPE_AGENT);
+                B.env_origins[(size_t)e * 3] = origin[0]; B.env_origins[(size_t)e * 3 + 1] = origin[1]; B.env_origins[(size_t)e * 3 + 2] = origin[2];
+            }
+            ep_len = 0;
+        }
+        sh.rst[lane] = reset ? 1 : 0; sh.root_z[lane] = root[2];
+        po = karg_take(po_f);
+        write_observations<T, true>(A, e, k, live, step, root, q, qd, act, tab, blv, bav, pg, cmd, false, &reset_rand, lane,
+                                    po.roll_obs + (size_t)(rt + 1) * po.num_envs * po.num_obs, lds_obs[lane / K], &po);
+        pr_f = karg_request(A.post.rew);
+        roll_barrier();
+        pr = karg_take(pr_f);
+        LG_PROF(PF_POST_OBS);
+        if (live) {
+            float *cf = ph.contact_forces + ((size_t)e * (1 + K * NREP) + rep0) * 3;
+#pragma unroll
+            for (int r = 0; r < NREP; r++) { cf[3 * r] = Frep[r][0]; cf[3 * r + 1] = Frep[r][1]; cf[3 * r + 2] = Frep[r][2]; }
+            if (k == 0) { float *c0 = ph.contact_forces + (size_t)e * (1 + K * NREP) * 3; c0[0] = Fbase[0]; c0[1] = Fbase[1]; c0[2] = Fbase[2]; }
+        }
+        roll_barrier();
+    }
+#define RQ_(j) (ROLL ? q_pre[j] : q[j])
+#define RQD_(j) (ROLL ? qd_pre[j] : qd[j])
+#define RCMD_(i) (ROLL ? cmd_pre[i] : cmd[i])
     if (!EARLY_POST) {
 #pragma unroll
         for (int j = 0; j < L; j++) { last_act[j] = U_(pr.last_actions, B.last_actions)[d0 + j]; if (L > 3) last_qd[j] = B.last_dof_vel[d0 + j]; }
@@ -1818,18 +1940,18 @@
     for (int j = 0; j < L; j++) {
         const float *tj = tab + j * LG_JS;
         float da = last_act[j] - act[j]; s_ar += da * da;
-        float dd = (last_qd[j] - qd[j]) / U_(pr.dt_policy, P.dt_policy); s_acc += dd * dd;
-        float ol = -fminf(q[j] - tj[J_SLO], 0.0f); ol += fmaxf(q[j] - tj[J_SHI], 0.0f); s_lim += ol;
-        s_dv += qd[j] * qd[j];
-        s_dvl += fminf(fmaxf(fabsf(qd[j]) - tj[J_DVL] * U_(pr.soft_dof_vel_limit, P.soft_dof_vel_limit), 0.0f), 1.0f);
+        float dd = (last_qd[j] - RQD_(j)) / U_(pr.dt_policy, P.dt_policy); s_acc += dd * dd;
+        float ol = -fminf(RQ_(j) - tj[J_SLO], 0.0f); ol += fmaxf(RQ_(j) - tj[J_SHI], 0.0f); s_lim += ol;
+        s_dv += RQD_(j) * RQD_(j);
+        s_dvl += fminf(fmaxf(fabsf(RQD_(j)) - tj[J_DVL] * U_(pr.soft_dof_vel_limit, P.soft_dof_vel_limit), 0.0f), 1.0f);
         s_tl += fmaxf(fabsf(tau[j]) - tj[J_TLIM] * U_(pr.soft_torque_limit, P.soft_torque_limit), 0.0f);
         s_tq += tau[j] * tau[j];
-        s_ss += fabsf(q[j] - tj[J_Q0]);
+        s_ss += fabsf(RQ_(j) - tj[J_Q0]);
     }
     s_ar = group_sum<K>(s_ar); s_acc = group_sum<K>(s_acc); s_lim = group_sum<K>(s_lim); s_dv = group_sum<K>(s_dv);
     s_dvl = group_sum<K>(s_dvl); s_tl = group_sum<K>(s_tl); s_tq = group_sum<K>(s_tq); s_ss = group_sum<K>(s_ss);
     const float *ff = Frep[T::FOOT_REP];
-    const float cmd_xy = sqrtf(cmd[0] * cmd[0] + cmd[1] * cmd[1]);
+    const float cmd_xy = sqrtf(RCMD_(0) * RCMD_(0) + RCMD_(1) * RCMD_(1));
     float fnorm = sqrtf(ff[0] * ff[0] + ff[1] * ff[1] + ff[2] * ff[2]);
     float fcf = group_sum<K>(fmaxf(fnorm - U_(pr.max_contact_force, P.max_contact_force), 0.0f));
     int stumble = group_or<K>(sqrtf(ff[0] * ff[0] + ff[1] * ff[1]) > 5.0f * fabsf(ff[2]) ? 1 : 0);
@@ -1845,7 +1967,7 @@
         fat *= filt ? 0.0f : 1.0f;
         air = group_sum<K>(air) * ((cmd_xy > 0.1f) ? 1.0f : 0.0f);
     }
-    const float base_h = U_(0, P.measure_heights) ? group_sum<K>(hsum) / (float)U_(pr.num_height_points, P.num_height_points) : root[2];
+    const float base_h = U_(0, P.measure_heights) ? group_sum<K>(hsum) / (float)U_(pr.num_height_points, P.num_height_points) : (ROLL ? z_pre : root[2]);
     float term[LG_NUM_REWARD_TERMS];
     term[LG_REW_ACTION_RATE] = s_ar;
     term[LG_REW_ANG_VEL_XY] = bav.x * bav.x + bav.y * bav.y;
@@ -1866,11 +1988,12 @@
     term[LG_REW_TORQUE_LIMITS] = s_tl;
     term[LG_REW_TORQUES] = s_tq;
     {
-        float ex = cmd[0] - blv.x, ey = cmd[1] - blv.y, ew = cmd[2] - bav.z;
+        float ex = RCMD_(0) - blv.x, ey = RCMD_(1) - blv.y, ew = RCMD_(2) - bav.z;
         term[LG_REW_TRACKING_LIN_VEL] = __expf(-(ex * ex + ey * ey) / U_(pr.tracking_sigma, P.tracking_sigma));
         term[LG_REW_TRACKING_ANG_VEL] = __expf(-(ew * ew) / U_(pr.tracking_sigma, P.tracking_sigma));
     }
     LG_PROF(PF_POST_TERMS);
+    if constexpr (ROLL) roll_barrier();
     float rew = 0.0f;
     const bool writer = live && k == 0;
     float r_t[LG_NUM_REWARD_TERMS];
@@ -1884,7 +2007,13 @@
     for (int t = 0; t < LG_NUM_REWARD_TERMS; t++) sh.r_t[t][lane] = r_t[t];
 
     LG_PROF(PF_POST_REWARD);
-    if (!EARLY_POST) { const float *eo = U_(pr.env_origins, B.env_origins); origin[0] = eo[(size_t)e * 3]; origin[1] = eo[(size_t)e * 3 + 1]; origin[2] = eo[(size_t)e * 3 + 2]; }
+    if constexpr (ROLL) {
+        if (reset) fat = 0.0f;
+        ps_f = karg_request(A.post.store);
+        roll_barrier();
+        ps = karg_take(ps_f);
+    } else {
+    if (!EARLY_POST) { const float *eo = U_(ph.env_origins, B.env_origins); origin[0] = eo[(size_t)e * 3]; origin[1] = eo[(size_t)e * 3 + 1]; origin[2] = eo[(size_t)e * 3 + 2]; }
     if (reset) {
         int level = 0; bool level_changed = false;
         reset_values<T>(A, tab, e, k, step, root, q, qd, cmd, origin, level, level_changed, s_xr, NW > 1 ? &reset_rand : nullptr, lane);
@@ -1897,18 +2026,15 @@
 
     sh.rst[lane] = reset ? 1 : 0; sh.root_z[lane] = root[2];
     if (NW > 1 && U_(pr.terrain_curriculum, P.terrain_curriculum)) asm volatile("s_waitcnt vmcnt(0)" ::: "memory");
-    if constexpr (ROLL) { po_f = karg_request(A.post.obs); ps_f = karg_request(A.post.store); }
     __syncthreads();
-    if constexpr (ROLL) { po = karg_take(po_f); ps = karg_take(ps_f); }
+    }
     if (NW == 1) { EpisodeSums es; const bool keep = live && k == 0; if (keep) es.load(A, e); es.template update<K>(A, e, lane, sh, keep, accum_slot(A, step)); }
 
-    LG_PROF(PF_POST_RESET);
+    if constexpr (!ROLL) LG_PROF(PF_POST_RESET);
 #ifdef LG_PROFILE
     { int nr = 0; for (int i = 0; i < LG_BLOCK; i += K) nr += sh.rst[i]; LG_PROF_NOTE(18, (unsigned long long)nr); }
 #endif
-    if constexpr (ROLL) write_observations<T, true>(A, e, k, live, step, root, q, qd, act, tab, blv, bav, pg, cmd, false, &reset_rand, lane,
-                                                    po.roll_obs + (size_t)(rt + 1) * po.num_envs * po.num_obs, lds_obs[lane / K], &po);
-    else write_observations<T>(A, e, k, live, step, root, q, qd, act, tab, blv, bav, pg, cmd, false, NW > 1 ? &reset_rand : nullptr, lane, roll_obs_out, ROLL ? lds_obs[lane / K] : nullptr);
+    if constexpr (!ROLL) write_observations<T>(A, e, k, live, step, root, q, qd, act, tab, blv, bav, pg, cmd, false, NW > 1 ? &reset_rand : nullptr, lane, roll_obs_out, ROLL ? lds_obs[lane / K] : nullptr);
     if (U_(0, P.measure_heights)) {
         if (NW > 1) {
             float un[HeightCrew<T, NW>::NCH][4];
@@ -1918,7 +2044,7 @@
         } else hc.write_obs(A, e, k, live, step, root[2]);
     }
 
-    LG_PROF(PF_POST_OBS);
+    if constexpr (!ROLL) LG_PROF(PF_POST_OBS);
     if constexpr (ROLL) pe_f = karg_request(A.post.store_env);
     if (live) {
 #pragma unroll
@@ -1955,6 +2081,10 @@
         }
     }
 #undef U_
+#undef RQ_
+#undef RQD_
+#undef RCMD_
+    if constexpr (ROLL) LG_PROF(PF_POST);
     }
     };
     if constexpr (ROLL) {
@@ -1962,14 +2092,28 @@
         if (threadIdx.x == 0 && A.prof && blockIdx.x < LG_NPROF_BLOCKS) A.prof[LG_NPROF + LG_NPROF_BLOCKS * 40 + blockIdx.x] = wall_clock64();
 #endif
         __syncthreads();
+        {
+            const KArgs &A = step_args<ROLL>(A_launch);
+            if (s_roll[0] == 0 && A.roll.obs0) {
+                const size_t row0 = (size_t)blockIdx.x * 16 * A.P.num_obs;
+                const int n = min(16, A.P.num_envs - (int)blockIdx.x * 16) * A.P.num_obs;
+                for (int i = threadIdx.x; i < n; i += NW * LG_BLOCK) A.roll.obs[row0 + i] = A.roll.obs0[row0 + i];
+            }
+        }
+        if (__builtin_amdgcn_readfirstlane(wave) > 0) {
+            HelperWave<T, NET, HF, NW, SC>::roll(A_launch, step0, lds_x, lds_tau, sh, sc_store.get(), lds_tab, &reset_rand, hnoise, pol_xa, pol_xb, pol_xy,
+                                                 lds_act, lds_obs, s_roll);
+        } else {
+            roll_barrier(); roll_barrier(); roll_barrier();
 #pragma unroll 1
-        for (int rt = s_roll[0]; rt < s_roll[1]; rt++) {
-            one_step(rt);
-            asm volatile("s_waitcnt lgkmcnt(0)\n\ts_barrier" ::: "memory");
+            for (int rt = s_roll[0]; rt < s_roll[1]; rt++) {
+                one_step(rt);
 #ifdef LG_PROFILE
-            if (threadIdx.x == 0 && A.prof && blockIdx.x < LG_NPROF_BLOCKS && rt + 1 < LG_NPROF_ROLL)
-                A.prof[LG_NPROF + LG_NPROF_BLOCKS * 40 + (size_t)(rt + 1) * LG_NPROF_BLOCKS + blockIdx.x] = wall_clock64();
+                if (threadIdx.x == 0 && A.prof && blockIdx.x < LG_NPROF_BLOCKS && rt + 1 < LG_NPROF_ROLL)
+                    A.prof[LG_NPROF + LG_NPROF_BLOCKS * 40 + (size_t)(rt + 1) * LG_NPROF_BLOCKS + blockIdx.x] = wall_clock64();
 #endif
+            }
+            roll_barrier();
         }
         const KArgs &A = step_args<ROLL>(A_launch);
         const lg_params &P = A.P;
@@ -2414,13 +2558,13 @@
     h.resample_interval = P.resample_interval; h.heading_command = P.heading_command; h.push_interval = P.push_interval;
     h.max_episode_length = P.max_episode_length; h.max_push_vel = P.max_push_vel; h.termination_mask = a.termination_mask;
     h.penalised_mask = a.penalised_mask;
-    h.episode_length_buf = B.episode_length_buf; h.commands = B.commands; h.contact_forces = B.contact_forces;
+    h.episode_length_buf = B.episode_length_buf; h.commands = B.commands; h.contact_forces = B.contact_forces; h.env_origins = B.env_origins;
     PostRew &r = a.post.rew;
     r.dt_policy = P.dt_policy; r.soft_dof_vel_limit = P.soft_dof_vel_limit; r.soft_torque_limit = P.soft_torque_limit;
     r.max_contact_force = P.max_contact_force; r.base_height_target = P.base_height_target; r.tracking_sigma = P.tracking_sigma;
     r.only_positive_rewards = P.only_positive_rewards; r.num_height_points = P.num_height_points; r.terrain_curriculum = P.terrain_curriculum;
     for (int t = 0; t < LG_NUM_REWARD_TERMS; t++) { r.reward_scale[t] = P.reward_scale[t]; if (P.reward_slot[t] >= 0) r.slot_mask |= 1u << t; }
-    r.last_actions = B.last_actions; r.feet_air_time = B.feet_air_time; r.last_contacts = B.last_contacts; r.env_origins = B.env_origins;
+    r.last_actions = B.last_actions; r.feet_air_time = B.feet_air_time; r.last_contacts = B.last_contacts;
     PostObs &o = a.post.obs;
     o.obs_scale_lin_vel = P.obs_scale_lin_vel; o.obs_scale_ang_vel = P.obs_scale_ang_vel; o.obs_scale_dof_pos = P.obs_scale_dof_pos;
     o.obs_scale_dof_vel = P.obs_scale_dof_vel; o.noise_lin_vel = P.noise_lin_vel; o.noise_ang_vel = P.noise_ang_vel; o.noise_gravity = P.noise_gravity;
diff --git a/legged_games_gym_amd/csrc/lg_policy.h b/legged_games_gym_amd/csrc/lg_policy.h
--- a/legged_games_gym_amd/csrc/lg_policy.h
+++ b/legged_games_gym_amd/csrc/lg_policy.h
@@ -144,6 +144,129 @@
         }
     }
 }
+
+#define LG_ACTOR_HELPERS 3
+template <bool ACT, int IN_T, int N> LG_DEV void tiles_run(const TileW<IN_T> (&w)[N], const float4 (&xv)[IN_T], float4 (&y)[N]) {
+    f32x4 acc[N];
+#pragma unroll
+    for (int n = 0; n < N; n++) { acc[n][0] = w[n].b[0]; acc[n][1] = w[n].b[1]; acc[n][2] = w[n].b[2]; acc[n][3] = w[n].b[3]; }
+#pragma unroll
+    for (int t = 0; t < IN_T; t++) {
+#pragma unroll
+        for (int n = 0; n < N; n++) acc[n] = __builtin_amdgcn_mfma_f32_16x16x4f32(w[n].w[t * 4 + 0], xv[t].x, acc[n], 0, 0, 0);
+#pragma unroll
+        for (int n = 0; n < N; n++) acc[n] = __builtin_amdgcn_mfma_f32_16x16x4f32(w[n].w[t * 4 + 1], xv[t].y, acc[n], 0, 0, 0);
+#pragma unroll
+        for (int n = 0; n < N; n++) acc[n] = __builtin_amdgcn_mfma_f32_16x16x4f32(w[n].w[t * 4 + 2], xv[t].z, acc[n], 0, 0, 0);
+#pragma unroll
+        for (int n = 0; n < N; n++) acc[n] = __builtin_amdgcn_mfma_f32_16x16x4f32(w[n].w[t * 4 + 3], xv[t].w, acc[n], 0, 0, 0);
+    }
+#pragma unroll
+    for (int n = 0; n < N; n++)
+        y[n] = ACT ? make_float4(elu1(acc[n][0]), elu1(acc[n][1]), elu1(acc[n][2]), elu1(acc[n][3])) : make_float4(acc[n][0], acc[n][1], acc[n][2], acc[n][3]);
+}
+
+struct HelperActor {
+    TileW<3> w0[3];
+    TileW<8> w1[2];
+    TileW<4> w2[1];
+    TileW<2> w3[1];
+    LG_DEV void request(const PolicyArgs &A, int h, int lane) {
+        w0[0].load(A.w[0], A.b[0], h, lane); w0[1].load(A.w[0], A.b[0], h + 3, lane);
+        if (h < 2) w0[2].load(A.w[0], A.b[0], h + 6, lane);
+        w1[0].load(A.w[1], A.b[1], h < 2 ? h : 2, lane);
+        if (h == 2) w1[1].load(A.w[1], A.b[1], 3, lane);
+        if (h < 2) w2[0].load(A.w[2], A.b[2], h, lane);
+        if (h == 1) w3[0].load(A.w[3], A.b[3], 0, lane);
+    }
+    LG_DEV void layer0(const PolicyArgs &A, const float (*lds_obs)[48], float4 (*xb)[64], int block, int h, int lane) const {
+        const int g = lane >> 4;
+        int env = block * 16 + (lane & 15);
+        if (env >= A.num_envs) env = A.num_envs - 1;
+        const float *o = A.obs + (size_t)env * A.num_obs;
+        float4 xv[3];
+#pragma unroll
+        for (int t = 0; t < 3; t++) {
+            float v[4];
+#pragma unroll
+            for (int r = 0; r < 4; r++) { const int k = 16 * t + 4 * g + r; v[r] = k < A.num_obs ? (lds_obs ? lds_obs[lane & 15][k] : o[k]) : 0.0f; }
+            xv[t] = make_float4(v[0], v[1], v[2], v[3]);
+        }
+        if (h < 2) {
+            float4 y[3];
+            tiles_run<true>(w0, xv, y);
+            xb[h][lane] = y[0]; xb[h + 3][lane] = y[1]; xb[h + 6][lane] = y[2];
+        } else {
+            const TileW<3> w[2] = {w0[0], w0[1]};
+            float4 y[2];
+            tiles_run<true>(w, xv, y);
+            xb[h][lane] = y[0]; xb[h + 3][lane] = y[1];
+        }
+    }
+    LG_DEV void layer1(const float4 (*xb)[64], float4 (*xa)[64], int h, int lane) const {
+        float4 xv[8];
+#pragma unroll
+        for (int t = 0; t < 8; t++) xv[t] = xb[t][lane];
+        if (h < 2) {
+            const TileW<8> w[1] = {w1[0]};
+            float4 y[1];
+            tiles_run<true>(w, xv, y);
+            xa[h][lane] = y[0];
+        } else {
+            float4 y[2];
+            tiles_run<true>(w1, xv, y);
+            xa[2][lane] = y[0]; xa[3][lane] = y[1];
+        }
+    }
+    LG_DEV void layer2(const PolicyArgs &A, const float4 (*xa)[64], float4 (*xb)[64], float4 (*xy)[64], int block, int h, int lane, int64_t step) const {
+        if (h < 2) {
+            float4 xv[4], y[1];
+#pragma unroll
+            for (int t = 0; t < 4; t++) xv[t] = xa[t][lane];
+            tiles_run<true>(w2, xv, y);
+            xb[h][lane] = y[0];
+        } else {
+            const int g = lane >> 4;
+            int env = block * 16 + (lane & 15);
+            if (env >= A.num_envs) env = A.num_envs - 1;
+            float u[4];
+            rand4(A.seed ^ 0x9E3779B97F4A7C15ull, env, step, 100 + g, 0, u);
+            float rad0 = sqrtf(-2.0f * __logf(fmaxf(u[0], 1e-12f))), rad1 = sqrtf(-2.0f * __logf(fmaxf(u[2], 1e-12f)));
+            float s0, c0, s1, c1;
+            __sincosf(6.2831853f * u[1], &s0, &c0);
+            __sincosf(6.2831853f * u[3], &s1, &c1);
+            const float eps[4] = {rad0 * c0, rad0 * s0, rad1 * c1, rad1 * s1};
+            float ns[4];
+#pragma unroll
+            for (int r = 0; r < 4; r++) { const int a = 4 * g + r; ns[r] = (a < A.num_actions && !A.deterministic) ? A.std[a] * eps[r] : 0.0f; }
+            xy[0][lane] = make_float4(ns[0], ns[1], ns[2], ns[3]);
+        }
+    }
+    LG_DEV void output(const PolicyArgs &A, const float4 (*xb)[64], const float4 (*xy)[64], int block, int lane, float (*lds_act)[16]) const {
+        const int g = lane >> 4;
+        int env = block * 16 + (lane & 15);
+        const bool live = env < A.num_envs;
+        if (!live) env = A.num_envs - 1;
+        const float4 nv = xy[0][lane];
+        const float ns[4] = {nv.x, nv.y, nv.z, nv.w};
+        const float4 xv[2] = {xb[0][lane], xb[1][lane]};
+        float4 yv[1];
+        tiles_run<false>(w3, xv, yv);
+        const float y[4] = {yv[0].x, yv[0].y, yv[0].z, yv[0].w};
+#pragma unroll
+        for (int r = 0; r < 4; r++) {
+            const int a = 4 * g + r;
+            if (a < A.num_actions) {
+                const float m = y[r], act = m + ns[r];
+                lds_act[a][lane & 15] = act;
+                if (live) {
+                    if (A.mean) A.mean[(size_t)env * A.num_actions + a] = m;
+                    A.actions[(size_t)env * A.num_actions + a] = act;
+                }
+            }
+        }
+    }
+};
 
 template <int D0T, int D1T, int D2T, int D3T>
 __global__ void __launch_bounds__(64 * LG_POLICY_WAVES) k_policy_act(const PolicyArgs A) {
```

Result: slower. 71.33 million env-steps/s (-7.3%).
